# loicmagne/tinynerf

Measured on AMD Instinct MI355X. Metric: ray-samples/sec (K-Planes training step: sampler + render fwd + bwd + Adam), higher is better.
Workload: dtype f32 (f16x2-split products)

## Files before the change

include/tinynerf_hip.h:

```cpp
#ifndef TINYNERF_HIP_H
#define TINYNERF_HIP_H

#include <stdint.h>

#ifdef __cplusplus
extern "C" {
#endif

#define TN_ABI_VERSION 6

enum {
    TN_OK = 0,
    TN_E_NULL = -1,
    TN_E_SIZE = -2,
    TN_E_CONFIG = -3,
    TN_E_ALIGN = -4
};

const char *tn_last_error_string(void);
const char *tn_last_warning_string(void);
int tn_abi_version(void);

int tn_weights_fwd(const float *sigmas, const float *steps, const int32_t *info, float threshold,
                   float *weights, int64_t n_samples, int64_t n_rays, void *stream);
// ... 78 lines not shown
#define TN_MLP_STASHED 2
#define TN_MLP_CHAIN_ONLY 4
#define TN_MLP_WGRAD_ONLY 8
#define TN_MLP_GRAD_Y_ROWS 16

#define TN_MLP_BF16X3 32

#define TN_MLP_F16X2 64

#define TN_MLP_ROWS_ONLY 128
#define TN_MLP_X_FROM_ROWS 256

#define TN_MLP_SKIP_LAST 1024
#define TN_MLP_LAYERWISE 2048
#define TN_MLP_LEAN 512

typedef struct tn_mlp_desc {
    int32_t n_layers;
    int32_t in_dim;
    int32_t dims[TN_MLP_MAX_LAYERS + 1];
    int32_t encoding;
    int32_t n_freqs;
    int32_t out_activation;
    int32_t flags;
    const float *freqs;
    const float *weights[TN_MLP_MAX_LAYERS];
    const float *biases[TN_MLP_MAX_LAYERS];
    const int32_t *aux_index;
    int32_t aux_stride;
    int32_t reserved;
    const float *row_gate;
    const float *x_rows;
    float *grad_x_rows;
    int64_t x_rows_tile_stride;
    int64_t grad_x_rows_tile_stride;
    const void *grad_x_mask_rows;
    int64_t grad_x_mask_tile_stride;
} tn_mlp_desc;

#define TN_MERGE_MAX_HEADS 4
typedef struct tn_merge_head {
    const float *weight, *bias;
    int32_t rows, ld, col0, reserved;
    float *out_weight, *out_bias;
    const float *grad_merged_weight, *grad_merged_bias;
} tn_merge_head;
int tn_linear_merge_fwd(int32_t n_heads, const tn_merge_head *heads, const float *w_last, const float *b_last, int32_t F, void *stream);
int tn_linear_merge_bwd(int32_t n_heads, const tn_merge_head *heads, const float *w_last, const float *b_last, int32_t F,
                        float *grad_w_last, float *grad_b_last, void *stream);

int tn_linear_fwd(const float *x, const float *weight, const float *bias, int64_t n, int32_t in_features,
                  int32_t out_features, float *y, void *stream);
int tn_linear_bwd(const float *x, const float *weight, const float *grad_y, int64_t n, int32_t in_features,
                  int32_t out_features, float *grad_x, float *grad_weight, float *grad_bias, void *stream);

int tn_mlp_rows_view(const tn_mlp_desc *desc, int64_t n, int64_t *y_rows, int64_t *grad_y_rows, int64_t *tile_stride);
int tn_mlp_rows_view_hidden(const tn_mlp_desc *desc, int64_t n, int64_t *h_rows, int64_t *grad_h_rows, int64_t *mask_rows,
                            int64_t *tile_stride);

int tn_mlp_fwd(const tn_mlp_desc *desc, const float *x, const float *aux, int64_t n, float *y,
               float *pre_act, void *stream);
int64_t tn_mlp_fwd_workspace_bytes(const tn_mlp_desc *desc, int64_t n);
int tn_mlp_fwd_ws(const tn_mlp_desc *desc, const float *x, const float *aux, int64_t n, float *y, void *workspace,
                  int64_t workspace_bytes, void *stream);
int tn_mlp_fwd_stash(const tn_mlp_desc *desc, const float *x, const float *aux, int64_t n, float *y,
                     void *workspace, int64_t workspace_bytes, void *stream);
int tn_mlp_fwd_stash_pair(const tn_mlp_desc *desc, const tn_mlp_desc *partner, const float *x, const float *aux, int64_t n,
                          float *y, float *partner_y, void *workspace, int64_t workspace_bytes, void *partner_workspace,
                          int64_t partner_workspace_bytes, void *stream);
int tn_dir_encode(const float *dirs, int64_t n, const float *freqs, int n_freqs, float *out, int stride, void *stream);
int64_t tn_mlp_bwd_workspace_bytes(const tn_mlp_desc *desc, int64_t n);
int tn_mlp_bwd(const tn_mlp_desc *desc, const float *x, const float *aux, const float *grad_y,
               int64_t n, float *const *grad_weights, float *const *grad_biases, float *grad_x,
               void *workspace, int64_t workspace_bytes, void *stream);
int tn_mlp_bwd_pair(const tn_mlp_desc *desc, const tn_mlp_desc *partner, const float *x, const float *aux,
                    const float *grad_y, const float *partner_grad_y, int64_t n, float *const *grad_weights,
                    float *const *grad_biases, float *const *partner_grad_weights, float *const *partner_grad_biases,
                    float *grad_x, void *workspace, int64_t workspace_bytes, void *partner_workspace,
                    int64_t partner_workspace_bytes, void *stream);

int tn_mlp_lean_supported(const tn_mlp_desc *desc, const tn_mlp_desc *partner);

#define TN_KPLANES_MAX_SCALES 4
typedef struct tn_kplanes_desc {
    int32_t n_scales;
    int32_t channels;
    int32_t height[TN_KPLANES_MAX_SCALES];
    int32_t width[TN_KPLANES_MAX_SCALES];
    const float *planes[TN_KPLANES_MAX_SCALES][3];
} tn_kplanes_desc;

int tn_kplanes_fwd(const tn_kplanes_desc *desc, const float *x, int64_t x_stride, int64_t n,
                   float *feat, void *stream);
int tn_kplanes_bwd(const tn_kplanes_desc *desc, const float *x, int64_t x_stride, int64_t n,
                   const float *grad_feat, float *const (*grad_planes)[3], void *stream);

int tn_plane_reg_fwd(const float *plane, int H, int W, int C, double *sums, void *stream);
int tn_plane_reg_bwd(const float *plane, int H, int W, int C, float cy, float cx, float cl1,
                     const float *upstream, float *grad, void *stream);

#define TN_MULTI_MAX 32
typedef struct tn_plane_reg_item {
    const float *plane;
    float *grad;
    int32_t H, W, C;
    float cy, cx, cl1;
} tn_plane_reg_item;
int tn_plane_reg_multi(const tn_plane_reg_item *items, int32_t n_items, float upstream, double *sums, void *stream);

#define TN_COBAFA_MAX_LEVELS 8
typedef struct tn_cobafa_desc {
    int32_t n_levels;
    int32_t coef_res[3];
    int32_t res[TN_COBAFA_MAX_LEVELS][3];
    int32_t channels[TN_COBAFA_MAX_LEVELS];
    float freqs[TN_COBAFA_MAX_LEVELS];
    const float *coef;
    const float *basis[TN_COBAFA_MAX_LEVELS];
} tn_cobafa_desc;
int tn_cobafa_fwd(const tn_cobafa_desc *desc, const float *x, int64_t n, float *feat, void *stream);
int tn_cobafa_bwd(const tn_cobafa_desc *desc, const float *x, int64_t n, const float *grad_feat, float *grad_coef,
                  float *const *grad_basis, void *stream);

#define TN_HASHGRID_MAX_LEVELS 16
typedef struct tn_hashgrid_desc {
    int32_t n_levels, features;
    int32_t res[TN_HASHGRID_MAX_LEVELS];
    int32_t hashed[TN_HASHGRID_MAX_LEVELS];
    int64_t entries[TN_HASHGRID_MAX_LEVELS];
    int64_t offset[TN_HASHGRID_MAX_LEVELS];
    const float *table;
} tn_hashgrid_desc;
int tn_hashgrid_fwd(const tn_hashgrid_desc *desc, const float *x, int64_t x_stride, int64_t n, float *feat, void *stream);
int tn_hashgrid_bwd(const tn_hashgrid_desc *desc, const float *x, int64_t x_stride, int64_t n, const float *grad_feat,
                    float *grad_table, void *stream);

int tn_kplanes_mlp_fwd_pair(const tn_kplanes_desc *kdesc, const float *coords, int64_t coord_stride, const tn_mlp_desc *desc,
                            const tn_mlp_desc *partner, const float *aux, int64_t n, float *feat, float *y, float *partner_y,
                            void *workspace, int64_t workspace_bytes, void *partner_workspace, int64_t partner_workspace_bytes,
                            void *stream);

int tn_kplanes_mlp_fwd(const tn_kplanes_desc *kdesc, const float *coords, int64_t coord_stride, const tn_mlp_desc *desc, int64_t n,
                       float *feat, float *y, void *stream);

int tn_kplanes_mlp_bwd_pair(const tn_kplanes_desc *kdesc, const float *coords, int64_t coord_stride,
                            float *const (*grad_planes)[3], const tn_mlp_desc *desc, const tn_mlp_desc *partner,
                            const float *feat, const float *aux, const float *grad_y, const float *partner_grad_y, int64_t n,
                            float *const *grad_weights, float *const *grad_biases, float *const *partner_grad_weights,
                            float *const *partner_grad_biases, float *grad_feat, void *workspace, int64_t workspace_bytes,
                            void *partner_workspace, int64_t partner_workspace_bytes, void *stream);

int tn_basis_dot_fwd(const float *f, const float *basis, int64_t n, int32_t channels, int32_t n_out, int32_t activation,
                     float *out, void *stream);
int tn_basis_dot_bwd(const float *f, const float *basis, const float *grad_out, int64_t n, int32_t channels, int32_t n_out,
                     int32_t activation, float *grad_f, float *grad_basis, int32_t accumulate_f, void *stream);

int tn_ray_aux(const float *packed, const int32_t *info, int64_t n_rays, int32_t *ray_ids, float *steps, float *dirs,
               void *stream);

int tn_mse_grad(const float *rendered, const float *target, int64_t n, float scale, const float *scale_dev, float *grad,
                double *sumsq, void *stream);
int tn_render_rays_fwd(const float *sigmas, const float *steps, const float *rgbs, const int32_t *info, const float *bg,
                       float threshold, float *weights, float *rendered, float *gate, int64_t n_samples, int64_t n_rays,
                       void *stream);
int tn_render_rays_bwd(const float *sigmas, const float *steps, const float *rgbs, const int32_t *info, const float *bg,
                       const float *weights, const float *grad_rendered, float *grad_rgbs, float *grad_sigmas,
                       int64_t n_samples, int64_t n_rays, void *stream);
int tn_mse_grad_gated(const float *rendered, const float *target, int64_t n, float scale, const float *scale_dev,
                      const float *gate, float *grad, double *sumsq, void *stream);

enum { TN_DIST_LINEAR = 0, TN_DIST_UNBOUNDED = 1 };
int tn_distortion_fwd(const float *weights, const float *t_values, const float *steps, const int32_t *info, int64_t n_rays,
                      int32_t warp, float near, float range, float *loss, double *sum, void *stream);
int tn_distortion_bwd(const float *weights, const float *t_values, const float *steps, const int32_t *info, int64_t n_rays,
                      int32_t warp, float near, float range, const float *grad_loss, float scale, const float *scale_dev,
                      float *grad_weights, void *stream);
int tn_render_rays_bwd_dw(const float *sigmas, const float *steps, const float *rgbs, const int32_t *info, const float *bg,
                          const float *weights, const float *grad_rendered, const float *grad_weights_extra, float *grad_rgbs,
                          float *grad_sigmas, int64_t n_samples, int64_t n_rays, void *stream);
int tn_ssim_workspace_bytes(int64_t H, int64_t W, int32_t C, int64_t *bytes);
int tn_ssim(const float *a, const float *b, int64_t H, int64_t W, int32_t C, float data_range, float *map, void *workspace,
            int64_t workspace_bytes, float *mean, void *stream);
int tn_gather_rays(const float *rays_o, const float *rays_d, const float *rgbs, const int32_t *idx, int64_t n,
                   float *out_o, float *out_d, float *out_rgb, void *stream);
typedef struct tn_camera_table {
    const float *c2w;
    const float *lens;
    const int32_t *model;
    const int32_t *size;
    const int64_t *pixel_offset;
    const uint8_t *rgb;
    int64_t n_pixels;
    int32_t n_img, reserved;
} tn_camera_table;
enum { TN_LENS_PINHOLE = 0, TN_LENS_OPENCV = 1, TN_LENS_FISHEYE = 2 };
int tn_camera_rays(const tn_camera_table *cams, const int32_t *idx, int64_t first, int64_t stride, int64_t n,
                   float *out_o, float *out_d, float *out_rgb, void *stream);
int tn_points_workspace_bytes(int64_t n, int64_t *bytes);
int tn_points_compact(const float *rays_o, const float *rays_d,
                      const float *rgb,
                      const float *opacity, const float *depth,
                      const float *bg,
                      const float *box,
                      float min_opacity, int64_t n, int64_t capacity,
                      float *points,
                      uint8_t *colors,
                      int32_t *src,
                      int64_t *count,
                      void *workspace, void *stream);

int tn_adam_step(float *param, float *grad, float *exp_avg, float *exp_avg_sq, int64_t n, float lr, float beta1,
                 float beta2, float eps, float weight_decay, int32_t step, int32_t zero_grad, void *stream);

typedef struct tn_adam_item {
    float *param, *grad, *exp_avg, *exp_avg_sq;
    int64_t n;
} tn_adam_item;
int tn_adam_multi(const tn_adam_item *items, int32_t n_items, float lr, float beta1, float beta2, float eps,
                  float weight_decay, int32_t step, int32_t zero_grad, void *stream);

int tn_adam_multi_gated(const tn_adam_item *items, int32_t n_items, float lr, float beta1, float beta2, float eps,
                        float weight_decay, int32_t *step_dev, const float *gate, int32_t zero_grad, void *stream);

typedef struct tn_adam_reg_item {
    const float *param;
    float *param_out, *grad, *exp_avg, *exp_avg_sq;
    int64_t n;
    int32_t H, W, C, sum_slot;
    float cy, cx, cl1;
    int32_t row0, row1, reserved;
} tn_adam_reg_item;
int tn_adam_reg_multi(const tn_adam_reg_item *items, int32_t n_items, float lr, float beta1, float beta2, float eps,
                      float weight_decay, int32_t step, int32_t zero_grad, float upstream, double *sums, void *stream);

#ifdef __cplusplus
}
#endif
#endif
```

tinynerf_amd/_lib.py:

```python
from __future__ import annotations

import ctypes as C
import os
from typing import Optional

import torch

_HERE = os.path.dirname(os.path.abspath(__file__))
LIB_PATH = os.environ.get("TN_LIB_PATH") or os.path.join(_HERE, "libtinynerf_hip.so")

TN_MLP_MAX_LAYERS = 12
TN_KPLANES_MAX_SCALES = 4

MARCH_AABB, MARCH_UNBOUNDED = 0, 1
CONTRACT_AABB, CONTRACT_MIP360_INF, CONTRACT_MIP360_L2 = 0, 1, 2
ACT_NONE, ACT_EXP_M1, ACT_SIGMOID, ACT_EXP = 0, 1, 2, 3
ENC_NONE, ENC_POSENC, ENC_DIR_CAT, ENC_AUX_CAT = 0, 1, 2, 3
DIST_LINEAR, DIST_UNBOUNDED = 0, 1


class SamplerDesc(C.Structure):
    _fields_ = [
        ("marcher", C.c_int32), ("contraction", C.c_int32), ("n_samples", C.c_int32),
        ("grid_d", C.c_int32), ("grid_h", C.c_int32), ("grid_w", C.c_int32),
        ("aabb", C.c_float * 6), ("near", C.c_float), ("far", C.c_float),
        ("step_size", C.c_float), ("threshold", C.c_float),
        ("t_table", C.c_void_p), ("delta_table", C.c_void_p), ("grid", C.c_void_p), ("jitter", C.c_void_p),
        ("seed", C.c_uint64), ("use_rng", C.c_int32), ("reserved", C.c_int32),
        ("coarse", C.c_void_p),
    ]


class MlpDesc(C.Structure):
    _fields_ = [
        ("n_layers", C.c_int32), ("in_dim", C.c_int32), ("dims", C.c_int32 * (TN_MLP_MAX_LAYERS + 1)),
        ("encoding", C.c_int32), ("n_freqs", C.c_int32), ("out_activation", C.c_int32), ("flags", C.c_int32),
        ("freqs", C.c_void_p),
        ("weights", C.c_void_p * TN_MLP_MAX_LAYERS), ("biases", C.c_void_p * TN_MLP_MAX_LAYERS),
        ("aux_index", C.c_void_p), ("aux_stride", C.c_int32), ("reserved", C.c_int32),
        ("row_gate", C.c_void_p),
        ("x_rows", C.c_void_p), ("grad_x_rows", C.c_void_p), ("x_rows_tile_stride", C.c_int64), ("grad_x_rows_tile_stride", C.c_int64),
        ("grad_x_mask_rows", C.c_void_p), ("grad_x_mask_tile_stride", C.c_int64),
    ]


class MergeHead(C.Structure):
    _fields_ = [
        ("weight", C.c_void_p), ("bias", C.c_void_p),
        ("rows", C.c_int32), ("ld", C.c_int32), ("col0", C.c_int32), ("reserved", C.c_int32),
        ("out_weight", C.c_void_p), ("out_bias", C.c_void_p),
        ("grad_merged_weight", C.c_void_p), ("grad_merged_bias", C.c_void_p),
    ]


class KPlanesDesc(C.Structure):
    _fields_ = [
        ("n_scales", C.c_int32), ("channels", C.c_int32),
        ("height", C.c_int32 * TN_KPLANES_MAX_SCALES), ("width", C.c_int32 * TN_KPLANES_MAX_SCALES),
        ("planes", (C.c_void_p * 3) * TN_KPLANES_MAX_SCALES),
    ]


TN_COBAFA_MAX_LEVELS = 8
TN_MULTI_MAX = 32
MLP_ACCUM_GRAD_X = 1
MLP_STASHED = 2
MLP_CHAIN_ONLY = 4
MLP_WGRAD_ONLY = 8
MLP_GRAD_Y_ROWS = 16
MLP_BF16X3 = 32
MLP_F16X2 = 64
MLP_ROWS_ONLY = 128
MLP_X_FROM_ROWS = 256
MLP_LEAN = 512
MLP_SKIP_LAST = 1024
MLP_LAYERWISE = 2048
ABI_VERSION = 6


class PlaneRegItem(C.Structure):
    _fields_ = [("plane", C.c_void_p), ("grad", C.c_void_p), ("H", C.c_int32), ("W", C.c_int32), ("C", C.c_int32),
                ("cy", C.c_float), ("cx", C.c_float), ("cl1", C.c_float)]


class AdamItem(C.Structure):
    _fields_ = [("param", C.c_void_p), ("grad", C.c_void_p), ("exp_avg", C.c_void_p), ("exp_avg_sq", C.c_void_p), ("n", C.c_int64)]



class AdamRegItem(C.Structure):
    _fields_ = [("param", C.c_void_p), ("param_out", C.c_void_p), ("grad", C.c_void_p), ("exp_avg", C.c_void_p), ("exp_avg_sq", C.c_void_p),
                ("n", C.c_int64), ("H", C.c_int32), ("W", C.c_int32), ("C", C.c_int32), ("sum_slot", C.c_int32),
                ("cy", C.c_float), ("cx", C.c_float), ("cl1", C.c_float), ("row0", C.c_int32), ("row1", C.c_int32), ("reserved", C.c_int32)]


class CobafaDesc(C.Structure):
    _fields_ = [
        ("n_levels", C.c_int32), ("coef_res", C.c_int32 * 3), ("res", (C.c_int32 * 3) * TN_COBAFA_MAX_LEVELS),
        ("channels", C.c_int32 * TN_COBAFA_MAX_LEVELS), ("freqs", C.c_float * TN_COBAFA_MAX_LEVELS),
        ("coef", C.c_void_p), ("basis", C.c_void_p * TN_COBAFA_MAX_LEVELS),
    ]


TN_HASHGRID_MAX_LEVELS = 16


class HashGridDesc(C.Structure):
    _fields_ = [
        ("n_levels", C.c_int32), ("features", C.c_int32),
        ("res", C.c_int32 * TN_HASHGRID_MAX_LEVELS), ("hashed", C.c_int32 * TN_HASHGRID_MAX_LEVELS),
        ("entries", C.c_int64 * TN_HASHGRID_MAX_LEVELS), ("offset", C.c_int64 * TN_HASHGRID_MAX_LEVELS),
        ("table", C.c_void_p),
    ]


LENS_PINHOLE, LENS_OPENCV, LENS_FISHEYE = 0, 1, 2


class CameraTable(C.Structure):
    _fields_ = [("c2w", C.c_void_p), ("lens", C.c_void_p), ("model", C.c_void_p), ("size", C.c_void_p), ("pixel_offset", C.c_void_p),
                ("rgb", C.c_void_p), ("n_pixels", C.c_int64), ("n_img", C.c_int32), ("reserved", C.c_int32)]


_lib: Optional[C.CDLL] = None
_TRACE = bool(os.environ.get("TN_TRACE"))


def lib() -> C.CDLL:
    global _lib
    if _lib is None:
        if not os.path.exists(LIB_PATH):
            raise RuntimeError(
                f"{LIB_PATH} is missing: the HIP kernels were not built. Run `python -m tinynerf_amd.build` "
                "(needs hipcc). tinynerf_amd has no CPU fallback.")
        _lib = C.CDLL(LIB_PATH)
        _lib.tn_last_error_string.restype = C.c_char_p
        got = int(_lib.tn_abi_version())
        if got != ABI_VERSION:
            _lib = None
            raise RuntimeError(f"{LIB_PATH} has ABI version {got}, tinynerf_amd expects {ABI_VERSION}: rebuild it (`python -m tinynerf_amd.build`)")
    return _lib


def check(rc: int, fn: str) -> None:
    if rc != 0:
        msg = lib().tn_last_error_string().decode(errors="replace")
        raise RuntimeError(f"{fn} failed (code {rc}): {msg}")


def ptr(t: Optional[torch.Tensor]) -> C.c_void_p:
    return C.c_void_p(None) if t is None else C.c_void_p(t.data_ptr())


def stream(device: torch.device) -> C.c_void_p:
    return C.c_void_p(torch.cuda.current_stream(device).cuda_stream)


def require_cuda(*tensors: Optional[torch.Tensor]) -> torch.device:
    dev = None
    for t in tensors:
        if t is None:
            continue
        if not t.is_cuda:
            raise RuntimeError("tinynerf_amd: tensor must be a CUDA (HIP) tensor -- there is no CPU path")
        if not t.is_contiguous():
            raise RuntimeError("tinynerf_amd: tensor must be contiguous")
        if dev is None:
            dev = t.device
        elif t.device != dev:
            raise RuntimeError("tinynerf_amd: tensors are on different devices")
    assert dev is not None
    return dev


def call_plain(name: str, *args) -> None:
    check(getattr(lib(), name)(*args), name)
# ... 12 lines not shown
```

tinynerf_amd/config.py:

```python
from __future__ import annotations

import itertools
import os
from dataclasses import dataclass, fields, replace
from typing import Iterator, Mapping

MATMULS = ("f16x2", "bf16x3", "fp32")
_FLAGS = {"rows_handoff": "TN_ROWS_HANDOFF", "merge_last": "TN_MERGE_LAST", "heads_pair": "TN_HEADS_PAIR", "kp_lean": "TN_KP_LEAN",
          "infer_pair": "TN_INFER_PAIR", "adam_overlap": "TN_ADAM_OVERLAP", "side_plan": "TN_SIDE_PLAN"}


@dataclass(frozen=True)
class Config:
    matmul: str = "f16x2"
    rows_handoff: bool = True
    merge_last: bool = True
    heads_pair: bool = True
    kp_lean: bool = True
    infer_pair: bool = True
    adam_overlap: bool = True
    side_plan: bool = True

    def validate(self) -> "Config":
        if self.matmul not in MATMULS:
            raise RuntimeError(f"TN_MATMUL={self.matmul}: fp32, bf16x3 or f16x2")
        off = [n for n in _FLAGS if not getattr(self, n)]
        if self.matmul != "f16x2" and off:
            raise RuntimeError(f"tinynerf_amd.config: {', '.join(_FLAGS[n] + '=0' for n in off)} with TN_MATMUL={self.matmul}: the A / B switches "
                               "belong to the f16x2 path; with bf16x3 / fp32 they stay at their defaults (see tinynerf_amd/config.py)")
        if self.merge_last and not self.rows_handoff:
            return replace(self, merge_last=False)
        return self

    @staticmethod
    def from_env(env: Mapping[str, str] = os.environ) -> "Config":
        kw = {"matmul": env.get("TN_MATMUL", "f16x2").lower()}
        for name, var in _FLAGS.items():
            kw[name] = env.get(var, "1") != "0"
        return Config(**kw).validate()

    def as_env(self) -> dict:
        return {"TN_MATMUL": self.matmul, **{var: "1" if getattr(self, name) else "0" for name, var in _FLAGS.items()}}


def supported_combinations() -> Iterator[Config]:
    seen = set()
    for mm in MATMULS:
        names = list(_FLAGS) if mm == "f16x2" else []
        for bits in itertools.product((True, False), repeat=len(names)):
            try:
                c = Config(matmul=mm, **dict(zip(names, bits))).validate()
            except RuntimeError:
                continue
            if c not in seen:
                seen.add(c)
                yield c


def apply(cfg: Config) -> None:
    from . import fused, models, run
    cfg = cfg.validate()
    models.MATMUL = cfg.matmul
    fused.ROWS_HANDOFF, fused.MERGE_LAST, fused.HEADS_PAIR_BACKWARD = cfg.rows_handoff, cfg.merge_last, cfg.heads_pair
    fused.KP_LEAN, fused.INFER_PAIR = cfg.kp_lean, cfg.infer_pair
    run.ADAM_OVERLAP, run.SIDE_PLAN = cfg.adam_overlap, cfg.side_plan


CONFIG = Config.from_env()
```

tinynerf_amd/csrc/kplanes.hip:

```cpp
#include "kplanes_scatter.h"
#include <algorithm>

namespace {

using tn::f32x4k;

struct KpArgs {
    int n_scales, C;
    int H[TN_KPLANES_MAX_SCALES], W[TN_KPLANES_MAX_SCALES];
    const float *planes[TN_KPLANES_MAX_SCALES][3];
    float *grads[TN_KPLANES_MAX_SCALES][3];
};

template <int NV>
__global__ __launch_bounds__(256) void kplanes_fwd_kernel(KpArgs a, const float *__restrict__ x, int64_t x_stride,
                                                          int64_t n, float *__restrict__ feat)
{
    const int lane = tn::lane_id(), j = lane & 31, h = lane >> 5;
    const int64_t n_tiles = (n + 31) >> 5;
    const int C = a.C, FD = a.n_scales * C;
    for (int64_t tile = (int64_t)blockIdx.x * 4 + (threadIdx.x >> 6); tile < n_tiles; tile += (int64_t)gridDim.x * 4) {
        const int64_t row = tile * 32 + j;
        if (row >= n) continue;
        const float xs[3] = {x[row * x_stride], x[row * x_stride + 1], x[row * x_stride + 2]};
        for (int s = 0; s < a.n_scales; ++s) {
            f32x4k prod[NV];
#pragma unroll
            for (int q = 0; q < NV; ++q) prod[q] = f32x4k{1.f, 1.f, 1.f, 1.f};
#pragma unroll
            for (int p = 0; p < 3; ++p) {
                if (a.planes[s][p] == nullptr) continue;
                float u, v;
                tn::pair_uv(xs, p, u, v);
                const tn::PlaneTaps t = tn::plane_taps(u, v, a.H[s], a.W[s], C);
                f32x4k val[NV];
                tn::plane_gather<NV>(a.planes[s][p], t, h * (C / 2), val);
#pragma unroll
                for (int q = 0; q < NV; ++q) prod[q] = prod[q] * val[q];
            }
            f32x4k *o = reinterpret_cast<f32x4k *>(feat + row * FD + s * C + h * (C / 2));
#pragma unroll
            for (int q = 0; q < NV; ++q) o[q] = prod[q];
        }
    }
}

template <int NV>
__global__ __launch_bounds__(256, 3) void kplanes_bwd_kernel(KpArgs a, const float *__restrict__ x, int64_t x_stride,
                                                          int64_t n, const float *__restrict__ grad_feat)
{
    __shared__ __attribute__((aligned(16))) float lds[4 * tn::KP_WAVE_LDS];
    const int lane = tn::lane_id(), j = lane & 31, h = lane >> 5;
    float *wave_lds = lds + (threadIdx.x >> 6) * tn::KP_WAVE_LDS;
    const int64_t n_tiles = (n + 31) >> 5;
    const int C = a.C, FD = a.n_scales * C;
    for (int64_t tile = (int64_t)blockIdx.x * 4 + (threadIdx.x >> 6); tile < n_tiles; tile += (int64_t)gridDim.x * 4) {
        const int64_t row = tile * 32 + j;
        const bool valid = row < n;
        const int64_t rr = valid ? row : 0;
        const float xs[3] = {x[rr * x_stride], x[rr * x_stride + 1], x[rr * x_stride + 2]};
        for (int s = 0; s < a.n_scales; ++s) {
            f32x4k g[NV];
#pragma unroll
            for (int q = 0; q < NV; ++q)
                g[q] = valid ? reinterpret_cast<const f32x4k *>(grad_feat + row * FD + s * C + h * (C / 2))[q]
                             : f32x4k{0.f, 0.f, 0.f, 0.f};
            const float *const pl[3] = {a.planes[s][0], a.planes[s][1], a.planes[s][2]};
            float *const gr[3] = {a.grads[s][0], a.grads[s][1], a.grads[s][2]};
            tn::kp_scatter_scale<NV, 4>(pl, gr, a.H[s], a.W[s], C, xs, valid, g, h * (C / 2), wave_lds, j, h);
        }
    }
}

int make_args(const tn_kplanes_desc *d, KpArgs &a, float *const (*grads)[3])
{
    TN_REQUIRE(d, TN_E_NULL, "kplanes: null descriptor");
    TN_REQUIRE(d->n_scales >= 1 && d->n_scales <= TN_KPLANES_MAX_SCALES, TN_E_CONFIG, "kplanes: n_scales out of range");
    TN_REQUIRE(d->channels == 8 || d->channels == 16 || d->channels == 32, TN_E_CONFIG, "kplanes: channels must be 8, 16 or 32");
    a.n_scales = d->n_scales; a.C = d->channels;
    for (int s = 0; s < d->n_scales; ++s) {
        TN_REQUIRE(d->height[s] > 0 && d->width[s] > 0, TN_E_SIZE, "kplanes: bad plane resolution");
        TN_REQUIRE((int64_t)d->height[s] * d->width[s] * d->channels < (1ll << 30), TN_E_SIZE, "kplanes: plane too large (2^30 elements)");
        a.H[s] = d->height[s]; a.W[s] = d->width[s];
        TN_REQUIRE(d->planes[s][0], TN_E_NULL, "kplanes: null plane pointer");
        for (int p = 0; p < 3; ++p) {
            TN_REQUIRE(((uintptr_t)d->planes[s][p] & 15) == 0, TN_E_ALIGN, "kplanes: planes must be 16-byte aligned");
            a.planes[s][p] = d->planes[s][p];
            a.grads[s][p] = nullptr;
            if (grads && d->planes[s][p]) {
                TN_REQUIRE(grads[s][p], TN_E_NULL, "kplanes: null grad plane pointer");
                a.grads[s][p] = grads[s][p];
            }
        }
    }
    return TN_OK;
}

template <int ACT>
__device__ __forceinline__ float bd_act(float v)
{
    if (ACT == TN_ACT_EXP_M1) return expf(v - 1.0f);
    if (ACT == TN_ACT_EXP) return expf(v);
    if (ACT == TN_ACT_SIGMOID) return 1.0f / (1.0f + expf(-v));
    return v;
}

template <int ACT>
__global__ __launch_bounds__(256) void basis_dot_fwd_kernel(const float *__restrict__ f, const float *__restrict__ basis, int64_t n, int C,
                                                            int K, float *__restrict__ out)
{
    const int lane = tn::lane_id();
    const int64_t wave = ((int64_t)blockIdx.x * blockDim.x + threadIdx.x) >> 6, n_waves = ((int64_t)gridDim.x * blockDim.x) >> 6;
    for (int64_t i = wave; i < n; i += n_waves) {
        const float *fi = f + i * C, *bi = basis + i * (int64_t)K * C;
        for (int k = 0; k < K; ++k) {
            float acc = 0.0f;
            for (int c = lane; c < C; c += 64) acc += fi[c] * bi[k * C + c];
            acc = tn::wave_sum(acc);
            if (lane == 0) out[i * K + k] = bd_act<ACT>(acc);
        }
    }
}

template <int ACT>
__global__ __launch_bounds__(256) void basis_dot_bwd_kernel(const float *__restrict__ f, const float *__restrict__ basis,
                                                            const float *__restrict__ g_out, int64_t n, int C, int K,
                                                            float *__restrict__ g_f, float *__restrict__ g_basis, int accumulate_f)
{
    const int lane = tn::lane_id();
    const int64_t wave = ((int64_t)blockIdx.x * blockDim.x + threadIdx.x) >> 6, n_waves = ((int64_t)gridDim.x * blockDim.x) >> 6;
    for (int64_t i = wave; i < n; i += n_waves) {
        const float *fi = f + i * C, *bi = basis + i * (int64_t)K * C;
        float gv[4];
        for (int k = 0; k < K; ++k) {
            float acc = 0.0f;
            for (int c = lane; c < C; c += 64) acc += fi[c] * bi[k * C + c];
            acc = tn::wave_sum(acc);
            const float g = g_out[i * K + k];
            if (ACT == TN_ACT_EXP_M1) gv[k] = g * expf(fminf(fmaxf(acc - 1.0f, -15.0f), 15.0f));
            else if (ACT == TN_ACT_EXP) gv[k] = g * expf(fminf(fmaxf(acc, -15.0f), 15.0f));
            else if (ACT == TN_ACT_SIGMOID) { const float y = 1.0f / (1.0f + expf(-acc)); gv[k] = g * y * (1.0f - y); }
            else gv[k] = g;
        }
        for (int c = lane; c < C; c += 64) {
            const float fc = fi[c];
            float a = accumulate_f ? g_f[i * C + c] : 0.0f;
            for (int k = 0; k < K; ++k) {
                a += gv[k] * bi[k * C + c];
                if (g_basis) g_basis[(i * K + k) * C + c] = gv[k] * fc;
            }
            g_f[i * C + c] = a;
        }
    }
}

inline unsigned tile_blocks(int64_t n) { return (unsigned)std::min<int64_t>(((n + 31) / 32 + 3) / 4, 256 * 8); }

}

extern "C" int tn_kplanes_fwd(const tn_kplanes_desc *desc, const float *x, int64_t x_stride, int64_t n, float *feat,
                              void *stream)
{
    KpArgs a;
    if (int rc = make_args(desc, a, nullptr)) return rc;
    TN_REQUIRE(n >= 0 && x_stride >= 3, TN_E_SIZE, "tn_kplanes_fwd: bad size");
    if (n == 0) return TN_OK;
    TN_REQUIRE(x && feat, TN_E_NULL, "tn_kplanes_fwd: null pointer");
    TN_REQUIRE(((uintptr_t)feat & 15) == 0, TN_E_ALIGN, "tn_kplanes_fwd: feat must be 16-byte aligned");
    hipStream_t s = (hipStream_t)stream;
    const dim3 grid(tile_blocks(n)), block(256);
    switch (a.C) {
    case 8: kplanes_fwd_kernel<1><<<grid, block, 0, s>>>(a, x, x_stride, n, feat); break;
    case 16: kplanes_fwd_kernel<2><<<grid, block, 0, s>>>(a, x, x_stride, n, feat); break;
    default: kplanes_fwd_kernel<4><<<grid, block, 0, s>>>(a, x, x_stride, n, feat); break;
    }
    return tn::check_launch("kplanes_fwd_kernel");
}
// ... 57 lines not shown
```

tinynerf_amd/csrc/kplanes_device.h:

```cpp
#pragma once
#include "tn_common.h"

namespace tn {

typedef float f32x4k __attribute__((ext_vector_type(4)));

struct PlaneTaps {
    int off[4];
    float w[4];
    int cell;
};

__device__ __forceinline__ PlaneTaps plane_taps(float u, float v, int H, int W, int C) {
    PlaneTaps t;
    float u1 = u + 1.0f, v1 = v + 1.0f;
    asm volatile("" : "+v"(u1), "+v"(v1));
    float ix = (u1 * 0.5f) * (float)(W - 1);
    float iy = (v1 * 0.5f) * (float)(H - 1);
    asm volatile("" : "+v"(ix), "+v"(iy));
    const float x0f = floorf(ix), y0f = floorf(iy);
    const float fx = ix - x0f, fy = iy - y0f;
    const float gx = (x0f + 1.0f) - ix, gy = (y0f + 1.0f) - iy;
    t.w[0] = gx * gy; t.w[1] = fx * gy; t.w[2] = gx * fy; t.w[3] = fx * fy;
    const bool bx0 = x0f >= 0.0f && x0f < (float)W, bx1 = x0f + 1.0f >= 0.0f && x0f + 1.0f < (float)W;
    const bool by0 = y0f >= 0.0f && y0f < (float)H, by1 = y0f + 1.0f >= 0.0f && y0f + 1.0f < (float)H;
    const int x0 = bx0 ? (int)x0f : 0, x1 = bx1 ? (int)x0f + 1 : 0;
    const int y0 = by0 ? (int)y0f : 0, y1 = by1 ? (int)y0f + 1 : 0;
    t.off[0] = (bx0 && by0) ? (y0 * W + x0) * C : -1;
    t.off[1] = (bx1 && by0) ? (y0 * W + x1) * C : -1;
    t.off[2] = (bx0 && by1) ? (y1 * W + x0) * C : -1;
    t.off[3] = (bx1 && by1) ? (y1 * W + x1) * C : -1;
    const float cx = fminf(fmaxf(x0f, -2.0f), (float)W + 1.0f), cy = fminf(fmaxf(y0f, -2.0f), (float)H + 1.0f);
    t.cell = ((int)cy + 2) * (W + 4) + (int)cx + 2;
    return t;
}

template <int NV, int CS = 4>
__device__ __forceinline__ void plane_gather(const float *__restrict__ plane, const PlaneTaps &t, int c0, f32x4k (&out)[NV]) {
    f32x4k tex[4][NV];
    float w[4];
    const char *base = reinterpret_cast<const char *>(plane);
#pragma unroll
    for (int k = 0; k < 4; ++k) {
        const bool in = t.off[k] >= 0;
        unsigned boff = (unsigned)((in ? t.off[k] : 0) + c0) * 4u;
        asm volatile("" : "+v"(boff));
        w[k] = in ? t.w[k] : 0.0f;
#pragma unroll
        for (int v = 0; v < NV; ++v) tex[k][v] = *reinterpret_cast<const f32x4k *>(base + boff + (unsigned)(v * CS * 4));
    }
#pragma unroll
    for (int v = 0; v < NV; ++v) {
        f32x4k acc = tex[0][v] * w[0];
#pragma unroll
        for (int k = 1; k < 4; ++k)
#pragma unroll
            for (int e = 0; e < 4; ++e) acc[e] = __builtin_fmaf(tex[k][v][e], w[k], acc[e]);
        out[v] = acc;
    }
}

__device__ __forceinline__ void pair_uv(const float x[3], int p, float &u, float &v) {
    u = (p == 2) ? x[1] : x[0];
    v = (p == 0) ? x[1] : x[2];
}

}
```

tinynerf_amd/csrc/kplanes_scatter.h:

```cpp
#pragma once
#include "kplanes_device.h"

#ifdef TN_PHASE_TIMERS
extern __device__ unsigned long long tn_phase_cycles_b[16];
#endif
namespace tn {

constexpr int KP_GS = 36;
constexpr int KP_WAVE_LDS = 32 * KP_GS + 2 * 4 * 32;

template <int NV, int CS>
__device__ __forceinline__ void kp_scatter_scale(const float *const (&planes)[3], float *const (&grads)[3], int H, int W, int C,
                                                 const float (&xs)[3], bool valid, const f32x4k (&g)[NV], int c0,
                                                 float *__restrict__ wave_lds, int j, int h)
{
#ifdef TN_PHASE_TIMERS
    unsigned long long pts_ = __builtin_amdgcn_s_memtime();
#define TN_PTS(k) { __builtin_amdgcn_sched_barrier(0); const unsigned long long n_ = __builtin_amdgcn_s_memtime(); if (tn::lane_id() == 0) atomicAdd(&tn_phase_cycles_b[k], n_ - pts_); pts_ = __builtin_amdgcn_s_memtime(); __builtin_amdgcn_sched_barrier(0); }
#endif
    float *tileG = wave_lds;
    int *tileO = reinterpret_cast<int *>(tileG + 32 * KP_GS);
    float *tileW = tileG + 32 * KP_GS + 4 * 32;
    PlaneTaps t[3];
    f32x4k val[3][NV];
#pragma unroll
    for (int p = 0; p < 3; ++p) {
        float u, v;
        pair_uv(xs, p, u, v);
        t[p] = plane_taps(u, v, H, W, C);
        if (planes[p]) {
            plane_gather<NV, CS>(planes[p], t[p], c0, val[p]);
            __builtin_amdgcn_sched_barrier(0);
        } else {
#pragma unroll
            for (int q = 0; q < NV; ++q) val[p][q] = f32x4k{1.f, 1.f, 1.f, 1.f};
        }
    }
#ifdef TN_PHASE_TIMERS
    TN_PTS(8)
#endif
#pragma unroll
    for (int p = 0; p < 3; ++p) {
        if (grads[p] == nullptr) continue;
#pragma unroll
        for (int q = 0; q < NV; ++q) {
            const f32x4k gp = p == 0 ? g[q] * val[1][q] * val[2][q]
                                     : (p == 1 ? g[q] * val[0][q] * val[2][q] : g[q] * (val[0][q] * val[1][q]));
            *reinterpret_cast<f32x4k *>(tileG + j * KP_GS + c0 + CS * q) = gp;
        }
#pragma unroll
        for (int k = 0; k < 2; ++k) {
            const int o = h ? t[p].off[2 + k] : t[p].off[0 + k];
            const float w = h ? t[p].w[2 + k] : t[p].w[0 + k];
            const bool live = valid && o >= 0;
            tileO[(2 * h + k) * 32 + j] = live ? 4 * o : 0;
            tileW[(2 * h + k) * 32 + j] = live ? w : 0.0f;
        }
        const int cell = valid ? t[p].cell : -1 - j;
        const int next_cell = __shfl_down(cell, 1, 64);
        const int dcell = (j < 31) ? next_cell - cell : 0x40000000;
        const int rowlen = W + 4;
        const unsigned run_end = (unsigned)__ballot(dcell != 0);
        const unsigned mv_xp = (unsigned)__ballot(dcell == 1), mv_xm = (unsigned)__ballot(dcell == -1);
        const unsigned mv_yp = (unsigned)__ballot(dcell == rowlen), mv_ym = (unsigned)__ballot(dcell == -rowlen);
        const unsigned mv_pp = (unsigned)__ballot(dcell == rowlen + 1), mv_mp = (unsigned)__ballot(dcell == rowlen - 1);
        const unsigned mv_pm = (unsigned)__ballot(dcell == -rowlen + 1), mv_mm = (unsigned)__ballot(dcell == -rowlen - 1);
        const unsigned mv_diag = mv_pp | mv_mp | mv_pm | mv_mm;
        asm volatile("" ::: "memory");
#ifdef TN_PHASE_TIMERS
        TN_PTS(9)
#endif
        const int c = j;
        char *const gplane = reinterpret_cast<char *>(grads[p]);
        const unsigned c4 = 4u * (unsigned)c;
        auto add_at = [&](unsigned byte_off, float v) { atomicAdd(reinterpret_cast<float *>(gplane + byte_off), v); };
        if (c < C) {
            const int4 *O0 = reinterpret_cast<const int4 *>(tileO + (2 * h) * 32), *O1 = O0 + 8;
            const f32x4k *W0 = reinterpret_cast<const f32x4k *>(tileW + (2 * h) * 32);
            const f32x4k *W1 = W0 + 8;
            float a0 = 0.0f, a1 = 0.0f;
#pragma clang loop unroll(disable)
            for (int s4 = 0; s4 < 8; ++s4) {
                const f32x4k w0 = W0[s4], w1 = W1[s4];
                const int4 o0v = O0[s4], o1v = O1[s4];
                const int o0a[4] = {o0v.x, o0v.y, o0v.z, o0v.w}, o1a[4] = {o1v.x, o1v.y, o1v.z, o1v.w};
                float gv[4];
#pragma unroll
                for (int u = 0; u < 4; ++u) gv[u] = tileG[(4 * s4 + u) * KP_GS + c];
#pragma unroll
                for (int u = 0; u < 4; ++u) {
                    const int sI = 4 * s4 + u;
                    a0 = fmaf(gv[u], w0[u], a0);
                    a1 = fmaf(gv[u], w1[u], a1);
                    if ((run_end >> sI) & 1u) {
                        const unsigned o0 = (unsigned)o0a[u] + c4, o1 = (unsigned)o1a[u] + c4;
                        if ((mv_xp >> sI) & 1u) {
                            add_at(o0, a0);
                            a0 = a1; a1 = 0.0f;
                        } else if ((mv_xm >> sI) & 1u) {
                            add_at(o1, a1);
                            a1 = a0; a0 = 0.0f;
                        } else if ((mv_yp >> sI) & 1u) {
                            const float t0 = __shfl_xor(a0, 32, 64), t1 = __shfl_xor(a1, 32, 64);
                            if (h == 0) {
                                add_at(o0, a0);
                                add_at(o1, a1);
                            }
                            a0 = h == 0 ? t0 : 0.0f; a1 = h == 0 ? t1 : 0.0f;
                        } else if ((mv_ym >> sI) & 1u) {
                            const float t0 = __shfl_xor(a0, 32, 64), t1 = __shfl_xor(a1, 32, 64);
                            if (h == 1) {
                                add_at(o0, a0);
                                add_at(o1, a1);
                            }
                            a0 = h == 1 ? t0 : 0.0f; a1 = h == 1 ? t1 : 0.0f;
                        } else if ((mv_diag >> sI) & 1u) {
                            const float t0 = __shfl_xor(a0, 32, 64), t1 = __shfl_xor(a1, 32, 64);
                            if ((mv_pp >> sI) & 1u) {
                                add_at(o0, a0);
                                if (h == 0) add_at(o1, a1);
                                a0 = h == 0 ? t1 : 0.0f; a1 = 0.0f;
                            } else if ((mv_mp >> sI) & 1u) {
                                add_at(o1, a1);
                                if (h == 0) add_at(o0, a0);
                                a1 = h == 0 ? t0 : 0.0f; a0 = 0.0f;
                            } else if ((mv_pm >> sI) & 1u) {
                                add_at(o0, a0);
                                if (h == 1) add_at(o1, a1);
                                a0 = h == 1 ? t1 : 0.0f; a1 = 0.0f;
                            } else {
                                add_at(o1, a1);
                                if (h == 1) add_at(o0, a0);
                                a1 = h == 1 ? t0 : 0.0f; a0 = 0.0f;
                            }
                        } else {
                            add_at(o0, a0);
                            add_at(o1, a1);
                            a0 = 0.0f; a1 = 0.0f;
                        }
                    }
                }
            }
        }
        asm volatile("" ::: "memory");
// ... 8 lines not shown
```

tinynerf_amd/csrc/mlp_bwd2.hip:

```cpp
#include "mlp_stage.h"
#include "kplanes_scatter.h"
#include "phase_timers.h"
#include <algorithm>
#include <type_traits>

extern "C" int64_t tn_mlp_bwd_layers_workspace_bytes(const tn_mlp_desc *desc, int64_t n);
extern "C" int tn_mlp_bwd_layers(const tn_mlp_desc *desc, const float *x, const float *aux, const float *grad_y, int64_t n,
                                 float *const *grad_weights, float *const *grad_biases, float *grad_x, float *workspace, void *stream);
extern "C" int tn_mlp_wgrad_rows2(const float *g_rows, int64_t g_stride, const float *g_rows2, int64_t g_stride2, const float *a_rows,
                                  int64_t a_stride, int na, float *gW, int ldw, int col0, float *gB, float *gW2, int ldw2, int col02,
                                  float *gB2, int64_t n, void *stream);
extern "C" int tn_heads_dx_rows(const float *w_a, int ld_a, int col0_a, const float *w_b, int ld_b, int col0_b, const float *g_a, int64_t gs_a,
                                const float *g_b, int64_t gs_b, int F, float *out, int64_t out_stride, const void *mask, int64_t mask_stride,
                                int64_t n, void *stream);
extern "C" int tn_mlp_wgrad_lean_pair(const tn_mlp_desc *desc, const tn_mlp_desc *partner, const float *x, const float *aux, int64_t n,
                                      float *const *gw, float *const *gb, float *const *gws, float *const *gbs, const float *ws_a,
                                      const float *ws_b, void *stream);
extern "C" int tn_mlp_wgrad_lean_check(const tn_mlp_desc *desc, const tn_mlp_desc *partner, const float *x, const float *aux, int64_t n,
                                       float *const *gw, float *const *gb, float *const *gws, float *const *gbs, const float *ws_a,
                                       const float *ws_b);
extern "C" int tn_mlp_wgrad_rows(const float *g_rows, int64_t g_stride, int ng, const float *a_rows, int64_t a_stride, int na, float *gW,
                                 int ldw, int col0, int kmax, float *gB, int64_t n, void *stream);

TN_PHASE_COUNTERS(tn_phase_cycles_b, tn_debug_phase_cycles_b)
#define TN_PTB_BEGIN TN_PHASE_BEGIN(ptb_)
#define TN_PTB(k) TN_PHASE(tn_phase_cycles_b, ptb_, k)
namespace {

using tn::f32x16;
using tn::f32x4;
using tn::act_grad;
using namespace tn::mlp;

template <int N, class F>
__device__ __forceinline__ void static_for(F &&f) {
    if constexpr (N > 0) {
        static_for<N - 1>(f);
        f(std::integral_constant<int, N - 1>{});
    }
}

struct PairArgs { MlpArgs b; const float *gy; float *stash; int64_t g0_stride = 0; };

struct KpBwd {
    int H[3], W[3];
    const float *planes[3][3];
    float *grads[3][3];
    const float *coords;
    int64_t coord_stride;
};

template <int H>
__device__ __forceinline__ void first_dgrad(const float *__restrict__ Wf, int sf, int out, const float (&gp)[4],
                                            const unsigned (&mask)[H / 32], int h, f32x16 (&G)[H / 32])
{
#pragma unroll
    for (int kb = 0; kb < H / 32; ++kb) {
#pragma unroll
        for (int q = 0; q < 4; ++q) {
            f32x4 acc4 = {0.f, 0.f, 0.f, 0.f};
#pragma unroll
            for (int o = 0; o < 4; ++o) {
                if (o < out) {
                    const f32x4 w = *reinterpret_cast<const f32x4 *>(Wf + o * sf + 32 * kb + 8 * q + 4 * h);
                    acc4 += w * gp[o];
                }
            }
#pragma unroll
            for (int u = 0; u < 4; ++u) G[kb][4 * q + u] = mask_keep(acc4[u], mask[kb], 4 * q + u);
        }
    }
}

template <int H, int NH, int WPB, bool STASHED, bool ACCUM = false, bool PAIR = false, bool KP = false, bool G0B = false>
__global__ __launch_bounds__(WPB * 64) void mlp_chain_kernel(MlpArgs a, const float *__restrict__ x, const float *__restrict__ aux,
                                                             const float *__restrict__ gy, int64_t n, float *__restrict__ gx,
                                                             float *__restrict__ stash, PairArgs pr, KpBwd kp)
{
    static_assert(!KP || (STASHED && PAIR && !ACCUM && H == 64), "the fused scatter belongs to the paired, stashed chain of the width-64 heads");
    static_assert(!G0B || (STASHED && !PAIR && !KP && !ACCUM), "G0B: another head's G_0 rows join a stashed, unpaired chain's grad_x");
    extern __shared__ __attribute__((aligned(16))) float lds[];
    constexpr int T = H / 32;
    constexpr int L = NH + 1;
    stage_weights(a, lds);
    const float *ldsb = lds + a.lds_floats;
    if constexpr (PAIR || G0B) stage_weights(pr.b, lds + a.lds_floats);
    __syncthreads();
    if constexpr (STASHED && NH > 1) {
        constexpr int sl = H + 4;
        for (int l = 1; l < NH; ++l) {
            float *W = lds + a.w_off[l];
            for (int e = threadIdx.x; e < H * H; e += blockDim.x) {
                const int r = e / H, c = e - r * H;
                if (r < c) { const float t = W[r * sl + c]; W[r * sl + c] = W[c * sl + r]; W[c * sl + r] = t; }
            }
        }
        __syncthreads();
    }
    const int lane = tn::lane_id(), j_ = lane & 31, h_ = lane >> 5;
    const int wave = __builtin_amdgcn_readfirstlane(threadIdx.x >> 6);
    const int64_t n_tiles = (n + 31) >> 5;
    const int out = a.out_dim;

    unsigned nmask[NH][T];
    float npre[4], ngy[4];
    unsigned bmask[T];
    float bpre[4], bgy[4];
    const StashTile sb(H, 1, 0);
    const StashTile sa(H, NH, a.enc, a.in_dim, a.K0_pad);
    auto fetch_tile = [&](int64_t t) {
        if constexpr (PAIR) {
            const float *tb = pr.stash + t * (int64_t)sb.floats(), *qb = tb + sb.pre();
            const unsigned *mb = reinterpret_cast<const unsigned *>(tb + sb.masks());
#pragma unroll
            for (int ob = 0; ob < T; ++ob) bmask[ob] = mb[sb.mask(0, ob) + lane];
            int64_t rb = t * 32 + j_;
            rb = rb < n ? rb : n - 1;
            const int outb = pr.b.out_dim;
#pragma unroll
            for (int o = 0; o < 4; ++o) {
                const int oc = o < outb ? o : outb - 1;
                bpre[o] = qb[oc * 32 + j_];
                bgy[o] = pr.gy[rb * outb + oc];
            }
        }
        const float *ta = stash + t * (int64_t)sa.floats(), *q = ta + sa.pre();
        const unsigned *mm = reinterpret_cast<const unsigned *>(ta + sa.masks());
#pragma unroll
        for (int l = 0; l < NH; ++l)
#pragma unroll
            for (int ob = 0; ob < T; ++ob) nmask[l][ob] = mm[sa.mask(l, ob) + lane];
        int64_t r = t * 32 + j_;
        r = r < n ? r : n - 1;
#pragma unroll
        for (int o = 0; o < 4; ++o) {
            const int oc = o < out ? o : out - 1;
            npre[o] = q[oc * 32 + j_];
            ngy[o] = gy[r * out + oc];
        }
    };
    if constexpr (STASHED) {
        const int64_t t0 = (int64_t)blockIdx.x * WPB + wave;
        fetch_tile(t0 < n_tiles ? t0 : n_tiles - 1);
    }

    for (int64_t tile = (int64_t)blockIdx.x * WPB + wave; tile < n_tiles; tile += (int64_t)gridDim.x * WPB) {
        int j = j_, h = h_;
        asm volatile("" : "+v"(j), "+v"(h));
        TN_PTB_BEGIN
        const int64_t row = tile * 32 + j;
        const bool valid = row < n;
        float *st = stash + tile * (int64_t)sa.floats();
        float *stH = st, *stG = st + sa.g(0), *stP = st + sa.g_pre(), *stE = st + sa.e();
        const float *Wf = lds + a.w_off[L - 1];
        const float *Bf = lds + a.b_off[L - 1];
        const int sf = a.stride[L - 1];
        unsigned mask[NH][T];
        float gp[4];
        unsigned pmask[T];
        float gpb[4];
        if constexpr (STASHED) {
#pragma unroll
            for (int l = 0; l < NH; ++l)
#pragma unroll
                for (int ob = 0; ob < T; ++ob) mask[l][ob] = nmask[l][ob];
#pragma unroll
            for (int o = 0; o < 4; ++o) gp[o] = (valid && o < out) ? ngy[o] * act_grad(npre[o], a.out_act) : 0.0f;
            if constexpr (PAIR) {
#pragma unroll
// ... 139 lines not shown
                {
                    constexpr int NG = 4 * T;
                    float cur[4], nxt[4];
#pragma unroll
                    for (int u = 0; u < 4; ++u) cur[u] = W0[(4 * h + u) * s0 + 32 * kt + j];
#pragma unroll
                    for (int g = 0; g < NG; ++g) {
                        const int tn_ = g >> 2, q = g & 3;
                        if (g + 1 < NG) {
#pragma unroll
                            for (int u = 0; u < 4; ++u) nxt[u] = W0[(8 * (g + 1) + 4 * h + u) * s0 + 32 * kt + j];
                        }
#pragma unroll
                        for (int u = 0; u < 4; ++u) acc = tn::mfma32(cur[u], G[tn_][4 * q + u], acc);
                        __builtin_amdgcn_sched_barrier(0);
#pragma unroll
                        for (int u = 0; u < 4; ++u) cur[u] = nxt[u];
                    }
                }
                if constexpr (PAIR || G0B) {
                    const float *W0b = ldsb + pr.b.w_off[0];
                    const int s0b = pr.b.stride[0];
#pragma unroll
                    for (int tn_ = 0; tn_ < T; ++tn_)
#pragma unroll
                        for (int q = 0; q < 4; ++q)
#pragma unroll
                            for (int u = 0; u < 4; ++u)
                                acc = tn::mfma32(W0b[(32 * tn_ + 8 * q + 4 * h + u) * s0b + 32 * kt + j], Gb[tn_][4 * q + u], acc);
                }
                tn::pin16(acc);
                if constexpr (KP) {
                    if (kt == 0) gacc[0] = acc; else if (kt == 1) gacc[1] = acc; else gacc[2] = acc;
                    if (gx == nullptr) continue;
                }
                if (gxr != nullptr) {
                    if (!KP && a.gx_mask_rows != nullptr) {
                        const unsigned mb = a.gx_mask_rows[tile * a.gx_mask_stride + kt * 64 + lane];
#pragma unroll
                        for (int r = 0; r < 16; ++r) acc[r] = mask_keep(acc[r], mb, r);
                    }
                    store_rows(gxr + kt * 32 * 32, acc, 0, j, h);
                    continue;
                }
                if constexpr (ACCUM) {
                    if (valid) {
#pragma unroll
                        for (int q = 0; q < 4; ++q) {
                            f32x4 v = old[q];
#pragma unroll
                            for (int u = 0; u < 4; ++u) v[u] += acc[4 * q + u];
                            *reinterpret_cast<f32x4 *>(gx + row * a.in_dim + 32 * kt + 8 * q + 4 * h) = v;
                        }
                    }
#pragma unroll
                    for (int q = 0; q < 4; ++q) old[q] = oldn[q];
                } else if (valid) {
#pragma unroll
                    for (int q = 0; q < 4; ++q) {
                        const int f0 = 32 * kt + 8 * q + 4 * h;
                        if (f0 + 3 < a.in_dim && (a.in_dim & 3) == 0) {
                            f32x4 v;
#pragma unroll
                            for (int u = 0; u < 4; ++u) v[u] = acc[4 * q + u];
                            f32x4 *dst = reinterpret_cast<f32x4 *>(gx + row * a.in_dim + f0);
                            if (a.accum_gx) v += *dst;
                            *dst = v;
                        } else {
#pragma unroll
                            for (int u = 0; u < 4; ++u)
                                if (f0 + u < a.in_dim) {
                                    float *dst = gx + row * a.in_dim + f0 + u;
                                    *dst = a.accum_gx ? *dst + acc[4 * q + u] : acc[4 * q + u];
                                }
                        }
                    }
                }
            }
            TN_PTB(2)
            if constexpr (KP) {
                const float *cr = kp.coords + (valid ? row : 0) * kp.coord_stride;
                const float xs[3] = {cr[0], cr[1], cr[2]};
                float *wave_lds = lds + a.lds_floats + pr.b.lds_floats + wave * tn::KP_WAVE_LDS;
#pragma unroll
                for (int sc = 0; sc < 3; ++sc) {
                    tn::f32x4k g4[4];
#pragma unroll
                    for (int q = 0; q < 4; ++q) g4[q] = tn::f32x4k{gacc[sc][4 * q], gacc[sc][4 * q + 1], gacc[sc][4 * q + 2], gacc[sc][4 * q + 3]};
                    const float *const pl[3] = {kp.planes[sc][0], kp.planes[sc][1], kp.planes[sc][2]};
                    float *const gr[3] = {kp.grads[sc][0], kp.grads[sc][1], kp.grads[sc][2]};
                    tn::kp_scatter_scale<4, 8>(pl, gr, kp.H[sc], kp.W[sc], 32, xs, valid, g4, 4 * h, wave_lds, j, h);
                    TN_PTB(3 + sc)
                }
            }
        }
    }
}

struct WgradArgs {
    int n_layers, in_dim, K0, K0_pad, enc, n_freqs, out_dim, Tk0, total_tiles;
    int tk_skip;
    const int *aux_index;
    int aux_stride;
    float *gW[TN_MLP_MAX_LAYERS];
    float *gB[TN_MLP_MAX_LAYERS];
    int K[TN_MLP_MAX_LAYERS], N[TN_MLP_MAX_LAYERS];
};

constexpr int RS = 36;

template <bool AUX>
__device__ __forceinline__ void first_layer_column(const WgradArgs &a, int q, int xs, int aw, const float *ldsX, const float *ldsA, int h,
                                                   const float *&cp, int &cstride)
{
    if (q < xs) { cp = ldsX + 16 * h * a.in_dim + q; cstride = a.in_dim; }
    else if (AUX && q < a.K0_pad) { cp = ldsA + 16 * h * aw + (q - xs); cstride = aw; }
}

__device__ __forceinline__ void flush_tile(const WgradArgs &a, int l, int tn_, int tk, f32x16 &acc, float dbsum, int i, int h)
{
    tn::pin16(acc);
    const int Nl = a.N[l], Kl = a.K[l];
    const int k = 32 * tk + i;
    const bool kok = k < Kl;
    float *col = a.gW[l] + (kok ? (l == 0 ? layer0_col(a.enc, a.K0, a.in_dim, k) : k) : 0);
#pragma unroll
    for (int r = 0; r < 16; ++r) {
        const int nn = 32 * tn_ + tn::frow(r, h);
        if (kok && nn < Nl) atomicAdd(col + (int64_t)nn * Kl, acc[r]);
    }
    if (tk == 0) {
        dbsum += __shfl_xor(dbsum, 32, 64);
        const int nn = 32 * tn_ + i;
        if (h == 0 && nn < Nl) atomicAdd(&a.gB[l][nn], dbsum);
    }
}

template <int H, int NH>
__device__ __forceinline__ void decode_tile(const WgradArgs &a, int id, int &l, int &tn_, int &tk) {
    constexpr int T = H / 32;
    const int tk0n = a.Tk0 - a.tk_skip;
    const int n0 = T * tk0n;
    if (id < n0) { l = 0; tn_ = id / tk0n; tk = a.tk_skip + id - tn_ * tk0n; return; }
    id -= n0;
    if (id < (NH - 1) * T * T) { l = 1 + id / (T * T); id -= (l - 1) * T * T; tn_ = id / T; tk = id - tn_ * T; return; }
    id -= (NH - 1) * T * T;
    l = NH; tn_ = 0; tk = id;
}

template <int H, int NH, int MAXS, int NW, int NCH, bool AUX>
__global__ __launch_bounds__(NW * 64) void mlp_wgrad_kernel(WgradArgs a, const float *__restrict__ x, const float *__restrict__ aux,
                                                            int64_t n, const float *__restrict__ stash)
{
    extern __shared__ __attribute__((aligned(16))) float lds[];
    const int lane = tn::lane_id(), i_ = lane & 31, h_ = lane >> 5;
    const int wave = __builtin_amdgcn_readfirstlane(threadIdx.x >> 6);
    const int64_t n_tiles = (n + 31) >> 5;
    const int xs = x_slots(a.enc, a.in_dim);
    const int xs_st = 32 * a.tk_skip >= xs ? 0 : xs;
    const StashTile st(H, NH, a.enc, a.in_dim, a.K0_pad);
    const int extra = st.extra;
    const int R = st.rows_w();
    const int row_chunks = R * 8;
    const int x_chunks = xs_st > 0 ? (32 * a.in_dim) / 4 : 0;
    const int aw = AUX ? a.K0_pad - a.in_dim : 0;
    float *ldsR = lds;
    float *ldsX = lds + R * RS;
    float *ldsA = ldsX + (xs_st > 0 ? 32 * a.in_dim : 0);
    f32x16 acc[MAXS];
    float dbacc[MAXS];
    int tl[MAXS], ttn[MAXS], ttk[MAXS];
    tn::zero_tiles(acc);
#pragma unroll
    for (int m = 0; m < MAXS; ++m) {
// ... 210 lines not shown
            for (int e = 0; e < 4; ++e) {
                f32x4 gv0 = g0[e], gv1 = g1[e];
                if (!gok) { gv0 = f32x4{0.f, 0.f, 0.f, 0.f}; gv1 = gv0; }
                f32x4 av0 = {0.f, 0.f, 0.f, 0.f}, av1;
                if (kind == 0) {
                    if (cp != nullptr) {
#pragma unroll
                        for (int u = 0; u < 4; ++u) av0[u] = cp[(4 * e + u) * cstride];
                    }
                    av1 = av0;
                } else if (kind == 1) { av0 = hc[e]; av1 = av0; }
                else { av0 = r0[e]; av1 = r1[e]; }
#pragma unroll
                for (int u = 0; u < 4; ++u) {
                    acc[0] = tn::mfma32(gv0[u], av0[u], acc[0]);
                    acc[1] = tn::mfma32(gv1[u], av1[u], acc[1]);
                }
                gs0 += (gv0[0] + gv0[1]) + (gv0[2] + gv0[3]);
                gs1 += (gv1[0] + gv1[1]) + (gv1[2] + gv1[3]);
            }
            if (kind == 2 || tk == 0) { dbacc[0] += gs0; dbacc[1] += gs1; }
        }
        __syncthreads();
        cur ^= 1;
    }
    if (kind < 0) return;
#pragma unroll
    for (int m = 0; m < 2; ++m) flush_tile(a, l, kind == 2 ? 0 : m, kind == 2 ? m : tk, acc[m], dbacc[m], i_, h_);
}

struct WgradPlan { int R, Rt, xs, aw, chunks; size_t lds; };
WgradPlan wgrad_plan(int enc, int in_dim, int K0_pad, int H, int NH, bool x_elsewhere = false) {
    WgradPlan p;
    const StashTile st(H, NH, enc, in_dim, K0_pad);
    p.R = st.rows_w(); p.Rt = st.rows();
    p.xs = x_elsewhere ? 0 : x_slots(enc, in_dim);
    p.aw = enc == TN_ENC_AUX_CAT ? K0_pad - in_dim : 0;
    p.chunks = p.R * 8 + (p.xs > 0 ? 8 * in_dim : 0);
    p.lds = ((size_t)p.R * 36 + (p.xs > 0 ? 32 * (size_t)in_dim : 0) + 32 * (size_t)p.aw) * 4;
    return p;
}

MlpArgs compact_first_layer(const MlpArgs &a)
{
    MlpArgs c = a;
    const int H = a.N[0];
    c.K0_pad = (a.in_dim + 7) & ~7;
    lay_out_lds(c, H);
    return c;
}

MlpArgs first_layer_only(const MlpArgs &a)
{
    MlpArgs c = compact_first_layer(a);
    c.n_layers = 1;
    c.lds_floats = c.b_off[0] + ((a.N[0] + 3) & ~3);
    return c;
}

int launch_chain_g0b(const MlpArgs &b, const MlpArgs &a, const float *x, const float *gy_b, int64_t n, float *gx, float *stash_b,
                     const float *g0_rows_a, int64_t g0_stride_a, hipStream_t s)
{
    constexpr int WPS = 8;
    PairArgs pr;
    pr.b = first_layer_only(a); pr.gy = nullptr; pr.stash = const_cast<float *>(g0_rows_a); pr.g0_stride = g0_stride_a;
    const size_t lds_bytes = ((size_t)b.lds_floats + (size_t)pr.b.lds_floats) * 4;
    return launch(mlp_chain_kernel<64, 1, WPS, true, false, false, false, true>, WPS, lds_bytes, grid_per_cu(n, WPS, lds_bytes), s,
                  "mlp_chain_kernel(g0b)", b, x, nullptr, gy_b, n, gx, stash_b, pr, KpBwd());
}

StashTile stash_tile(const MlpArgs &m) { return StashTile(64, m.n_layers - 1, m.enc, m.in_dim, m.K0_pad); }
int64_t tile_floats(const MlpArgs &m) { return stash_tile(m).floats(); }
int64_t g0_floats(const MlpArgs &m) { return stash_tile(m).g(0); }

bool x_cols_from_rows(const MlpArgs &a, bool stashed) {
    return stashed && a.x_rows != nullptr && (a.in_dim == 128 || a.in_dim == 256) && x_slots(a.enc, a.in_dim) == a.in_dim;
}
bool x_cols_from_rows2(const MlpArgs &a, const MlpArgs &b) {
    return x_cols_from_rows(a, true) && b.x_rows == a.x_rows && b.x_rows_stride == a.x_rows_stride && extra_rows(a.enc, a.in_dim, a.K0_pad) == 0;
}

template <int H, int NH>
int launch_chain(const MlpArgs &a, const float *x, const float *aux, const float *gy, int64_t n, float *gx, float *stash, bool stashed,
                 hipStream_t s, const PairArgs *pair = nullptr, const KpBwd *kpb = nullptr)
{
    if (kpb) {
        if constexpr (H == 64 && NH == 4) {
            if (!(pair && stashed && a.enc == TN_ENC_AUX_CAT && a.in_dim == 96)) return tn::fail(TN_E_CONFIG, "mlp_bwd: fused scatter needs the paired K-Planes heads");
            constexpr int WPK = 8;
            const MlpArgs ac = compact_first_layer(a);
            PairArgs pr = *pair;
            pr.b = compact_first_layer(pair->b);
            const size_t lds_bytes = ((size_t)ac.lds_floats + (size_t)pr.b.lds_floats + (size_t)WPK * tn::KP_WAVE_LDS) * 4;
            if (lds_bytes > (size_t)LDS_LIMIT_BYTES) return tn::fail(TN_E_CONFIG, "mlp_bwd: weights + scatter tiles do not fit LDS");
            return launch(mlp_chain_kernel<H, NH, WPK, true, false, true, true>, WPK, lds_bytes, grid_blocks(n, WPK, 256), s,
                          "mlp_chain_kernel(kplanes)", ac, x, aux, gy, n, gx, stash, pr, *kpb);
        } else return tn::fail(TN_E_CONFIG, "mlp_bwd: fused scatter is built for the 5-layer colour head");
    }
    size_t lds_bytes = (size_t)a.lds_floats * 4;
    constexpr int WPB = 8;
    constexpr int WPS = NH == 1 ? 10 : 16;
    constexpr int WPP = 8;
    int wpb = stashed ? WPS : WPB;
    auto kern = stashed ? mlp_chain_kernel<H, NH, WPS, true> : mlp_chain_kernel<H, NH, WPB, false>;
    if (stashed && a.accum_gx && (gx != nullptr || a.gx_rows != nullptr) && a.enc != TN_ENC_POSENC && (a.in_dim & 31) == 0) kern = mlp_chain_kernel<H, NH, WPS, true, true>;
    PairArgs pr;
    pr.gy = nullptr; pr.stash = nullptr;
    if (pair) {
        pr = *pair;
        if constexpr (NH == 4) kern = mlp_chain_kernel<H, NH, WPP, true, false, true>;
        else return tn::fail(TN_E_CONFIG, "mlp_bwd: the paired chain is built for the 5-layer colour head");
        wpb = WPP;
        lds_bytes += (size_t)pr.b.lds_floats * 4;
    } else pr.b = a;
    if (lds_bytes > (size_t)LDS_LIMIT_BYTES) return tn::fail(TN_E_CONFIG, "mlp_bwd: weights do not fit LDS");
    return launch(kern, wpb, lds_bytes, grid_per_cu(n, wpb, lds_bytes), s, "mlp_chain_kernel", a, x, aux, gy, n, gx, stash, pr, KpBwd());
}

int chain(const MlpArgs &a, const float *x, const float *aux, const float *gy, int64_t n, float *gx, float *stash, bool stashed,
          hipStream_t s, const PairArgs *pair = nullptr, const KpBwd *kpb = nullptr)
{
    return a.n_layers == 2 ? launch_chain<64, 1>(a, x, aux, gy, n, gx, stash, stashed, s, pair, kpb)
                           : launch_chain<64, 4>(a, x, aux, gy, n, gx, stash, stashed, s, pair, kpb);
}

using WgradKern = decltype(&mlp_wgrad_kernel<64, 1, 1, 8, 4, false>);

struct WgradStep {
    WgradArgs w;
    bool rows;
    WgradKern kern;
    int waves;
    size_t lds;
    int64_t blocks;
    const char *what;
};

template <int H, int NH>
int plan_wgrad(WgradStep &st, const MlpArgs &a, float *const *gw, float *const *gb, int64_t n, bool stashed)
{
    WgradArgs &w = st.w;
    constexpr int T = H / 32;
    w.n_layers = a.n_layers; w.in_dim = a.in_dim; w.K0 = a.K0; w.K0_pad = a.K0_pad; w.enc = a.enc; w.n_freqs = a.n_freqs;
    w.out_dim = a.out_dim;
    w.Tk0 = (a.K0_pad + 31) / 32;
    for (int l = 0; l < a.n_layers; ++l) { w.gW[l] = gw[l]; w.gB[l] = gb[l]; w.K[l] = a.K[l]; w.N[l] = a.N[l]; }
    w.aux_index = a.aux_index; w.aux_stride = a.aux_stride;
    st.rows = x_cols_from_rows(a, stashed);
    w.tk_skip = st.rows ? a.in_dim / 32 : 0;
    w.total_tiles = T * (w.Tk0 - w.tk_skip) + (NH - 1) * T * T + T;
    const WgradPlan wp = wgrad_plan(a.enc, a.in_dim, a.K0_pad, H, NH, st.rows);
    if (wp.lds > (size_t)LDS_LIMIT_BYTES) return tn::fail(TN_E_CONFIG, "mlp_bwd: workspace tile does not fit LDS");
    if (wp.xs > 0 && (a.in_dim & 3)) return tn::fail(TN_E_CONFIG, "mlp_bwd: in_dim must be a multiple of 4");
    const bool aux = a.enc == TN_ENC_AUX_CAT;
    st.what = "mlp_wgrad_kernel";
    if (extra_rows(a.enc, a.in_dim, a.K0_pad) == 0 && (wp.xs > 0 || (st.rows && aux)) && NH >= 2) {
        if constexpr (H == 64 && NH >= 2) {
            constexpr int RG4 = H + NH * H + 4;
            const int xw4 = st.rows ? 0 : a.in_dim;
            st.lds = 2 * ((size_t)RG4 * RS + 32 * (size_t)xw4 + 32 * (size_t)wp.aw) * 4 + 32 * 16;
            if (st.lds <= (size_t)LDS_LIMIT_BYTES && w.Tk0 - w.tk_skip + (NH - 1) * 2 + 1 <= 12 && RG4 * 8 + 8 * xw4 <= 5 * 768) {
                st.kern = aux ? mlp_wgrad4_kernel<NH, 12, 5, true> : mlp_wgrad4_kernel<NH, 12, 5, false>;
                st.waves = 12; st.blocks = grid_blocks(n, 1, 256); st.what = "mlp_wgrad4_kernel";
                return TN_OK;
            }
        }
    }
    struct Tiling { int max_tiles, max_chunks; WgradKern kern; int waves; };
    const Tiling tilings[] = {
        {8, 4 * 512, mlp_wgrad_kernel<H, NH, 1, 8, 4, false>, 8},    {16, 4 * 1024, mlp_wgrad_kernel<H, NH, 1, 16, 4, false>, 16},
        {24, 7 * 768, mlp_wgrad_kernel<H, NH, 2, 12, 7, false>, 12}, {32, 6 * 1024, mlp_wgrad_kernel<H, NH, 2, 16, 6, false>, 16},
        {48, 10 * 1024, mlp_wgrad_kernel<H, NH, 3, 16, 10, false>, 16}};
    st.lds = wp.lds; st.blocks = grid_blocks(n, 1, 256 * (wp.lds * 2 <= (size_t)LDS_LIMIT_BYTES ? 2 : 1));
    if (aux) {
        if constexpr (NH == 4) {
            if (st.rows && w.total_tiles <= 24 && wp.chunks <= 7 * 768 && wp.aw <= 64) {
                st.kern = mlp_wgrad_kernel<H, NH, 2, 12, 7, true>; st.waves = 12; st.what = "mlp_wgrad_kernel(aux)";
                return TN_OK;
            }
        }
        return tn::fail(TN_E_CONFIG, "mlp_bwd: TN_ENC_AUX_CAT outside the paired weight-gradient tiling");
    }
    for (const Tiling &t : tilings)
        if (w.total_tiles <= t.max_tiles && wp.chunks <= t.max_chunks) { st.kern = t.kern; st.waves = t.waves; return TN_OK; }
    return tn::fail(TN_E_CONFIG, "mlp_bwd: configuration outside the wgrad tiling");
}

int plan_wgrad(WgradStep &st, const MlpArgs &a, float *const *gw, float *const *gb, int64_t n, bool stashed)
{
    return a.n_layers == 2 ? plan_wgrad<64, 1>(st, a, gw, gb, n, stashed) : plan_wgrad<64, 4>(st, a, gw, gb, n, stashed);
}

int run_wgrad(const WgradStep &st, const MlpArgs &a, const float *x, const float *aux, int64_t n, float *stash, hipStream_t s)
{
    if (st.rows && !a.x_wgrad_done) {
        const int col0 = (a.enc == TN_ENC_DIR_CAT || a.enc == TN_ENC_AUX_CAT) ? a.K0 - a.in_dim : 0;
        if (int rc = tn_mlp_wgrad_rows(stash + g0_floats(a), tile_floats(a), 64, a.x_rows, a.x_rows_stride, a.in_dim, st.w.gW[0], a.K0, col0,
                                       a.in_dim, st.w.gB[0], n, s)) return rc;
    }
    return launch(st.kern, st.waves, st.lds, st.blocks, s, st.what, st.w, x, aux, n, stash);
}

}

extern "C" int64_t tn_mlp_bwd_workspace_bytes(const tn_mlp_desc *desc, int64_t n)
{
    if (n <= 0 || !desc) return 0;
    if (!two_pass_supported(desc)) {
        if (desc->encoding == TN_ENC_AUX_CAT) return 0;
        return tn_mlp_bwd_layers_workspace_bytes(desc, n);
    }
    const int H = desc->dims[1], NH = desc->n_layers - 1;
    return ((n + 31) / 32) * (int64_t)StashTile(H, NH, desc->encoding, desc->in_dim, (desc->dims[0] + 7) & ~7).floats() * (int64_t)sizeof(float);
}

extern "C" int tn_mlp_bwd(const tn_mlp_desc *desc, const float *x, const float *aux, const float *grad_y, int64_t n,
                          float *const *grad_weights, float *const *grad_biases, float *grad_x, void *workspace,
                          int64_t workspace_bytes, void *stream)
{
    TN_REQUIRE(desc, TN_E_NULL, "tn_mlp_bwd: null descriptor");
    const int64_t need = tn_mlp_bwd_workspace_bytes(desc, n);
    const bool stashed = (desc->flags & TN_MLP_STASHED) != 0;
    const bool two_pass = two_pass_supported(desc);
    if (stashed || desc->encoding == TN_ENC_AUX_CAT) {
        TN_REQUIRE(two_pass || (stashed && desc->encoding != TN_ENC_AUX_CAT && need > 0), TN_E_CONFIG,
                   "tn_mlp_bwd: TN_ENC_AUX_CAT needs a configuration of the two-pass form, TN_MLP_STASHED one with a workspace");
        if (n == 0) return TN_OK;
        TN_REQUIRE(workspace && workspace_bytes >= need, TN_E_NULL, "tn_mlp_bwd: TN_MLP_STASHED / TN_ENC_AUX_CAT need the workspace");
    }
    if (!two_pass) {
        if (n == 0) return TN_OK;
        TN_REQUIRE(need > 0, TN_E_CONFIG, "tn_mlp_bwd: unsupported layer configuration");
        TN_REQUIRE(workspace && workspace_bytes >= need, TN_E_NULL, "tn_mlp_bwd: this configuration needs the workspace");
        TN_REQUIRE(((uintptr_t)workspace & 15) == 0, TN_E_ALIGN, "tn_mlp_bwd: workspace must be 16-byte aligned");
        return tn_mlp_bwd_layers(desc, x, aux, grad_y, n, grad_weights, grad_biases, grad_x, (float *)workspace, stream);
    }
    if (n == 0) return TN_OK;
    TN_REQUIRE(workspace != nullptr && workspace_bytes >= need, TN_E_NULL, "tn_mlp_bwd: workspace missing or too small (tn_mlp_bwd_workspace_bytes)");
    MlpArgs a;
    int H = 0;
    if (int rc = plan(desc, a, H)) return rc;
    TN_REQUIRE(x && grad_y && grad_weights && grad_biases, TN_E_NULL, "tn_mlp_bwd: null pointer");
    TN_REQUIRE((a.enc != TN_ENC_DIR_CAT && a.enc != TN_ENC_AUX_CAT) || aux, TN_E_NULL, "tn_mlp_bwd: dir_cat / aux_cat need aux");
    TN_REQUIRE(((uintptr_t)workspace & 15) == 0, TN_E_ALIGN, "tn_mlp_bwd: workspace must be 16-byte aligned");
    TN_REQUIRE(a.enc != TN_ENC_AUX_CAT || ((uintptr_t)aux & 15) == 0, TN_E_ALIGN, "tn_mlp_bwd: aux table must be 16-byte aligned");
    for (int l = 0; l < a.n_layers; ++l)
        TN_REQUIRE(grad_weights[l] && grad_biases[l], TN_E_NULL, "tn_mlp_bwd: null gradient pointer");
    hipStream_t s = (hipStream_t)stream;
    float *ws = (float *)workspace;
    WgradStep w;
    if (int rc = plan_wgrad(w, a, grad_weights, grad_biases, n, stashed)) return rc;
    if (int rc = chain(a, x, aux, grad_y, n, grad_x, ws, stashed, s)) return rc;
    return run_wgrad(w, a, x, aux, n, ws, s);
}

static int bwd_pair_common(const tn_mlp_desc *desc, const tn_mlp_desc *partner, const float *x, const float *aux,
                           const float *grad_y, const float *partner_grad_y, int64_t n, float *const *grad_weights,
                           float *const *grad_biases, float *const *partner_grad_weights, float *const *partner_grad_biases,
                           float *grad_x, void *workspace, int64_t workspace_bytes, void *partner_workspace,
                           int64_t partner_workspace_bytes, void *stream, const KpBwd *kpb)
{
    TN_REQUIRE(desc && partner, TN_E_NULL, "tn_mlp_bwd_pair: null descriptor");
    TN_REQUIRE((desc->flags & TN_MLP_STASHED) && (partner->flags & TN_MLP_STASHED), TN_E_CONFIG,
               "tn_mlp_bwd_pair: both heads need TN_MLP_STASHED workspaces (tn_mlp_fwd_stash)");
    TN_REQUIRE(two_pass_supported(desc) && two_pass_supported(partner), TN_E_CONFIG, "tn_mlp_bwd_pair: outside the two-pass form's configurations");
    TN_REQUIRE(desc->n_layers == 5 && partner->n_layers == 2 && partner->encoding == TN_ENC_NONE && partner->in_dim == desc->in_dim &&
                   partner->dims[1] == desc->dims[1] && desc->dims[1] == 64 && (desc->in_dim & 31) == 0 && desc->encoding != TN_ENC_POSENC,
               TN_E_CONFIG, "tn_mlp_bwd_pair: a 5-layer head and a 2-layer partner on the same x (width 64, in_dim % 32 == 0)");
    if (n == 0) return TN_OK;
    const int64_t need_a = tn_mlp_bwd_workspace_bytes(desc, n), need_b = tn_mlp_bwd_workspace_bytes(partner, n);
    TN_REQUIRE(workspace && workspace_bytes >= need_a && partner_workspace && partner_workspace_bytes >= need_b, TN_E_NULL,
               "tn_mlp_bwd_pair: workspace missing or too small");
    TN_REQUIRE(x && grad_y && partner_grad_y && (grad_x || kpb || desc->grad_x_rows) && grad_weights && grad_biases && partner_grad_weights && partner_grad_biases,
               TN_E_NULL, "tn_mlp_bwd_pair: null pointer");
    MlpArgs a, b;
    int H = 0, Hb = 0;
    if (int rc = plan(desc, a, H)) return rc;
    if (int rc = plan(partner, b, Hb)) return rc;
    TN_REQUIRE((a.enc != TN_ENC_DIR_CAT && a.enc != TN_ENC_AUX_CAT) || aux, TN_E_NULL, "tn_mlp_bwd_pair: dir_cat / aux_cat need aux");
    for (int l = 0; l < a.n_layers; ++l) TN_REQUIRE(grad_weights[l] && grad_biases[l], TN_E_NULL, "tn_mlp_bwd_pair: null gradient pointer");
    for (int l = 0; l < b.n_layers; ++l)
        TN_REQUIRE(partner_grad_weights[l] && partner_grad_biases[l], TN_E_NULL, "tn_mlp_bwd_pair: null gradient pointer");
    hipStream_t s = (hipStream_t)stream;
    float *ws_a = (float *)workspace, *ws_b = (float *)partner_workspace;
    PairArgs pr;
    pr.b = b; pr.gy = partner_grad_y; pr.stash = ws_b;
    a.accum_gx = 0;
    const bool chain_half = !(desc->flags & TN_MLP_WGRAD_ONLY), wgrad = !(desc->flags & TN_MLP_CHAIN_ONLY);
    TN_REQUIRE(chain_half || wgrad, TN_E_CONFIG, "tn_mlp_bwd_pair: TN_MLP_CHAIN_ONLY and TN_MLP_WGRAD_ONLY exclude each other");
    const bool lean = (desc->flags & TN_MLP_LEAN) != 0;
    TN_REQUIRE(lean == ((partner->flags & TN_MLP_LEAN) != 0), TN_E_CONFIG, "tn_mlp_bwd_pair: TN_MLP_LEAN must be set on both heads or on neither");
    if (lean) {
        if (wgrad)
            if (int rc = tn_mlp_wgrad_lean_check(desc, partner, x, aux, n, grad_weights, grad_biases, partner_grad_weights,
                                                 partner_grad_biases, ws_a, ws_b)) return rc;
        if (chain_half)
            if (int rc = chain(a, x, aux, grad_y, n, grad_x, ws_a, true, s, &pr, kpb)) return rc;
        if (!wgrad) return TN_OK;
        return tn_mlp_wgrad_lean_pair(desc, partner, x, aux, n, grad_weights, grad_biases, partner_grad_weights, partner_grad_biases,
                                      ws_a, ws_b, stream);
    }
    MlpArgs aw = a, bw = b;
    const bool rows2 = x_cols_from_rows2(a, b);
    if (rows2) { aw.x_wgrad_done = 1; bw.x_wgrad_done = 1; }
    WgradStep wa, wb;
    if (wgrad) {
        if (int rc = plan_wgrad(wa, aw, grad_weights, grad_biases, n, true)) return rc;
        if (int rc = plan_wgrad(wb, bw, partner_grad_weights, partner_grad_biases, n, true)) return rc;
    }
    const bool rows_split = kpb == nullptr && a.gx_rows != nullptr && b.gx_rows == a.gx_rows && a.x_rows != nullptr && grad_x == nullptr &&
                            a.enc == TN_ENC_AUX_CAT && (a.in_dim & 31) == 0 &&
                            ((size_t)b.lds_floats + (size_t)first_layer_only(a).lds_floats) * 4 <= (size_t)LDS_LIMIT_BYTES;
    const bool fits = kpb != nullptr || ((size_t)a.lds_floats + (size_t)b.lds_floats) * 4 <= (size_t)LDS_LIMIT_BYTES;
    if (chain_half) {
        if (rows_split) {
            MlpArgs a0 = a;
            a0.gx_rows = nullptr;
            if (int rc = chain(a0, x, aux, grad_y, n, nullptr, ws_a, true, s)) return rc;
            if (a.f2 && b.f2 && (a.in_dim == 128 || a.in_dim == 256)) {
                MlpArgs b0 = b;
                b0.gx_rows = nullptr;
                if (int rc = chain(b0, x, nullptr, partner_grad_y, n, nullptr, ws_b, true, s)) return rc;
                const int col0 = a.K0 - a.in_dim;
                if (int rc = tn_heads_dx_rows(desc->weights[0], a.K0, col0, partner->weights[0], b.K0, 0, ws_a + g0_floats(a), tile_floats(a),
                                              ws_b + g0_floats(b), tile_floats(b), a.in_dim, a.gx_rows, a.gx_rows_stride, a.gx_mask_rows,
                                              a.gx_mask_stride, n, s)) return rc;
            } else if (int rc = launch_chain_g0b(b, a, x, partner_grad_y, n, nullptr, ws_b, ws_a + g0_floats(a), tile_floats(a), s)) return rc;
        } else if (fits) {
            if (int rc = chain(a, x, aux, grad_y, n, grad_x, ws_a, true, s, &pr, kpb)) return rc;
        } else {
            if (int rc = chain(a, x, aux, grad_y, n, grad_x, ws_a, true, s)) return rc;
            MlpArgs b1 = b;
            b1.accum_gx = 1;
            if (int rc = chain(b1, x, nullptr, partner_grad_y, n, grad_x, ws_b, true, s)) return rc;
        }
    }
    if (!wgrad) return TN_OK;
    if (rows2) {
        const int col0 = (a.enc == TN_ENC_DIR_CAT || a.enc == TN_ENC_AUX_CAT) ? a.K0 - a.in_dim : 0;
        if (int rc = tn_mlp_wgrad_rows2(ws_a + g0_floats(a), tile_floats(a), ws_b + g0_floats(b), tile_floats(b), a.x_rows, a.x_rows_stride,
                                        a.in_dim, grad_weights[0], a.K0, col0, grad_biases[0], partner_grad_weights[0], b.K0, 0,
                                        partner_grad_biases[0], n, s)) return rc;
    }
    if (int rc = run_wgrad(wa, aw, x, aux, n, ws_a, s)) return rc;
    return run_wgrad(wb, bw, x, nullptr, n, ws_b, s);
}

extern "C" int tn_mlp_bwd_pair(const tn_mlp_desc *desc, const tn_mlp_desc *partner, const float *x, const float *aux,
                               const float *grad_y, const float *partner_grad_y, int64_t n, float *const *grad_weights,
                               float *const *grad_biases, float *const *partner_grad_weights, float *const *partner_grad_biases,
                               float *grad_x, void *workspace, int64_t workspace_bytes, void *partner_workspace,
                               int64_t partner_workspace_bytes, void *stream)
{
    return bwd_pair_common(desc, partner, x, aux, grad_y, partner_grad_y, n, grad_weights, grad_biases, partner_grad_weights,
                           partner_grad_biases, grad_x, workspace, workspace_bytes, partner_workspace, partner_workspace_bytes, stream,
                           nullptr);
}

extern "C" int tn_kplanes_mlp_bwd_pair(const tn_kplanes_desc *kd, const float *coords, int64_t coord_stride,
                                       float *const (*grad_planes)[3], const tn_mlp_desc *desc, const tn_mlp_desc *partner,
                                       const float *feat, const float *aux, const float *grad_y, const float *partner_grad_y, int64_t n,
                                       float *const *grad_weights, float *const *grad_biases, float *const *partner_grad_weights,
                                       float *const *partner_grad_biases, float *grad_feat, void *workspace, int64_t workspace_bytes,
                                       void *partner_workspace, int64_t partner_workspace_bytes, void *stream)
{
    TN_REQUIRE(kd && desc && partner && grad_planes, TN_E_NULL, "tn_kplanes_mlp_bwd_pair: null descriptor");
    TN_REQUIRE(kd->n_scales == 3 && kd->channels == 32 && desc->in_dim == 96 && partner->in_dim == 96 && desc->encoding == TN_ENC_AUX_CAT,
               TN_E_CONFIG, "tn_kplanes_mlp_bwd_pair: 3 scales x 32 channels feeding the aux-table colour head and the sigma head (run.py:136-139)");
    TN_REQUIRE(coord_stride >= 3, TN_E_SIZE, "tn_kplanes_mlp_bwd_pair: bad coordinate stride");
    if (n == 0) return TN_OK;
    TN_REQUIRE(coords, TN_E_NULL, "tn_kplanes_mlp_bwd_pair: null coordinates");
    KpBwd kp;
    if (int rc = kp_planes(kd, coords, coord_stride, kp)) return rc;
    for (int s = 0; s < 3; ++s)
        for (int p = 0; p < 3; ++p) kp.grads[s][p] = grad_planes[s][p];
    return bwd_pair_common(desc, partner, feat, aux, grad_y, partner_grad_y, n, grad_weights, grad_biases, partner_grad_weights,
                           partner_grad_biases, grad_feat, workspace, workspace_bytes, partner_workspace, partner_workspace_bytes, stream,
                           &kp);
}
```

tinynerf_amd/csrc/planes_reg.hip:

```cpp
#include "tn_common.h"
#include <algorithm>
#include <math.h>

namespace {

typedef float f4 __attribute__((ext_vector_type(4)));

struct AdamHyper { float lr, b1, b2, eps, wd, bc1, bc2_sqrt; };

__host__ __device__ inline void bias_corrections(float b1, float b2, double step, float &bc1, float &bc2_sqrt)
{
    bc1 = (float)(1.0 - pow((double)b1, step));
    bc2_sqrt = (float)sqrt(1.0 - pow((double)b2, step));
}

__device__ __forceinline__ void adam_update(const AdamHyper &h, float &p, float g, float &m, float &v)
{
    const float gg = g + h.wd * p;
    m = m + (gg - m) * (1.0f - h.b1);
    v = h.b2 * v + (1.0f - h.b2) * gg * gg;
    const float denom = sqrtf(v) / h.bc2_sqrt + h.eps;
    p = p - (h.lr / h.bc1) * (m / denom);
}

// ... 86 lines not shown
                adam_update(h, p[e], g[e], m[e], v[e]);
                if (zero_grad) g[e] = 0.0f;
            }
        }
    }
}

struct RegItems { tn_plane_reg_item it[TN_MULTI_MAX]; };
struct AdamItems { tn_adam_item it[TN_MULTI_MAX]; };

__global__ __launch_bounds__(256) void plane_reg_multi_kernel(RegItems items, float up, double *__restrict__ sums)
{
    const tn_plane_reg_item &t = items.it[blockIdx.y];
    const int W = t.W, H = t.H, C4 = t.C >> 2;
    const int64_t total = (int64_t)H * W * C4;
    const f4 *q = reinterpret_cast<const f4 *>(t.plane);
    f4 *g = reinterpret_cast<f4 *>(t.grad);
    const float cy2 = 2.0f * t.cy, cx2 = 2.0f * t.cx;
    Sums3<float> s;
    for (int64_t i = (int64_t)blockIdx.x * blockDim.x + threadIdx.x; i < total; i += (int64_t)gridDim.x * blockDim.x) {
        const f4 r = reg_texel<true>(q, i, q[i], H, W, C4, cy2, cx2, t.cl1, &s);
        if (g != nullptr) g[i] += r * up;
    }
    if (sums == nullptr) return;
    block_add3(s.y, s.x, s.l, sums + 3 * blockIdx.y);
}

__global__ void adam_gate_kernel(int32_t *__restrict__ step, const float *__restrict__ gate)
{
    if (gate[0] > 0.0f) step[0] += 1;
}

template <bool GATED>
__global__ __launch_bounds__(256) void adam_multi_kernel(AdamItems items, float lr, float b1, float b2, float eps, float wd, float bc1,
                                                         float bc2_sqrt, int zero_grad, const int32_t *__restrict__ step_dev,
                                                         const float *__restrict__ gate, int32_t *__restrict__ nonfinite)
{
    const tn_adam_item &t = items.it[blockIdx.y];
    bool bad = false;
    float *__restrict__ p = t.param; float *__restrict__ g = t.grad; float *__restrict__ m = t.exp_avg; float *__restrict__ v = t.exp_avg_sq;
    const int64_t n = t.n, n4 = (n + 3) / 4;
    if constexpr (GATED) {
        if (!(gate[0] > 0.0f)) {
            if (zero_grad)
                for (int64_t e = (int64_t)blockIdx.x * blockDim.x + threadIdx.x; e < n; e += (int64_t)gridDim.x * blockDim.x) g[e] = 0.0f;
            return;
        }
        bias_corrections(b1, b2, (double)step_dev[0], bc1, bc2_sqrt);
    }
    const AdamHyper h{lr, b1, b2, eps, wd, bc1, bc2_sqrt};
    for (int64_t i = (int64_t)blockIdx.x * blockDim.x + threadIdx.x; i < n4; i += (int64_t)gridDim.x * blockDim.x) {
        if (4 * i + 3 < n) {
            f4 pv = reinterpret_cast<f4 *>(p)[i], gv = reinterpret_cast<f4 *>(g)[i];
            f4 mv = reinterpret_cast<f4 *>(m)[i], vv = reinterpret_cast<f4 *>(v)[i];
            adam_update4(h, pv, gv, mv, vv);
#pragma unroll
            for (int c = 0; c < 4; ++c) bad |= !(fabsf(pv[c]) <= 3.402823466e38f);
            reinterpret_cast<f4 *>(p)[i] = pv; reinterpret_cast<f4 *>(m)[i] = mv; reinterpret_cast<f4 *>(v)[i] = vv;
            if (zero_grad) reinterpret_cast<f4 *>(g)[i] = f4{0.f, 0.f, 0.f, 0.f};
        } else {
            for (int64_t e = 4 * i; e < n; ++e) {
                adam_update(h, p[e], g[e], m[e], v[e]);
                bad |= !(fabsf(p[e]) <= 3.402823466e38f);
                if (zero_grad) g[e] = 0.0f;
            }
        }
    }
    if (nonfinite != nullptr && bad) nonfinite[0] = 1;
}

struct AdamRegItems { tn_adam_reg_item it[TN_MULTI_MAX / 2]; };

__global__ __launch_bounds__(256) void adam_reg_multi_kernel(AdamRegItems items, float lr, float b1, float b2, float eps, float wd, float bc1,
                                                             float bc2_sqrt, int zero_grad, float up, double *__restrict__ sums)
{
    const tn_adam_reg_item &t = items.it[blockIdx.y];
    const AdamHyper h{lr, b1, b2, eps, wd, bc1, bc2_sqrt};
    const float *__restrict__ p = t.param; float *__restrict__ po = t.param_out;
    float *__restrict__ g = t.grad; float *__restrict__ m = t.exp_avg; float *__restrict__ v = t.exp_avg_sq;
    const int64_t n = t.n, n4 = (n + 3) / 4;
    const bool reg = t.H > 0;
    const int W = t.W, H = t.H, C4 = t.C >> 2;
    const float cy2 = 2.0f * t.cy, cx2 = 2.0f * t.cx;
    Sums3<float> s;
    const int64_t own0 = (reg && t.row1 > 0) ? (int64_t)t.row0 * W * C4 : 0, own1 = (reg && t.row1 > 0) ? (int64_t)t.row1 * W * C4 : n4;
    for (int64_t i = (int64_t)blockIdx.x * blockDim.x + threadIdx.x; i < n4; i += (int64_t)gridDim.x * blockDim.x) {
        if (i < own0 || i >= own1) {
            if (zero_grad) reinterpret_cast<f4 *>(g)[i] = f4{0.f, 0.f, 0.f, 0.f};
            continue;
        }
        if (4 * i + 3 < n) {
            const f4 *q = reinterpret_cast<const f4 *>(p);
            f4 pv = q[i], gv = reinterpret_cast<f4 *>(g)[i];
            f4 mv = reinterpret_cast<f4 *>(m)[i], vv = reinterpret_cast<f4 *>(v)[i];
            if (reg) gv += reg_texel<true>(q, i, pv, H, W, C4, cy2, cx2, t.cl1, &s) * up;
            adam_update4(h, pv, gv, mv, vv);
            reinterpret_cast<f4 *>(po)[i] = pv; reinterpret_cast<f4 *>(m)[i] = mv; reinterpret_cast<f4 *>(v)[i] = vv;
            if (zero_grad) reinterpret_cast<f4 *>(g)[i] = f4{0.f, 0.f, 0.f, 0.f};
        } else {
            for (int64_t e = 4 * i; e < n; ++e) {
                float pe = p[e];
                adam_update(h, pe, g[e], m[e], v[e]);
                po[e] = pe;
                if (zero_grad) g[e] = 0.0f;
            }
        }
    }
    if (!reg || sums == nullptr) return;
    block_add3(s.y, s.x, s.l, sums + 3 * t.sum_slot);
}

inline unsigned blocks_for(int64_t n) { return (unsigned)std::min<int64_t>((n + 255) / 256, 256 * 8); }

inline bool plane_shape_ok(int H, int W, int C) { return H > 0 && W > 0 && C > 0 && (C & 3) == 0; }
template <typename... P> inline bool none_null(const P *...p) { return (... && (p != nullptr)); }
template <typename... P> inline bool aligned16(const P *...p) { return ((... | (uintptr_t)p) & 15) == 0; }

#define REQUIRE_ADAM_ITEM(fn, t, ...)                                                                     \
    do {                                                                                                  \
        TN_REQUIRE((t).n >= 0, TN_E_SIZE, fn ": negative size");                                          \
        TN_REQUIRE((t).n == 0 || none_null(__VA_ARGS__), TN_E_NULL, fn ": null pointer");                 \
        TN_REQUIRE(aligned16(__VA_ARGS__), TN_E_ALIGN, fn ": buffers must be 16-byte aligned");           \
    } while (0)

inline int64_t float4s(const tn_plane_reg_item &t) { return (int64_t)t.H * t.W * (t.C / 4); }
template <typename Item> inline int64_t float4s(const Item &t) { return (t.n + 3) / 4; }

template <typename Pack, typename Item, typename Check, typename Launch>
int for_chunks(const Item *items, int n_items, Check check, Launch launch)
{
    constexpr int MAXI = (int)(sizeof(Pack) / sizeof(Item));
    for (int base = 0; base < n_items; base += MAXI) {
        Pack pack;
        const int cnt = std::min(MAXI, n_items - base);
        int64_t largest = 0;
        for (int i = 0; i < cnt; ++i) {
            if (int rc = check(items[base + i])) return rc;
            pack.it[i] = items[base + i];
            largest = std::max(largest, float4s(items[base + i]));
        }
        if (largest == 0) continue;
        if (int rc = launch(pack, dim3(std::min<unsigned>(blocks_for(largest), 1024), (unsigned)cnt), base)) return rc;
    }
    return TN_OK;
}

}

extern "C" int tn_plane_reg_fwd(const float *plane, int H, int W, int C, double *sums, void *stream)
{
    TN_REQUIRE(plane_shape_ok(H, W, C), TN_E_SIZE, "tn_plane_reg_fwd: bad shape (C must be a multiple of 4)");
    TN_REQUIRE(plane && sums, TN_E_NULL, "tn_plane_reg_fwd: null pointer");
    TN_REQUIRE(aligned16(plane), TN_E_ALIGN, "tn_plane_reg_fwd: plane must be 16-byte aligned");
    const int64_t n = (int64_t)H * W * (C / 4);
    plane_reg_fwd_kernel<<<dim3(blocks_for(n)), dim3(256), 0, (hipStream_t)stream>>>(plane, H, W, C / 4, sums);
    return tn::check_launch("plane_reg_fwd_kernel");
}

extern "C" int tn_plane_reg_bwd(const float *plane, int H, int W, int C, float cy, float cx, float cl1, const float *upstream,
                                float *grad, void *stream)
{
    TN_REQUIRE(plane_shape_ok(H, W, C), TN_E_SIZE, "tn_plane_reg_bwd: bad shape (C must be a multiple of 4)");
    TN_REQUIRE(plane && upstream && grad, TN_E_NULL, "tn_plane_reg_bwd: null pointer");
    TN_REQUIRE(aligned16(plane, grad), TN_E_ALIGN, "tn_plane_reg_bwd: buffers must be 16-byte aligned");
    const int64_t n = (int64_t)H * W * (C / 4);
    plane_reg_bwd_kernel<<<dim3(blocks_for(n)), dim3(256), 0, (hipStream_t)stream>>>(plane, H, W, C / 4, cy, cx, cl1, upstream, grad);
    return tn::check_launch("plane_reg_bwd_kernel");
}

extern "C" int tn_adam_step(float *param, float *grad, float *exp_avg, float *exp_avg_sq, int64_t n, float lr, float beta1,
                            float beta2, float eps, float weight_decay, int32_t step, int32_t zero_grad, void *stream)
{
    TN_REQUIRE(n >= 0 && step >= 1, TN_E_SIZE, "tn_adam_step: bad size / step");
    if (n == 0) return TN_OK;
    TN_REQUIRE(param && grad && exp_avg && exp_avg_sq, TN_E_NULL, "tn_adam_step: null pointer");
    TN_REQUIRE(aligned16(param, grad, exp_avg, exp_avg_sq), TN_E_ALIGN, "tn_adam_step: buffers must be 16-byte aligned");
    float bc1, bc2_sqrt;
    bias_corrections(beta1, beta2, (double)step, bc1, bc2_sqrt);
    const int64_t n4 = (n + 3) / 4;
    adam_kernel<<<dim3(blocks_for(n4)), dim3(256), 0, (hipStream_t)stream>>>(param, grad, exp_avg, exp_avg_sq, n4, n, lr, beta1, beta2, eps,
                                                                             weight_decay, bc1, bc2_sqrt, zero_grad);
    return tn::check_launch("adam_kernel");
}

extern "C" int tn_plane_reg_multi(const tn_plane_reg_item *items, int32_t n_items, float upstream, double *sums, void *stream)
{
    TN_REQUIRE(n_items >= 0, TN_E_SIZE, "tn_plane_reg_multi: negative item count");
    TN_REQUIRE(n_items == 0 || items, TN_E_NULL, "tn_plane_reg_multi: null items");
    return for_chunks<RegItems>(
        items, n_items,
        [](const tn_plane_reg_item &t) -> int {
            TN_REQUIRE(plane_shape_ok(t.H, t.W, t.C), TN_E_SIZE, "tn_plane_reg_multi: bad shape (C must be a multiple of 4)");
            TN_REQUIRE(t.plane, TN_E_NULL, "tn_plane_reg_multi: null plane");
            TN_REQUIRE(aligned16(t.plane, t.grad), TN_E_ALIGN, "tn_plane_reg_multi: buffers must be 16-byte aligned");
            return TN_OK;
        },
        [&](const RegItems &pack, dim3 grid, int base) {
            plane_reg_multi_kernel<<<grid, dim3(256), 0, (hipStream_t)stream>>>(pack, upstream, sums ? sums + 3 * base : nullptr);
            return tn::check_launch("plane_reg_multi_kernel");
        });
}

extern "C" int tn_adam_multi(const tn_adam_item *items, int32_t n_items, float lr, float beta1, float beta2, float eps,
                             float weight_decay, int32_t step, int32_t zero_grad, void *stream)
{
    TN_REQUIRE(n_items >= 0 && step >= 1, TN_E_SIZE, "tn_adam_multi: bad item count / step");
    TN_REQUIRE(n_items == 0 || items, TN_E_NULL, "tn_adam_multi: null items");
    float bc1, bc2_sqrt;
    bias_corrections(beta1, beta2, (double)step, bc1, bc2_sqrt);
    return for_chunks<AdamItems>(
        items, n_items,
        [](const tn_adam_item &t) -> int {
            REQUIRE_ADAM_ITEM("tn_adam_multi", t, t.param, t.grad, t.exp_avg, t.exp_avg_sq);
            return TN_OK;
        },
        [&](const AdamItems &pack, dim3 grid, int) {
            adam_multi_kernel<false><<<grid, dim3(256), 0, (hipStream_t)stream>>>(pack, lr, beta1, beta2, eps, weight_decay, bc1, bc2_sqrt,
                                                                                  zero_grad, nullptr, nullptr, nullptr);
            return tn::check_launch("adam_multi_kernel");
        });
}

extern "C" int tn_adam_multi_gated(const tn_adam_item *items, int32_t n_items, float lr, float beta1, float beta2, float eps,
                                   float weight_decay, int32_t *step_dev, const float *gate, int32_t zero_grad, void *stream)
{
    TN_REQUIRE(n_items >= 0, TN_E_SIZE, "tn_adam_multi_gated: bad item count");
    TN_REQUIRE((n_items == 0 || items) && step_dev && gate, TN_E_NULL, "tn_adam_multi_gated: null items / step counter / gate");
    adam_gate_kernel<<<dim3(1), dim3(1), 0, (hipStream_t)stream>>>(step_dev, gate);
    if (int rc = tn::check_launch("adam_gate_kernel")) return rc;
    return for_chunks<AdamItems>(
        items, n_items,
        [](const tn_adam_item &t) -> int {
            REQUIRE_ADAM_ITEM("tn_adam_multi_gated", t, t.param, t.grad, t.exp_avg, t.exp_avg_sq);
            return TN_OK;
        },
        [&](const AdamItems &pack, dim3 grid, int) {
            adam_multi_kernel<true><<<grid, dim3(256), 0, (hipStream_t)stream>>>(pack, lr, beta1, beta2, eps, weight_decay, 1.0f, 1.0f, zero_grad & 1,
                                                                                 step_dev, gate, (zero_grad & 2) ? step_dev + 1 : nullptr);
            return tn::check_launch("adam_multi_kernel<gated>");
        });
}

extern "C" int tn_adam_reg_multi(const tn_adam_reg_item *items, int32_t n_items, float lr, float beta1, float beta2, float eps,
                                 float weight_decay, int32_t step, int32_t zero_grad, float upstream, double *sums, void *stream)
{
    TN_REQUIRE(n_items >= 0 && step >= 1, TN_E_SIZE, "tn_adam_reg_multi: bad item count / step");
    TN_REQUIRE(n_items == 0 || items, TN_E_NULL, "tn_adam_reg_multi: null items");
    float bc1, bc2_sqrt;
    bias_corrections(beta1, beta2, (double)step, bc1, bc2_sqrt);
    return for_chunks<AdamRegItems>(
        items, n_items,
        [&](const tn_adam_reg_item &t) -> int {
            REQUIRE_ADAM_ITEM("tn_adam_reg_multi", t, t.param, t.param_out, t.grad, t.exp_avg, t.exp_avg_sq);
            if (t.H > 0) {
                TN_REQUIRE(t.W > 0 && t.C > 0 && (t.C & 3) == 0 && (int64_t)t.H * t.W * t.C == t.n, TN_E_SIZE,
                           "tn_adam_reg_multi: plane shape must match n (C a multiple of 4)");
                TN_REQUIRE(t.param_out != t.param, TN_E_CONFIG, "tn_adam_reg_multi: a regularised plane needs a separate output buffer");
                TN_REQUIRE(sums == nullptr || t.sum_slot >= 0, TN_E_SIZE, "tn_adam_reg_multi: bad sum slot");
            }
            TN_REQUIRE(t.row1 == 0 ? t.row0 == 0 : (t.H > 0 && t.row0 >= 0 && t.row0 < t.row1 && t.row1 <= t.H), TN_E_SIZE,
                       "tn_adam_reg_multi: rows [row0, row1) must satisfy 0 <= row0 < row1 <= H (row1 == 0, row0 == 0: every row)");
            return TN_OK;
        },
        [&](const AdamRegItems &pack, dim3 grid, int) {
            adam_reg_multi_kernel<<<grid, dim3(256), 0, (hipStream_t)stream>>>(pack, lr, beta1, beta2, eps, weight_decay, bc1, bc2_sqrt, zero_grad,
                                                                               upstream, sums);
            return tn::check_launch("adam_reg_multi_kernel");
        });
}
```

tinynerf_amd/fused.py:

```python
from __future__ import annotations

import ctypes as C
import enum
from dataclasses import dataclass
from typing import Any, Callable, List, Optional, Sequence, Tuple

import torch
from torch.autograd import Function

from . import _lib as L
from .arena import Arena
from .config import CONFIG
from .models import _empty_rows, _hwc, _kplanes_desc, _mlp_desc


ROWS_HANDOFF = CONFIG.rows_handoff


def MATMUL_F16X2() -> bool:
    from . import models
    return ROWS_HANDOFF and models.MATMUL == "f16x2"


FUSE_GATHER = True
# ... 274 lines not shown
    if grad_out is None:
        grad_out = torch.zeros((info.size(0), 3), device=sigma.device)
    g_out = grad_out.contiguous()
    if ctx.gate is not None and not (ctx.gate_in_slot and ctx.stats is not None and ctx.stats.get("upstream_gated")):
        g_out = g_out * (ctx.gate > 0).to(g_out.dtype)
    dev, n, R = sigma.device, sigma.size(0), info.size(0)
    g_rgbs = _alloc(ctx.call.arena, "g_rgbs", (n, 3), dev)
    g_sigma = _alloc(ctx.call.arena, "g_sigma", (n,), dev)
    if not ctx.plan.covered:
        g_rgbs.zero_(); g_sigma.zero_()
    dist = ctx.call.dist
    scale = dist.get("scale") if dist is not None else None
    if dist is None or (scale is None and grad_dist is None):
        L.call("tn_render_rays_bwd", dev, L.ptr(sigma), L.ptr(steps), L.ptr(rgbs), L.ptr(info), L.ptr(bg), L.ptr(weights),
               L.ptr(g_out), L.ptr(g_rgbs), L.ptr(g_sigma), C.c_int64(n), C.c_int64(R))
        return g_rgbs, g_sigma
    g_extra = _alloc(ctx.call.arena, "g_weights_dist", (n,), dev)
    if not ctx.plan.covered:
        g_extra.zero_()
    warp, near, rng = dist["warp"]
    g_dist = None if scale is not None else grad_dist.contiguous()
    L.call("tn_distortion_bwd", dev, L.ptr(weights), L.ptr(dist["t"]), L.ptr(steps), L.ptr(info), C.c_int64(R), C.c_int32(warp),
           C.c_float(near), C.c_float(rng), L.ptr(g_dist), C.c_float(1.0 if scale is None else scale), C.c_void_p(None), L.ptr(g_extra))
    L.call("tn_render_rays_bwd_dw", dev, L.ptr(sigma), L.ptr(steps), L.ptr(rgbs), L.ptr(info), L.ptr(bg), L.ptr(weights),
           L.ptr(g_out), L.ptr(g_extra), L.ptr(g_rgbs), L.ptr(g_sigma), C.c_int64(n), C.c_int64(R))
    return g_rgbs, g_sigma


class _RenderKPlanes(Function):
    @staticmethod
    def forward(ctx: Any, a: _Call, packed: torch.Tensor, info: torch.Tensor, bg: Optional[torch.Tensor], freqs: torch.Tensor,
                *params: torch.Tensor) -> torch.Tensor:
        planes, sig_p, rgb_p = a.split(params)
        dev = L.require_cuda(packed, info, *sig_p, *rgb_p)
        n, R = packed.size(0), info.size(0)
        kdesc, keep = _kplanes_desc(planes)
        F = kdesc.n_scales * kdesc.channels
        feat = _alloc(a.arena, "feat", (n, F), dev)
        table, ray_ids, steps = _ray_aux(packed, info, freqs, a.n_freqs, a.arena, a.hint)
        rdesc, sdesc = _head_descs(sig_p, rgb_p, F, a.n_freqs, freqs, ray_ids, table)
        ws_s, sb = _workspace(sdesc, n, dev, a.arena, "ws_sigma") if a.train else (None, 0)
        ws_r, rb = _workspace(rdesc, n, dev, a.arena, "ws_rgb") if a.train else (None, 0)
        ready = a.hint.get("planes_ready") if (a.hint is not None and a.accumulate) else None
        p = _plan_kplanes(kdesc, keep, rdesc, sdesc, sig_p, rgb_p, a.train, sb, rb, _covered(a.hint, packed, R), ready is not None,
                          a.stats)
        rdesc.flags, sdesc.flags = rdesc.flags | p.flags, sdesc.flags | p.flags
        sigma = _alloc(a.arena, "sigma", (n,), dev)
        rgbs = _alloc(a.arena, "rgbs", (n, 3), dev)
        kp = (C.byref(kdesc), L.ptr(packed), C.c_int64(7))
        if p.fwd in (_KpFwd.INFER_PAIR, _KpFwd.TRAIN_GATHER_PAIR):
            L.call("tn_kplanes_mlp_fwd_pair", dev, *kp, C.byref(rdesc), C.byref(sdesc), L.ptr(table), C.c_int64(n), L.ptr(feat), L.ptr(rgbs),
                   L.ptr(sigma), L.ptr(ws_r), C.c_int64(rb), L.ptr(ws_s), C.c_int64(sb))
        elif p.fwd is _KpFwd.INFER_GATHER_SIGMA:
            L.call("tn_kplanes_mlp_fwd", dev, *kp, C.byref(sdesc), C.c_int64(n), L.ptr(feat), L.ptr(sigma))
        else:
            L.call("tn_kplanes_fwd", dev, *kp, C.c_int64(n), L.ptr(feat))
            if p.fwd is _KpFwd.TRAIN_PAIR:
                L.call("tn_mlp_fwd_stash_pair", dev, C.byref(rdesc), C.byref(sdesc), L.ptr(feat), L.ptr(table), C.c_int64(n), L.ptr(rgbs),
                       L.ptr(sigma), L.ptr(ws_r), C.c_int64(rb), L.ptr(ws_s), C.c_int64(sb))
            else:
                _head_fwd(dev, sdesc, feat, None, n, sigma, ws_s, sb)
        colour = None if p.rays_fwd else lambda w: _head_fwd(dev, rdesc, feat, table, n, rgbs, ws_r, rb, w)
        out, weights = _composite(ctx, a, p.covered, dev, sigma, steps, rgbs, info, bg, colour, rays=p.rays_fwd)
        if p.note_live:
            _note_live_fraction(a.stats, weights)
        ctx.save_for_backward(packed, info, bg, freqs, feat, sigma, steps, table, ray_ids, weights, rgbs, ws_s, ws_r, *params)
        ctx.call, ctx.plan, ctx.planes_ready = a, p, ready
        ctx.param_refs = params if a.accumulate else None
        if a.dist is not None:
            return out, _distortion(ctx, a, dev, weights, steps, info)
        return out

    @staticmethod
    def backward(ctx: Any, grad_out: torch.Tensor, grad_dist: Optional[torch.Tensor] = None):
        packed, info, bg, freqs, feat, sigma, steps, table, ray_ids, weights, rgbs, ws_s, ws_r, *params = ctx.saved_tensors
        a, p = ctx.call, ctx.plan
        planes, sig_p, rgb_p = a.split(params)
        dev, n, F = packed.device, packed.size(0), feat.size(1)
        g_rgbs, g_sigma = _rays_bwd(ctx, grad_out, sigma, steps, rgbs, info, bg, weights, grad_dist)
        grads, returned = _grad_buffers(ctx, params)
        g_planes, k = grads[:a.n_planes], a.n_planes + a.n_sigma
        gw = _grad_ptrs(grads[a.n_planes:k], grads[k:])
        g_feat = _alloc(a.arena, "g_feat", (n, F), dev)
        kdesc, _ = _kplanes_desc(planes)
        gp = ((C.c_void_p * 3) * L.TN_KPLANES_MAX_SCALES)(*[tuple(_hwc(g).data_ptr() for g in g_planes[3 * s:3 * s + 3])
                                                              for s in range(kdesc.n_scales)])
        if p.bwd is _KpBwd.SEPARATE:
            rflags, sflags = L.MLP_STASHED if ws_r is not None else 0, L.MLP_ACCUM_GRAD_X | (L.MLP_STASHED if ws_s is not None else 0)
        else:
            rflags = sflags = L.MLP_STASHED | p.flags
        rdesc, sdesc = _head_descs(sig_p, rgb_p, F, a.n_freqs, freqs, ray_ids, table, rflags, sflags)
        rb, sb = p.rb, p.sb
        if ws_r is None:
            ws_r, rb = _workspace(rdesc, n, dev, a.arena, "ws_rgb")
        if ws_s is None:
            ws_s, sb = _workspace(sdesc, n, dev, a.arena, "ws_sigma")
        base_flags = rdesc.flags
        for phase in (0,) if p.bwd in (_KpBwd.SEPARATE, _KpBwd.PAIR) else (L.MLP_CHAIN_ONLY, L.MLP_WGRAD_ONLY):
            rdesc.flags = base_flags | phase
            if p.bwd is _KpBwd.SCATTER_CHAIN:
                L.call("tn_kplanes_mlp_bwd_pair", dev, C.byref(kdesc), L.ptr(packed), C.c_int64(7), gp, C.byref(rdesc), C.byref(sdesc),
                       L.ptr(feat), L.ptr(table), L.ptr(g_rgbs), L.ptr(g_sigma), C.c_int64(n), *gw, C.c_void_p(None), L.ptr(ws_r),
                       C.c_int64(rb), L.ptr(ws_s), C.c_int64(sb))
            else:
                _heads_bwd(dev, p.bwd is not _KpBwd.SEPARATE, rdesc, sdesc, feat, table, g_rgbs, g_sigma, gw, g_feat, ws_r, rb, ws_s, sb)
                if phase != L.MLP_WGRAD_ONLY:
                    L.call("tn_kplanes_bwd", dev, C.byref(kdesc), L.ptr(packed), C.c_int64(7), C.c_int64(n), L.ptr(g_feat), gp)
            if phase == L.MLP_CHAIN_ONLY and ctx.planes_ready is not None:
                ctx.planes_ready(g_planes)
        return (None, None, None, None, None, *returned)


class _MergeLast(Function):

    @staticmethod
    def forward(ctx: Any, accumulate: bool, pe: int, wc: torch.Tensor, bc: torch.Tensor, ws: torch.Tensor, bs: torch.Tensor,
                w_last: torch.Tensor, b_last: torch.Tensor):
        dev = L.require_cuda(wc, bc, ws, bs, w_last, b_last)
        ps = [t.contiguous() for t in (wc, bc, ws, bs, w_last, b_last)]
        F = w_last.size(0)
        outs = [torch.empty_like(t) for t in ps[:4]]
        heads = (L.MergeHead * 2)()
        for k, col0 in ((0, pe), (1, 0)):
            heads[k].weight, heads[k].bias = ps[2 * k].data_ptr(), ps[2 * k + 1].data_ptr()
            heads[k].rows, heads[k].ld, heads[k].col0 = ps[2 * k].size(0), ps[2 * k].size(1), col0
            heads[k].out_weight, heads[k].out_bias = outs[2 * k].data_ptr(), outs[2 * k + 1].data_ptr()
        L.call("tn_linear_merge_fwd", dev, C.c_int32(2), heads, L.ptr(ps[4]), L.ptr(ps[5]), C.c_int32(F))
        ctx.save_for_backward(*ps)
        ctx.cfg = (accumulate, pe)
        ctx.refs = (wc, bc, ws, bs, w_last, b_last) if accumulate else None
        return tuple(outs)

    @staticmethod
    def backward(ctx: Any, g_wc: torch.Tensor, g_bc: torch.Tensor, g_ws: torch.Tensor, g_bs: torch.Tensor):
        ps = ctx.saved_tensors
        accumulate, pe = ctx.cfg
        dev = ps[0].device
        gm = [g.contiguous() if g is not None else torch.zeros_like(p) for g, p in zip((g_wc, g_bc, g_ws, g_bs), ps[:4])]
        refs = ctx.refs if ctx.refs is not None else [None] * 6
        in_place = [r is not None and r.is_leaf and r.grad is not None and r.grad.is_contiguous() and r.grad.dtype == p.dtype
                    for r, p in zip(refs, ps)]
        grads = [r.grad if ip else torch.zeros_like(p) for r, p, ip in zip(refs, ps, in_place)]
        heads = (L.MergeHead * 2)()
        for k, col0 in ((0, pe), (1, 0)):
            heads[k].weight, heads[k].bias = ps[2 * k].data_ptr(), ps[2 * k + 1].data_ptr()
            heads[k].rows, heads[k].ld, heads[k].col0 = ps[2 * k].size(0), ps[2 * k].size(1), col0
            heads[k].out_weight, heads[k].out_bias = grads[2 * k].data_ptr(), grads[2 * k + 1].data_ptr()
            heads[k].grad_merged_weight, heads[k].grad_merged_bias = gm[2 * k].data_ptr(), gm[2 * k + 1].data_ptr()
        L.call("tn_linear_merge_bwd", dev, C.c_int32(2), heads, L.ptr(ps[4]), L.ptr(ps[5]), C.c_int32(ps[4].size(0)), L.ptr(grads[4]), L.ptr(grads[5]))
        return (None, None, *[None if ip else g for g, ip in zip(grads, in_place)])


class _RenderHeads(Function):

    @staticmethod
    def forward(ctx: Any, a: _Call, feat: torch.Tensor, packed: torch.Tensor, info: torch.Tensor, bg: Optional[torch.Tensor],
                freqs: torch.Tensor, *params: torch.Tensor) -> torch.Tensor:
        _, sig_p, rgb_p = a.split(params)
        feat = feat.contiguous()
        link = a.link if (a.link and a.train and a.link.get("n") == feat.size(0) and a.link.get("y_ptr") == feat.data_ptr()
                          and a.link.get("width") == feat.size(1) and feat.size(1) in (128, 256)) else None
        if link is None and a.link and a.link.get("rows_only"):
            raise RuntimeError("tinynerf_amd: the feature stack left its output as workspace rows only (TN_MLP_ROWS_ONLY) but this render "
                               "node cannot read them")
        dev = L.require_cuda(feat, packed, info, *sig_p, *rgb_p)
        n, R, F = packed.size(0), info.size(0), feat.size(1)
        covered = _covered(a.hint, packed, R)
# ... 140 lines not shown
```

tinynerf_amd/models.py:

```python
from __future__ import annotations

import ctypes as C
import itertools
import os
from typing import Any, Callable, List, Optional, Sequence, Tuple, cast

import torch
from torch.autograd import Function

from . import _lib as L


from .config import CONFIG as _CONFIG
MATMUL = _CONFIG.matmul


def _mlp_desc(params: Sequence[torch.Tensor], in_dim: int, encoding: int, n_freqs: int, out_act: int,
              freqs: Optional[torch.Tensor], flags: int = 0, aux_index: Optional[torch.Tensor] = None, aux_stride: int = 0) -> L.MlpDesc:
    n_layers = len(params) // 2
    if n_layers > L.TN_MLP_MAX_LAYERS:
        raise RuntimeError(f"MLP with {n_layers} layers exceeds the kernel limit {L.TN_MLP_MAX_LAYERS}")
    d = L.MlpDesc()
    d.n_layers = n_layers
    d.in_dim = in_dim
# ... 215 lines not shown
        return out.reshape(*f.shape[:-1], n_out)

    @staticmethod
    def backward(ctx: Any, g: torch.Tensor):
        f2, b2 = ctx.saved_tensors
        n_out, act, f_shape, b_shape = ctx.cfg
        n, Cc = f2.shape
        g = g.reshape(n, n_out).to(torch.float32).contiguous()
        g_f = torch.empty_like(f2)
        g_b = torch.empty_like(b2) if ctx.needs_input_grad[1] else None
        L.call("tn_basis_dot_bwd", f2.device, L.ptr(f2), L.ptr(b2), L.ptr(g), C.c_int64(n), C.c_int32(Cc), C.c_int32(n_out), C.c_int32(act),
               L.ptr(g_f), L.ptr(g_b), C.c_int32(0))
        return g_f.reshape(f_shape) if ctx.needs_input_grad[0] else None, None if g_b is None else g_b.reshape(b_shape), None, None


class TruncatedExponential(Function):

    @staticmethod
    def forward(ctx, x):
        x = x.float().contiguous()
        dev = L.require_cuda(x)
        v = x.reshape(-1, 1)
        one = torch.ones((1, 1), device=dev).expand(v.size(0), 1).contiguous() if v.size(0) else v
        out = torch.empty_like(v)
        L.call("tn_basis_dot_fwd", dev, L.ptr(one), L.ptr(v), C.c_int64(v.size(0)), C.c_int32(1), C.c_int32(1), C.c_int32(L.ACT_EXP), L.ptr(out))
        ctx.save_for_backward(one, v)
        ctx.x_shape = x.shape
        return out.reshape(x.shape)

    @staticmethod
    def backward(ctx, g):
        one, v = ctx.saved_tensors
        g = g.float().contiguous().reshape(-1, 1)
        g_one, g_v = torch.empty_like(one), torch.empty_like(v)
        L.call("tn_basis_dot_bwd", v.device, L.ptr(one), L.ptr(v), L.ptr(g), C.c_int64(v.size(0)), C.c_int32(1), C.c_int32(1),
               C.c_int32(L.ACT_EXP), L.ptr(g_one), L.ptr(g_v), C.c_int32(0))
        return g_v.reshape(ctx.x_shape)


truncated_exp: Callable = TruncatedExponential.apply


class VanillaFeatureMLP(torch.nn.Module):
    def __init__(self, n_freqs: int, hidden_features: int, hidden_layers: int):
        super().__init__()
        in_features = n_freqs * 2 * 3
        self.encoding = PositionalEncoding(n_freqs=n_freqs)
        self.net = MLP(in_features, hidden_features, hidden_layers)
        self.feature_dim = hidden_features
        self.n_freqs = n_freqs

    def forward(self, x):
        return self.net.fused(x, None, L.ENC_POSENC, self.n_freqs, L.ACT_NONE, self.encoding.freqs)


class VanillaOpacityDecoder(torch.nn.Module):
    def __init__(self, feature_dim):
        super().__init__()
        self.net = MLP(feature_dim, 64, 0, 1)
        self.activation = lambda x: truncated_exp(x - 1.)

    def forward(self, features: torch.Tensor) -> torch.Tensor:
        return self.net.fused(features, None, L.ENC_NONE, 0, L.ACT_EXP_M1)


class VanillaColorDecoder(torch.nn.Module):
    def __init__(self, n_freqs: int, in_features: int, hidden_features: int, hidden_layers: int):
        super().__init__()
        self.pe = PositionalEncoding(n_freqs)
        total_features = in_features + n_freqs * 2 * 3 + 3
        self.net = MLP(total_features, hidden_features, hidden_layers, 3)
        self.activation = torch.nn.Sigmoid()
        self.n_freqs = n_freqs

    def forward(self, features: torch.Tensor, rays_d: torch.Tensor) -> torch.Tensor:
        return self.net.fused(features, rays_d, L.ENC_DIR_CAT, self.n_freqs, L.ACT_SIGMOID, self.pe.freqs)


def _hwc(plane: torch.Tensor) -> torch.Tensor:
    p = plane if plane.is_contiguous(memory_format=torch.channels_last) else plane.contiguous(memory_format=torch.channels_last)
    return p.permute(0, 2, 3, 1)[0]


def _kplanes_desc(planes: Sequence[Optional[torch.Tensor]]) -> Tuple[L.KPlanesDesc, List[torch.Tensor]]:
    n_scales = len(planes) // 3
    if n_scales > L.TN_KPLANES_MAX_SCALES:
        raise RuntimeError("too many K-Planes scales for the kernel")
    d = L.KPlanesDesc()
    d.n_scales = n_scales
    d.channels = planes[0].size(1)
    keep = []
    for s in range(n_scales):
        d.height[s] = planes[3 * s].size(2)
        d.width[s] = planes[3 * s].size(3)
        for p in range(3):
            if planes[3 * s + p] is None:
                d.planes[s][p] = None
                continue
            hwc = _hwc(planes[3 * s + p])
            assert hwc.is_contiguous()
            keep.append(hwc)
            d.planes[s][p] = hwc.data_ptr()
    return d, keep


class _KPlanesFeatures(Function):
    @staticmethod
    def forward(ctx: Any, x: torch.Tensor, *planes: torch.Tensor) -> torch.Tensor:
        lead = x.shape[:-1]
        x2 = x.reshape(-1, 3).to(torch.float32)
        if x2.stride(1) != 1 or (x2.size(0) > 1 and x2.stride(0) < 3):
            x2 = x2.contiguous()
        if not x2.is_cuda:
            raise RuntimeError("tinynerf_amd: tensor must be a CUDA (HIP) tensor -- there is no CPU path")
        dev = x2.device
        desc, keep = _kplanes_desc(planes)
        n = x2.size(0)
        stride = x2.stride(0) if n > 1 else 3
        feat = torch.empty((n, desc.n_scales * desc.channels), device=dev)
        L.call("tn_kplanes_fwd", dev, C.byref(desc), L.ptr(x2), C.c_int64(stride), C.c_int64(n), L.ptr(feat))
        ctx.present = [p is not None for p in planes]
        ctx.save_for_backward(x2, *[p if p is not None else x2.new_empty(0) for p in planes])
        return feat.reshape(*lead, feat.size(-1))

    @staticmethod
    def backward(ctx: Any, grad_feat: torch.Tensor):
        x2, *planes = ctx.saved_tensors
        dev = x2.device
        desc, keep = _kplanes_desc([p if ctx.present[i] else None for i, p in enumerate(planes)])
        n = x2.size(0)
        stride = x2.stride(0) if n > 1 else 3
        g = grad_feat.reshape(n, -1).to(torch.float32).contiguous()
        planes = [p if ctx.present[i] else None for i, p in enumerate(planes)]
        grads = [None if p is None else torch.zeros_like(p, memory_format=torch.channels_last) for p in planes]
        gp = ((C.c_void_p * 3) * L.TN_KPLANES_MAX_SCALES)()
        for s in range(desc.n_scales):
            for p in range(3):
                gp[s][p] = None if grads[3 * s + p] is None else _hwc(grads[3 * s + p]).data_ptr()
        L.call("tn_kplanes_bwd", dev, C.byref(desc), L.ptr(x2), C.c_int64(stride), C.c_int64(n), L.ptr(g), gp)
        return (None, *grads)


class _PlaneRegulariser(Function):

    @staticmethod
    def forward(ctx: Any, w_tv: float, w_l1: float, accumulate: bool, *planes: torch.Tensor) -> torch.Tensor:
        dev = planes[0].device
        ctx.refs = planes if accumulate else None
        if not planes[0].is_cuda:
            raise RuntimeError("tinynerf_amd: tensor must be a CUDA (HIP) tensor -- there is no CPU path")
        n = len(planes)
        sums = torch.zeros((n, 3), dtype=torch.float64, device=dev)
        coef = torch.empty((n, 3), dtype=torch.float64)
        for i, p in enumerate(planes):
            _, Cc, H, W = p.shape
            L.call("tn_plane_reg_fwd", dev, L.ptr(_hwc(p)), C.c_int(H), C.c_int(W), C.c_int(Cc),
                   C.c_void_p(sums.data_ptr() + i * 24))
            coef[i, 0] = w_tv / (n * Cc * max(H - 1, 1) * W)
            coef[i, 1] = w_tv / (n * Cc * H * max(W - 1, 1))
            coef[i, 2] = w_l1 / (n * Cc * H * W)
        ctx.coef = coef
        ctx.save_for_backward(*planes)
        return (sums * coef.to(dev)).sum().to(torch.float32)

    @staticmethod
    def backward(ctx: Any, grad_out: torch.Tensor):
        planes = ctx.saved_tensors
        dev = planes[0].device
        up = grad_out.reshape(1).to(torch.float32).contiguous()
        grads = []
        for i, p in enumerate(planes):
            _, Cc, H, W = p.shape
            ref = ctx.refs[i] if ctx.refs is not None else None
            in_place = ref is not None and ref.grad is not None and ref.grad.stride() == p.stride()
            g = ref.grad if in_place else torch.zeros_like(p, memory_format=torch.channels_last)
            cy, cx, cl1 = (float(v) for v in ctx.coef[i])
            L.call("tn_plane_reg_bwd", dev, L.ptr(_hwc(p)), C.c_int(H), C.c_int(W), C.c_int(Cc), C.c_float(cy), C.c_float(cx),
                   C.c_float(cl1), L.ptr(up), L.ptr(_hwc(g)))
            grads.append(None if in_place else g)
        return (None, None, None, *grads)


class KPlanesFeaturePlane(torch.nn.Module):
    def __init__(
        self,
# ... 340 lines not shown
```

tinynerf_amd/optim.py:

```python
from __future__ import annotations

import ctypes as C
from typing import Iterable, Tuple

import torch

from . import _lib as L


class FusedAdam(torch.optim.Optimizer):
    def __init__(self, params: Iterable[torch.Tensor], lr: float = 1e-3, betas: Tuple[float, float] = (0.9, 0.999),
                 eps: float = 1e-8, weight_decay: float = 0.0, zero_grad_in_step: bool = False):
        defaults = dict(lr=lr, betas=betas, eps=eps, weight_decay=weight_decay)
        super().__init__(params, defaults)
        self.zero_grad_in_step = zero_grad_in_step
        self._gated_count = {}
        self._gated_params = {}

    @torch.no_grad()
    def step(self, closure=None, plane_reg=None, gate=None, only=None):
        loss = closure() if closure is not None else None
        reg = {id(p): (slot, *rest) for slot, (p, *rest) in enumerate(plane_reg["spec"])} if plane_reg is not None else {}
        for group in self.param_groups:
            for (t, dev, with_reg), tensors in self._collect(group, reg, gate, only).items():
                common = (C.c_float(group["lr"]), *map(C.c_float, group["betas"]), C.c_float(group["eps"]), C.c_float(group["weight_decay"]),
                          C.c_int32(t), C.c_int32(1 if self.zero_grad_in_step else 0))
                if with_reg:
                    self._launch_reg(dev, tensors, common, reg, plane_reg)
                else:
                    self._launch_plain(dev, tensors, common, gate)
        return loss

    def _state(self, p, shadow: bool = False):
        st = self.state[p]
        if "exp_avg" not in st:
            st.setdefault("step", 0)
            st["exp_avg"] = torch.zeros_like(p, memory_format=torch.preserve_format)
            st["exp_avg_sq"] = torch.zeros_like(p, memory_format=torch.preserve_format)
        if shadow and "shadow" not in st:
            st["shadow"] = torch.empty_like(p, memory_format=torch.preserve_format)
        return st

    def _collect(self, group, reg, gate, only):
        by_step = {}
        for p in group["params"]:
            g = p.grad
            if g is None:
                continue
            if not p.is_cuda:
                raise RuntimeError("tinynerf_amd.FusedAdam: parameters must be CUDA (HIP) tensors -- there is no CPU path")
            if only is not None and (id(p) in reg) != (only == "reg"):
                continue
            st = self._state(p)
            st["step"] += 1
            m, v = st["exp_avg"], st["exp_avg_sq"]
            same = g.stride() == p.stride() == m.stride() == v.stride()
            dense = (p.is_contiguous() or (p.dim() == 4 and p.is_contiguous(memory_format=torch.channels_last))
                     or (p.dim() == 5 and p.is_contiguous(memory_format=torch.channels_last_3d)))
            if not (same and dense and p.dtype == torch.float32):
                raise RuntimeError("tinynerf_amd.FusedAdam: parameter, gradient and state must be dense fp32 with equal strides")
            by_step.setdefault((st["step"] if (gate is None or id(p) in reg) else -1, p.device, id(p) in reg), []).append((p, g, m, v))
        return by_step

    def _launch_plain(self, dev, tensors, common, gate):
        items = (L.AdamItem * len(tensors))()
        for it, (p, g, m, v) in zip(items, tensors):
            it.param, it.grad, it.exp_avg, it.exp_avg_sq, it.n = p.data_ptr(), g.data_ptr(), m.data_ptr(), v.data_ptr(), p.numel()
        if gate is None:
            return L.call("tn_adam_multi", dev, items, C.c_int32(len(tensors)), *common)
        if self._gated_count.get(dev) is None:
            self._gated_count[dev] = torch.tensor([min(self.state[p]["step"] for p, _, _, _ in tensors) - 1, 0], dtype=torch.int32, device=dev)
        self._gated_params[dev] = [p for p, _, _, _ in tensors]
        L.call("tn_adam_multi_gated", dev, items, C.c_int32(len(tensors)), *common[:5], L.ptr(self._gated_count[dev]),
               L.ptr(gate), C.c_int32(common[6].value | 2))

    def _launch_reg(self, dev, tensors, common, reg, plane_reg):
        items = (L.AdamRegItem * len(tensors))()
        for it, (p, g, m, v) in zip(items, tensors):
            slot, H, W, Cc, cy, cx, cl = reg[id(p)]
            if (Cc, H, W) != tuple(p.shape[1:]) or not p.is_contiguous(memory_format=torch.channels_last):
                raise RuntimeError("tinynerf_amd.FusedAdam: plane_reg expects channels_last [1,C,H,W] planes")
            it.param, it.param_out, it.grad = p.data_ptr(), self._state(p, shadow=True)["shadow"].data_ptr(), g.data_ptr()
            it.exp_avg, it.exp_avg_sq, it.n = m.data_ptr(), v.data_ptr(), p.numel()
            it.H, it.W, it.C, it.sum_slot, it.cy, it.cx, it.cl1 = H, W, Cc, slot, cy, cx, cl
            it.row0, it.row1 = (plane_reg.get("rows") or {}).get(id(p), (0, 0))
        L.call("tn_adam_reg_multi", dev, items, C.c_int32(len(tensors)), *common, C.c_float(plane_reg["upstream"]), L.ptr(plane_reg.get("sums")))
        for p, _, _, _ in tensors:
            st = self.state[p]
            p.data, st["shadow"] = st["shadow"], p.data

    def sync_step_counts(self) -> None:
        for dev, cnt in self._gated_count.items():
            if cnt is None:
                continue
            c = int(cnt[0].item())
            for p in self._gated_params.get(dev, []):
                if p in self.state:
                    self.state[p]["step"] = c

    def nonfinite_flag(self, device) -> "torch.Tensor | None":
        for dev, cnt in self._gated_count.items():
            if cnt is not None and dev.type == torch.device(device).type and (torch.device(device).index in (None, dev.index)):
                return cnt[1:2]
        return None

    partial_state_reason = None

    def preallocate(self, params, shadow: bool = False):
        for p in params:
            self._state(p, shadow)

    def state_dict(self):
        if self.partial_state_reason:
            raise RuntimeError("tinynerf_amd.FusedAdam.state_dict(): " + self.partial_state_reason)
        self.sync_step_counts()
        return super().state_dict()

    def load_state_dict(self, state_dict):
        super().load_state_dict(state_dict)
        self._gated_count, self._gated_params = {}, {}
```

tinynerf_amd/run.py:

```python
from __future__ import annotations

import os
import ctypes as C
import math
from dataclasses import dataclass, field
from typing import Callable, Dict, List, Optional, Tuple

import torch

from . import _lib as L
from .core import (ContractionAABB, ContractionMip360, NerfRenderer, OccupancyGrid, RayMarcherAABB,
                   RayMarcherUnbounded, RayProvider, distortion_warp)
from .optim import FusedAdam
from .models import (CobafaFeatureField, HashGridFeatureField, KPlanesFeatureField, VanillaColorDecoder, VanillaFeatureMLP,
                     VanillaOpacityDecoder)


def psnr(x: torch.Tensor, y: torch.Tensor) -> torch.Tensor:
    return -10. * torch.log10(torch.mean((x - y) ** 2))


def ssim(x: torch.Tensor, y: torch.Tensor, data_range: float = 1.0, return_map: bool = False):
    if x.dim() != 3 or x.shape != y.shape:
        raise RuntimeError("ssim: x and y must be [H, W, C] images of the same shape")
    if x.dtype != torch.float32 or y.dtype != torch.float32:
        raise RuntimeError("ssim: x and y must be float32")
    dev = L.require_cuda(x, y)
    H, W, Cn = x.shape
    if H < 11 or W < 11 or not 1 <= Cn <= 4:
        raise RuntimeError("ssim: needs H >= 11, W >= 11 (one whole 11 x 11 window) and 1 <= C <= 4")
    if not float(data_range) > 0.0:
        raise ValueError("ssim: data_range must be > 0")
    nbytes = C.c_int64(0)
    L.call_plain("tn_ssim_workspace_bytes", C.c_int64(H), C.c_int64(W), C.c_int32(Cn), C.byref(nbytes))
    workspace = torch.empty(nbytes.value, dtype=torch.uint8, device=dev)
    mean = torch.empty((), dtype=torch.float32, device=dev)
    smap = torch.empty((H - 10, W - 10, Cn), dtype=torch.float32, device=dev) if return_map else None
    L.call("tn_ssim", dev, L.ptr(x), L.ptr(y), C.c_int64(H), C.c_int64(W), C.c_int32(Cn), C.c_float(data_range), L.ptr(smap),
           L.ptr(workspace), C.c_int64(nbytes.value), L.ptr(mean))
    return (mean, smap) if return_map else mean


_image_ssim = ssim


from .config import CONFIG as _CONFIG
ADAM_OVERLAP = _CONFIG.adam_overlap
SIDE_PLAN = _CONFIG.side_plan


@dataclass
class TrainConfig:
    method: str = "kplanes"
    scene_type: str = "aabb"
    batch_size: int = 1024
    n_samples: int = 1024
    scene_scale: float = 1.0
    grad_scale: float = 2.0 ** 10
    seed: int = 0
    occupancy_res: int = 128
    deterministic: bool = False
    kplanes_resolutions: Tuple[int, ...] = (128, 256, 512)
    shard: int = 1
    host_shuffle: bool = False
    sharded_optimizer: Optional[bool] = None
    distortion_weight: float = 0.0
    hashgrid_log2_table_size: int = 19


def jitter_seed(seed: int, batch_no: int, rank: int = 0) -> int:
    import hashlib
    h = int.from_bytes(hashlib.blake2b(b"tinynerf-jitter:%d:%d" % (seed, batch_no), digest_size=8).digest(), "little")
    return (h & (2 ** 62 - 1)) * 2 + 1 + rank


def refresh_seed(seed: int, train_step: int) -> int:
    return (seed * 7919 + 104729 * (train_step + 1)) % (2 ** 62)


def build_renderer(cfg: TrainConfig, bg_color: Optional[torch.Tensor], device: torch.device):
    if cfg.method == "vanilla":
        feature_module: torch.nn.Module = VanillaFeatureMLP(10, 256, 8)
    elif cfg.method == "kplanes":
        feature_module = KPlanesFeatureField(32, cfg.kplanes_resolutions)
    elif cfg.method == "cobafa":
        feature_module = CobafaFeatureField(
            basis_res=torch.linspace(32., 128, 6).int().tolist(), coef_res=64,
            freqs=torch.linspace(2., 8., 6).tolist(), channels=[8, 8, 8, 4, 4, 4], mlp_hidden_dim=128)
    elif cfg.method == "hashgrid":
        feature_module = HashGridFeatureField(16, 2, cfg.hashgrid_log2_table_size, 16, 2048)
    else:
        raise NotImplementedError(f"Unknown method {cfg.method}.")
    dim = feature_module.feature_dim
    sigma_decoder = VanillaOpacityDecoder(dim)
    rgb_decoder = VanillaColorDecoder(8, dim, 64, 3)
    if cfg.scene_type == "unbounded":
        ray_marcher = RayMarcherUnbounded(cfg.n_samples, 0.1, 1e5, uniform_range=cfg.scene_scale)
        contraction = ContractionMip360(order=float("inf"))
    elif cfg.scene_type == "aabb":
        aabb = torch.tensor([[-1.5, -1.5, -1.5], [1.5, 1.5, 1.5]]).to(device)
        ray_marcher = RayMarcherAABB(aabb, cfg.n_samples, 0.1)
        contraction = ContractionAABB(aabb)
    else:
        raise NotImplementedError(f"Unknown scene type {cfg.scene_type}.")
    occupancy_grid = OccupancyGrid(size=cfg.occupancy_res, step_size=ray_marcher.step_size, threshold=0.01,
                                   decay=0.01 ** (1 / 16)).to(device)
    ray_provider = RayProvider(occupancy_grid=occupancy_grid, contraction=contraction, ray_marcher=ray_marcher)
    renderer = NerfRenderer(feature_module, sigma_decoder, rgb_decoder, bg_color=bg_color).to(device)
    return renderer, occupancy_grid, ray_provider


class Trainer:

    def __init__(self, cfg: TrainConfig, rays_o: Optional[torch.Tensor], rays_d: Optional[torch.Tensor], rgbs: Optional[torch.Tensor],
                 bg_color: Optional[torch.Tensor], device: torch.device, rank: int = 0, world_size: int = 1, *, ray_source=None):
        self.cfg, self.device, self.rank, self.world = cfg, device, rank, world_size
        self.rays_o, self.rays_d, self.rgbs = rays_o, rays_d, rgbs
        self.ray_source = ray_source
        if ray_source is not None:
            if rays_o is not None or rays_d is not None or rgbs is not None:
                raise ValueError("Trainer: either the ray tables or ray_source, not both")
            if ray_source.rgb is None:
                raise ValueError("Trainer: ray_source has no colours to train on")
            if ray_source.device != torch.device(device) and ray_source.device.index is not None and torch.device(device).index is not None:
                raise ValueError("Trainer: ray_source lives on another device")
        self._source_rays = 0 if ray_source is None else len(range(rank, ray_source.n_rays, world_size)) if world_size > 1 else ray_source.n_rays
        with torch.random.fork_rng(devices=[]):
            torch.manual_seed(cfg.seed)
            self.renderer, self.occupancy_grid, self.ray_provider = build_renderer(cfg, bg_color, device)
        bs_ratio = 4096 / cfg.batch_size
        self.steps = int(2048 * bs_ratio)
        self.occupancy_grid_updates = int(16 * bs_ratio)
        self.tv_reg_alpha, self.l1_reg_alpha = 0.0001, 0.
        if cfg.shard < 1 or cfg.batch_size % cfg.shard:
            raise ValueError(f"TrainConfig.shard = {cfg.shard} must divide batch_size = {cfg.batch_size}")
        self.loader_batch = cfg.batch_size // cfg.shard
        self.target_sample_size = self.loader_batch * cfg.n_samples
        if cfg.distortion_weight < 0:
            raise ValueError(f"TrainConfig.distortion_weight = {cfg.distortion_weight} must be >= 0")
        if cfg.distortion_weight > 0 and world_size > 1:
            raise ValueError("TrainConfig.distortion_weight > 0 is single-GPU for now: the mean over ALL ranks' rays is not exchanged yet")
        if cfg.method == "hashgrid" and world_size > 1:
            raise ValueError("TrainConfig.method = 'hashgrid' is single-GPU for now: the table's gradient (49 MB at the default size) "
                             "has no exchange of its own yet")
        self.renderer.distortion_warp = distortion_warp(self.ray_provider.ray_marcher)
        params = list(self.renderer.parameters())
        for p in params:
            p.grad = torch.zeros_like(p)
        self._flat, self._flat_used, self._flat_ids = Trainer._flat_small_grads(params, device) if world_size > 1 else (None, 0, set())
        self.renderer.accumulate_into_grad = True
        self.renderer.reuse_buffers = True
        from .arena import Arena
        from .models import MLP
        self.scratch = Arena()
        for i, m in enumerate(mod for mod in self.renderer.feature_module.modules() if isinstance(mod, MLP)):
            m.__dict__["scratch"] = (self.scratch, f"mlp_ws{i}", {}, True, {})
        if isinstance(self.renderer.feature_module, (CobafaFeatureField, HashGridFeatureField)):
            self.renderer.feature_module.__dict__["accumulate_into_grad"] = True
        self._arena: Dict[str, torch.Tensor] = {}
        self._arena_grown = 0
        self.optimizer = FusedAdam(params, lr=1e-2, eps=1e-15, weight_decay=1e-5, zero_grad_in_step=True)
        if isinstance(self.renderer.feature_module, KPlanesFeatureField):
            self.optimizer.preallocate(self.renderer.feature_module.plane_tensors(), shadow=True)
        self.scheduler = torch.optim.lr_scheduler.MultiStepLR(
            self.optimizer, milestones=[self.steps // 2, self.steps * 3 // 4, self.steps * 5 // 6, self.steps * 9 // 10],
            gamma=0.33)
        self.train_step = 0
        self._cursor = 0
        self._perm: Optional[torch.Tensor] = None
        self._perm_pos = 0
        self._carry = torch.empty(0, dtype=torch.int32, device=device)
        self._k_guess = 8
        self._gen = torch.Generator(device=device)
        self._gen.manual_seed(cfg.seed * 1000003 + rank + 1)
        self._host_gen = torch.Generator().manual_seed(cfg.seed * 1000003 + rank + 1)
        self._batch_no = 0
        self.last: Dict[str, float] = {}
        self.grad_hook: Optional[Callable[["Trainer"], None]] = None
        self._early: Dict[int, object] = {}
        self._pending: Optional[dict] = None
        self._plane_of: Dict[int, int] = {}
        self._reduce_rows: Optional[List[Tuple[int, int]]] = None
        self._reduce_rows_prev: Optional[List[Tuple[int, int]]] = None
        if world_size > 1 and isinstance(self.renderer.feature_module, KPlanesFeatureField):
            self._plane_of = {id(p): i for i, p in enumerate(self.renderer.feature_module.plane_tensors())}
        self._sharded = bool(cfg.sharded_optimizer and world_size > 1 and self._plane_of and
                             all(p.size(2) % world_size == 0 for p in self.renderer.feature_module.plane_tensors()))
        self._gathers: List[object] = []
        if self._sharded:
            self.optimizer.partial_state_reason = Trainer._PARTIAL
        self._plan_host: Optional[torch.Tensor] = None
        self._info_turn = 0
        self._side: Optional[torch.cuda.Stream] = None
        self._side2: Optional[torch.cuda.Stream] = None
        self._gate_ring = torch.zeros(256, device=device)
        self._gate_tick = 0
        self._acc_ring = torch.zeros((64, 1 + 32 * 3 + 1), dtype=torch.float64, device=device)
        self._batch_t: Optional[torch.Tensor] = None
        self._acc_tick = 0
        self.prefetch = True
        self._graveyard: List[torch.Tensor] = []

    @property
    def n_rays(self) -> int:
        return self._source_rays if self.ray_source is not None else self.rays_o.size(0)

    def __del__(self):
        side = getattr(self, "_side", None)
        if side is not None:
            try:
                side.synchronize()
            except Exception:
                pass

    def _on_stream(self, *tensors: Optional[torch.Tensor]) -> None:
        cur = torch.cuda.current_stream(self.device)
        for t in tensors:
            if t is not None and t.is_cuda and t.numel():
                t.record_stream(cur)

    def _buf(self, name: str, shape, dtype) -> torch.Tensor:
        numel = 1
        for d in shape:
            numel *= int(d)
        t = self._arena.get(name)
        if t is None or t.numel() < numel:
            if t is not None:
                self._graveyard.append(t)
            t = torch.empty(int(numel * 1.25) + 64, dtype=dtype, device=self.device)
            self._arena[name] = t
            self._arena_grown += 1
        self._on_stream(t)
        return t[:numel].view(*shape)

    def _epoch_block(self, m: int) -> torch.Tensor:
        n_rays = self.n_rays
        self._on_stream(self._perm, self._carry)
        while self._carry.numel() + (0 if self._perm is None else self._perm.numel() - self._perm_pos) < m:
            if self._perm is not None:
                self._graveyard += [self._perm, self._carry]
                self._carry = torch.cat([self._carry, self._perm[self._perm_pos:]])
            if self.cfg.host_shuffle:
                self._perm = torch.randperm(n_rays, generator=self._host_gen, dtype=torch.int32).to(self.device)
            else:
                self._perm = torch.randperm(n_rays, device=self.device, generator=self._gen, dtype=torch.int32)
            self._perm_pos = 0
        c = self._carry.numel()
        if c == 0:
            return self._perm[self._perm_pos:self._perm_pos + m]
        return torch.cat([self._carry[:m], self._perm[self._perm_pos:self._perm_pos + max(0, m - c)]])

    def _advance(self, r: int) -> None:
        c = self._carry.numel()
        if r >= c:
            self._carry = self._carry[:0]
            self._perm_pos += r - c
        else:
            self._carry = self._carry[r:]

    @torch.no_grad()
    def _launch_plan(self, n_b: Optional[int] = None) -> None:
        cfg, dev = self.cfg, self.device
        B, S = self.loader_batch, cfg.n_samples
        n_chunks = (S + 63) // 64
        n_b = n_b or min(4096, max(2, int(self._k_guess * 1.12) + 3))
        R_all = n_b * B
        if cfg.deterministic:
            idx = ((self._cursor + torch.arange(R_all, device=dev)) % self.n_rays).to(torch.int32)
        else:
            idx = self._epoch_block(R_all)
        self._info_turn ^= 1
        o = self._buf(f"cand_o{self._info_turn}", (R_all, 3), torch.float32)
        d = self._buf(f"cand_d{self._info_turn}", (R_all, 3), torch.float32)
        rgb = self._buf(f"cand_rgb{self._info_turn}", (R_all, 3), torch.float32)
        if self.ray_source is not None:
            self.ray_source.gather(idx, o, d, rgb, first=self.rank if self.world > 1 else 0, stride=self.world if self.world > 1 else 1)
        else:
            L.call("tn_gather_rays", dev, L.ptr(self.rays_o), L.ptr(self.rays_d), L.ptr(self.rgbs), L.ptr(idx), C.c_int64(R_all), L.ptr(o), L.ptr(d),
                   L.ptr(rgb))
        desc = self.ray_provider._desc(dev, not cfg.deterministic, None)
        desc.seed = jitter_seed(cfg.seed, self._batch_no, self.rank)
        maskbits = self._buf("maskbits", (R_all, n_chunks), torch.int64)
        counts = self._buf("counts", (R_all,), torch.int32)
        plan = self._buf("plan", (4,), torch.int32)
        info = self._buf(f"info{self._info_turn}", (R_all, 2), torch.int32)
        L.call("tn_sample_mask", dev, C.byref(desc), L.ptr(o), L.ptr(d), C.c_int64(R_all), L.ptr(maskbits), L.ptr(counts))
        L.call("tn_batch_plan_scan", dev, L.ptr(counts), C.c_int64(R_all), C.c_int32(B), C.c_int64(self.target_sample_size), L.ptr(plan),
               L.ptr(info))
        if self._plan_host is None:
            self._plan_host = torch.empty(4, dtype=torch.int32, pin_memory=True)
            self._plan_event = torch.cuda.Event()
        self._plan_host.copy_(plan, non_blocking=True)
        self._plan_event.record(torch.cuda.current_stream(dev))
        self._pending = dict(n_b=n_b, idx=idx, o=o, d=d, rgb=rgb, desc=desc, maskbits=maskbits, counts=counts, info=info)

    @torch.no_grad()
    def build_batch(self) -> Tuple[torch.Tensor, torch.Tensor, torch.Tensor, int]:
        dev, B = self.device, self.loader_batch
        while True:
            if self._pending is None:
                self._launch_plan()
            pend, self._pending = self._pending, None
            self._plan_event.synchronize()
            del self._graveyard[:]
            self._on_stream(*(pend[k] for k in ("idx", "o", "d", "rgb", "maskbits", "counts", "info")))
            k, n, R, tripped = self._plan_host.tolist()
            if tripped or pend["n_b"] >= 4096:
                break
            self._k_guess = pend["n_b"] * 2
        self._k_guess = k
        self._batch_no += 1
        self.last_plan_seed = int(pend["desc"].seed)
        self._cursor = (self._cursor + R) % self.n_rays
        if not self.cfg.deterministic:
            self._advance(R)
        info = pend["info"][:R]
        packed = self._buf("packed", (n, 7), torch.float32)
        ray_ids = self._buf("ray_ids", (n,), torch.int32)
        steps = self._buf("steps", (n,), torch.float32)
        t = None
        if self.cfg.distortion_weight > 0:
            t = self._buf("t_values", (n,), torch.float32)
            L.call("tn_sample_pack_t", dev, C.byref(pend["desc"]), L.ptr(pend["o"]), L.ptr(pend["d"]), C.c_int64(R), L.ptr(pend["maskbits"]),
                   L.ptr(info), C.c_void_p(None), L.ptr(packed), L.ptr(ray_ids), L.ptr(steps), L.ptr(t), C.c_int64(n))
        else:
            L.call("tn_sample_pack", dev, C.byref(pend["desc"]), L.ptr(pend["o"]), L.ptr(pend["d"]), C.c_int64(R), L.ptr(pend["maskbits"]),
                   L.ptr(info), C.c_void_p(None), L.ptr(packed), L.ptr(ray_ids), L.ptr(steps), C.c_int64(n))
        slot = self._gate_tick % self._gate_ring.numel()
        self._gate_tick += 1
        if slot == 0 and self._gate_tick > 1:
            self._gate_ring.zero_()
        self.renderer._batch_aux = {"key": (packed.data_ptr(), n, R), "ray_ids": ray_ids, "steps": steps, "dirs": pend["d"][:R],
                                    "planes_ready": self._planes_ready if self.world > 1 else (self._planes_adam_early if ADAM_OVERLAP else None),
                                    "gate": self._gate_ring[slot:slot + 1]}
        self._batch_t = t
        return packed, info, pend["rgb"][:R], k

    def sigma_fn(self, t: torch.Tensor) -> torch.Tensor:
        return self.renderer.sigma_decoder(self.renderer.feature_module(t))

    def step(self) -> Dict[str, float]:
        packed, info, target, k = self.build_batch()
        return self.step_on_batch(packed, info, target, k, t=self._batch_t)

    def step_on_batch(self, packed: torch.Tensor, info: torch.Tensor, target: torch.Tensor, k: int = 0,
                      prefetch: Optional[bool] = None, t: Optional[torch.Tensor] = None) -> Dict[str, float]:
        cfg = self.cfg
        if cfg.distortion_weight > 0 and t is None:
            raise ValueError("TrainConfig.distortion_weight > 0: step_on_batch needs t, the ray parameter of every packed sample")
        self.renderer.train()
        if self.train_step % self.occupancy_grid_updates == 0:
            jit = None
            if cfg.deterministic:
                r = cfg.occupancy_res
                jit = torch.full((r, r, r, 3), 0.5, device=self.device)
            self.occupancy_grid.update(self.sigma_fn, jitters=jit, seed=refresh_seed(cfg.seed, self.train_step))
            self._refresh_reduce_rows()
        ray_count = None
        if self.world > 1:
            ray_count = torch.full((1,), float(info.size(0)), device=self.device)
            ray_count_done = torch.distributed.all_reduce(ray_count, async_op=True)
        acc, dist_side = None, None
        if cfg.distortion_weight > 0:
            acc = self._next_acc_row()
            dist_side = {"sum": acc[-1:], "scale": cfg.distortion_weight * cfg.grad_scale / max(info.size(0), 1)}
            stats0 = self.renderer.__dict__.setdefault("_stats", {})
            stats0["dist_train"] = dist_side
            try:
                rendered, _ = self.renderer.render_with_distortion(packed, info, t)
            finally:
                stats0.pop("dist_train", None)
            if not dist_side.get("taken"):
                raise RuntimeError("tinynerf_amd: distortion_weight > 0 needs a renderer the fused render nodes take (fused.supports)")
        else:
            rendered = self.renderer(packed, info)
        gate = getattr(self.renderer, "_stats", {}).get("gate")
        gate_done = None
        if self.world > 1 and gate is not None:
            gate_done = torch.distributed.all_reduce(gate, async_op=True)
        if self.prefetch if prefetch is None else prefetch:
            if not SIDE_PLAN:
                self._launch_plan()
            else:
                if self._side is None:
                    self._side = torch.cuda.Stream(self.device)
                self._side.wait_stream(torch.cuda.current_stream(self.device))
                with torch.cuda.stream(self._side):
                    self._launch_plan()
        R = rendered.size(0)
        if acc is None:
            acc = self._next_acc_row()
        grad = self._buf("grad_rendered", (R, 3), torch.float32)
        if self.world == 1:
            inv, inv_dev = 1.0 / (3.0 * R), None
        else:
            ray_count_done.wait()
            if gate_done is not None:
                gate_done.wait()
            inv, inv_dev = 1.0, (1.0 / (3.0 * ray_count)).float()
        stats = getattr(self.renderer, "_stats", {})
        if gate is not None and stats.get("pre_gated"):
            stats["upstream_gated"] = True
            L.call("tn_mse_grad_gated", self.device, L.ptr(rendered.detach()), L.ptr(target), C.c_int64(3 * R), C.c_float(2.0 * cfg.grad_scale * inv),
                   L.ptr(inv_dev), L.ptr(gate), L.ptr(grad), L.ptr(acc))
        else:
            L.call("tn_mse_grad", self.device, L.ptr(rendered.detach()), L.ptr(target), C.c_int64(3 * R), C.c_float(2.0 * cfg.grad_scale * inv),
                   L.ptr(inv_dev), L.ptr(grad), L.ptr(acc))
        self._early_adam = None
        if ADAM_OVERLAP and self.world == 1 and cfg.method == "kplanes" and self.grad_hook is None:
            spec0, _ = self.renderer.feature_module.regulariser_spec(self.tv_reg_alpha, self.l1_reg_alpha)
            self._early_adam = {"plane_reg": {"spec": spec0, "upstream": cfg.grad_scale, "sums": acc[1:-1]}, "gate": gate, "done": False}
        early_done = False
        try:
            rendered.backward(grad)
            early_done = bool(self._early_adam is not None and self._early_adam.get("done"))
        finally:
            stats["upstream_gated"] = False
            if not early_done:
                self._early_adam = None if self._early_adam is None or not self._early_adam.get("done") else self._early_adam
        reg_coef, plane_reg = None, None
        if cfg.method == "kplanes":
            spec, reg_coef = self.renderer.feature_module.regulariser_spec(self.tv_reg_alpha, self.l1_reg_alpha)
            plane_reg = {"spec": spec, "upstream": cfg.grad_scale, "sums": acc[1:-1]}
            if self._sharded:
                plane_reg["rows"] = {id(p): Trainer._own_rows(p.size(2), self.rank, self.world) for p in self.renderer.feature_module.plane_tensors()}
        self._loss_parts = (acc, inv, inv_dev, reg_coef)
        self._loss_dist = cfg.distortion_weight / max(R, 1) if dist_side is not None else None
        if self.world > 1:
            self.all_reduce_grads(gate)
        if self.grad_hook is not None:
            self.grad_hook(self)
        if self._early_adam is not None and self._early_adam.get("done"):
            self.optimizer.step(plane_reg=plane_reg, gate=gate, only="rest")
            torch.cuda.current_stream(self.device).wait_stream(self._side2)
        else:
            self.optimizer.step(plane_reg=plane_reg, gate=gate)
        if self._sharded:
            works = []
            for p in self.renderer.feature_module.plane_tensors():
                works += Trainer._all_gather_rows(p.data, self.rank, self.world)
            for w in works:
                w.wait()
        self.scheduler.step()
        self.train_step += 1
        self.last = {"n_samples": float(packed.size(0)), "n_rays": float(info.size(0)), "k": float(k)}
        return self.last

    def _next_acc_row(self) -> torch.Tensor:
        row = self._acc_tick % self._acc_ring.size(0)
        self._acc_tick += 1
        if row == 0:
            self._acc_ring.zero_()
        return self._acc_ring[row]

    def global_ray_count(self, local_rays: int, gate: Optional[torch.Tensor] = None):
        if self.world == 1:
            return float(local_rays)
        both = torch.full((2,), float(local_rays), device=self.device)
        if gate is not None:
            both[1:2] = (gate > 0).float()
        torch.distributed.all_reduce(both)
        if gate is not None:
            gate.copy_(both[1:2])
        return both[0]

    def global_mse(self, rendered: torch.Tensor, target: torch.Tensor) -> torch.Tensor:
        return ((rendered - target) ** 2).sum() / (3.0 * Trainer.global_ray_count(self, rendered.size(0)))

    def loss_device(self) -> torch.Tensor:
        acc, inv, inv_dev, reg_coef = self._loss_parts
        v = acc[0] * inv * (inv_dev[0].double() if inv_dev is not None else 1.0)
        if reg_coef is not None:
            v = v + (acc[1:1 + reg_coef.numel()] * reg_coef.reshape(-1)).sum() / (1 if getattr(self, "_sharded", False) else self.world)
        if getattr(self, "_loss_dist", None) is not None:
            v = v + acc[-1] * self._loss_dist
        v = v.float().reshape(1).clone()
        if self.world > 1:
            torch.distributed.all_reduce(v)
        bad = self.optimizer.nonfinite_flag(self.device) if hasattr(self.optimizer, "nonfinite_flag") else None
        if bad is not None:
            v = torch.where(bad != 0, torch.full_like(v, float("nan")), v)
        return v

    def loss_value(self) -> float:
        return float(self.loss_device().item())

    @staticmethod
    def _dense_view(g: torch.Tensor) -> Optional[torch.Tensor]:
        if g.is_contiguous():
            return g
        order = sorted(range(g.dim()), key=lambda d: (-g.stride(d), -g.size(d)))
        v = g.permute(order)
        return v if v.is_contiguous() else None

    @torch.no_grad()
    def _refresh_reduce_rows(self) -> None:
        if not self._plane_of:
            return
        g = self.occupancy_grid
        occ = g.grid > g.threshold
        lo_hi = []
        for keep in (2, 1, 0):
            line = occ.amax(dim=tuple(d for d in range(3) if d != keep)).to(torch.int32)
            idx = torch.arange(line.numel(), device=line.device, dtype=torch.int32)
            big = line.numel() + 1
            lo_hi += [torch.where(line > 0, idx, torch.full_like(idx, big)).amin(), torch.where(line > 0, idx, torch.full_like(idx, -1)).amax()]
        vals = torch.stack(lo_hi).tolist()
        dims = (g.grid.size(2), g.grid.size(1), g.grid.size(0))
        rows: List[Tuple[int, int]] = []
        for i, p in enumerate(self.renderer.feature_module.plane_tensors()):
            axis = (1, 2, 2)[i % 3]
            i0, i1, S, Hp = vals[2 * axis], vals[2 * axis + 1], dims[axis], p.size(2)
            if i1 < 0:
                rows.append((0, 0))
                continue
            v_lo = max(-1.0, -1.0 + 2.0 * (i0 - 1) / max(S - 1, 1)); v_hi = min(1.0, -1.0 + 2.0 * (i1 + 1) / max(S - 1, 1))
            r0 = int(math.floor((v_lo + 1.0) * 0.5 * (Hp - 1))) - 1
            r1 = int(math.floor((v_hi + 1.0) * 0.5 * (Hp - 1))) + 3
            rows.append((max(0, r0), min(Hp, r1)))
        prev = self._reduce_rows if self._reduce_rows is not None else [(0, p.size(2)) for p in self.renderer.feature_module.plane_tensors()]
        self._reduce_rows_prev, self._reduce_rows = prev, rows

    def _reduce_view(self, g: torch.Tensor, plane: Optional[int]) -> Optional[torch.Tensor]:
        flat = Trainer._dense_view(g) if g.numel() >= (1 << 18) else None
        if flat is None or plane is None or self._reduce_rows is None or flat.dim() != 4 or not g.is_contiguous(memory_format=torch.channels_last):
            return flat
        (a0, a1), (b0, b1) = self._reduce_rows[plane], self._reduce_rows_prev[plane]
        r0, r1 = (min(a0, b0), max(a1, b1)) if a1 > a0 and b1 > b0 else ((a0, a1) if a1 > a0 else (b0, b1))
        return flat[:, r0:r1] if r1 > r0 else flat[:, :0]

    @staticmethod
    def _all_reduce_many(views):
        views = [v for v in views if v.numel()]
        if not views:
            return None
        if len(views) == 1:
            return torch.distributed.all_reduce(views[0], async_op=True)
        if torch.distributed.get_backend() != "nccl" and views[0].is_cuda:
            works = [torch.distributed.all_reduce(v, async_op=True) for v in views]

            class _All:
                def wait(self_inner):
                    for w in works:
                        w.wait()
            return _All()
        coalesced = getattr(torch.distributed, "all_reduce_coalesced", None)
        if coalesced is None:
            works = [torch.distributed.all_reduce(v, async_op=True) for v in views]

            class _Each:
                def wait(self_inner):
                    for w in works:
                        w.wait()
            return _Each()
        import warnings
        with warnings.catch_warnings():
            warnings.filterwarnings("ignore", message=".*all_reduce_coalesced.*", category=FutureWarning)
            warnings.filterwarnings("ignore", message=".*all_reduce_coalesced.*", category=UserWarning)
            warnings.filterwarnings("ignore", message=".*all_reduce_coalesced.*", category=DeprecationWarning)
            return coalesced(views, async_op=True)

    @staticmethod
    def _own_rows(H: int, rank: int, world: int) -> Tuple[int, int]:
        return H * rank // world, H * (rank + 1) // world

    @staticmethod
    def _reduce_scatter_rows(g: torch.Tensor, rank: int, world: int):
        flat = Trainer._dense_view(g).view(-1)
        chunk = flat.numel() // world
        own = flat[rank * chunk:(rank + 1) * chunk]
        if torch.distributed.get_backend() == "nccl" or not flat.is_cuda:
            return torch.distributed.reduce_scatter_tensor(own, flat, async_op=True)
        return torch.distributed.all_reduce(flat, async_op=True)

    @staticmethod
    def _all_gather_rows(p: torch.Tensor, rank: int, world: int):
        flat = Trainer._dense_view(p).view(-1)
        chunk = flat.numel() // world
        if torch.distributed.get_backend() == "nccl" or not flat.is_cuda:
            return [torch.distributed.all_gather_into_tensor(flat, flat[rank * chunk:(rank + 1) * chunk], async_op=True)]
        return [torch.distributed.broadcast(flat[r * chunk:(r + 1) * chunk], src=r, async_op=True) for r in range(world)]

    def optimizer_state_dict(self) -> dict:
        if getattr(self, "_sharded", False):
            works = []
            for p in self.renderer.feature_module.plane_tensors():
                st = self.optimizer.state.get(p, {})
                for key in ("exp_avg", "exp_avg_sq"):
                    if key in st:
                        works += Trainer._all_gather_rows(st[key], self.rank, self.world)
            for w in works:
                w.wait()
        self.optimizer.partial_state_reason = None
        try:
            return self.optimizer.state_dict()
        finally:
            if getattr(self, "_sharded", False):
                self.optimizer.partial_state_reason = Trainer._PARTIAL

    _PARTIAL = ("sharded optimizer pass: the planes' Adam moments are valid on the owning rank's rows only -- use "
                "Trainer.optimizer_state_dict(), which gathers them")

    def _planes_adam_early(self, grads) -> None:
        pend = getattr(self, "_early_adam", None)
# ... 198 lines not shown
```

Baseline: 350.3 million.

## Scatter K-Planes gradients into compact occupancy-derived boxes instead of full planes

```diff
diff --git a/include/tinynerf_hip.h b/include/tinynerf_hip.h
--- a/include/tinynerf_hip.h
+++ b/include/tinynerf_hip.h
@@ -184,12 +184,17 @@
 int tn_mlp_lean_supported(const tn_mlp_desc *desc, const tn_mlp_desc *partner);
 
 #define TN_KPLANES_MAX_SCALES 4
+typedef struct tn_kplanes_box {
+    int32_t x0, y0, x1, y1, pitch, reserved;
+} tn_kplanes_box;
 typedef struct tn_kplanes_desc {
     int32_t n_scales;
     int32_t channels;
     int32_t height[TN_KPLANES_MAX_SCALES];
     int32_t width[TN_KPLANES_MAX_SCALES];
     const float *planes[TN_KPLANES_MAX_SCALES][3];
+    tn_kplanes_box grad_box[TN_KPLANES_MAX_SCALES][3];
+    int32_t *grad_box_flag;
 } tn_kplanes_desc;
 
 int tn_kplanes_fwd(const tn_kplanes_desc *desc, const float *x, int64_t x_stride, int64_t n,
@@ -331,6 +336,7 @@
     int32_t H, W, C, sum_slot;
     float cy, cx, cl1;
     int32_t row0, row1, reserved;
+    int32_t box_x0, box_y0, box_x1, box_y1, box_pitch, reserved2;
 } tn_adam_reg_item;
 int tn_adam_reg_multi(const tn_adam_reg_item *items, int32_t n_items, float lr, float beta1, float beta2, float eps,
                       float weight_decay, int32_t step, int32_t zero_grad, float upstream, double *sums, void *stream);
diff --git a/tinynerf_amd/_lib.py b/tinynerf_amd/_lib.py
--- a/tinynerf_amd/_lib.py
+++ b/tinynerf_amd/_lib.py
@@ -53,11 +53,16 @@
     ]
 
 
+class KPlanesBox(C.Structure):
+    _fields_ = [("x0", C.c_int32), ("y0", C.c_int32), ("x1", C.c_int32), ("y1", C.c_int32), ("pitch", C.c_int32), ("reserved", C.c_int32)]
+
+
 class KPlanesDesc(C.Structure):
     _fields_ = [
         ("n_scales", C.c_int32), ("channels", C.c_int32),
         ("height", C.c_int32 * TN_KPLANES_MAX_SCALES), ("width", C.c_int32 * TN_KPLANES_MAX_SCALES),
         ("planes", (C.c_void_p * 3) * TN_KPLANES_MAX_SCALES),
+        ("grad_box", (KPlanesBox * 3) * TN_KPLANES_MAX_SCALES), ("grad_box_flag", C.c_void_p),
     ]
 
 
@@ -91,7 +96,9 @@
 class AdamRegItem(C.Structure):
     _fields_ = [("param", C.c_void_p), ("param_out", C.c_void_p), ("grad", C.c_void_p), ("exp_avg", C.c_void_p), ("exp_avg_sq", C.c_void_p),
                 ("n", C.c_int64), ("H", C.c_int32), ("W", C.c_int32), ("C", C.c_int32), ("sum_slot", C.c_int32),
-                ("cy", C.c_float), ("cx", C.c_float), ("cl1", C.c_float), ("row0", C.c_int32), ("row1", C.c_int32), ("reserved", C.c_int32)]
+                ("cy", C.c_float), ("cx", C.c_float), ("cl1", C.c_float), ("row0", C.c_int32), ("row1", C.c_int32), ("reserved", C.c_int32),
+                ("box_x0", C.c_int32), ("box_y0", C.c_int32), ("box_x1", C.c_int32), ("box_y1", C.c_int32), ("box_pitch", C.c_int32),
+                ("reserved2", C.c_int32)]
 
 
 class CobafaDesc(C.Structure):
diff --git a/tinynerf_amd/config.py b/tinynerf_amd/config.py
--- a/tinynerf_amd/config.py
+++ b/tinynerf_amd/config.py
@@ -67,3 +67,5 @@
 
 
 CONFIG = Config.from_env()
+GRAD_SCRATCH = os.environ.get("TN_GRAD_SCRATCH", "1") != "0"
+GRAD_SCRATCH_LOG = os.environ.get("TN_GRAD_SCRATCH", "1") == "2"
diff --git a/tinynerf_amd/csrc/kplanes.hip b/tinynerf_amd/csrc/kplanes.hip
--- a/tinynerf_amd/csrc/kplanes.hip
+++ b/tinynerf_amd/csrc/kplanes.hip
@@ -10,6 +10,8 @@
     int H[TN_KPLANES_MAX_SCALES], W[TN_KPLANES_MAX_SCALES];
     const float *planes[TN_KPLANES_MAX_SCALES][3];
     float *grads[TN_KPLANES_MAX_SCALES][3];
+    tn::KpGradBox box[TN_KPLANES_MAX_SCALES][3];
+    int *dropped;
 };
 
 template <int NV>
@@ -50,6 +52,15 @@
                                                           int64_t n, const float *__restrict__ grad_feat)
 {
     __shared__ __attribute__((aligned(16))) float lds[4 * tn::KP_WAVE_LDS];
+    __shared__ __attribute__((aligned(16))) int boxes[TN_KPLANES_MAX_SCALES * 3 * tn::KP_BOX_INTS];
+    if (threadIdx.x == 0) {
+#pragma unroll
+        for (int s = 0; s < TN_KPLANES_MAX_SCALES; ++s)
+#pragma unroll
+            for (int p = 0; p < 3; ++p)
+                if (s < a.n_scales) tn::kp_store_box(boxes + (3 * s + p) * tn::KP_BOX_INTS, a.box[s][p]);
+    }
+    __syncthreads();
     const int lane = tn::lane_id(), j = lane & 31, h = lane >> 5;
     float *wave_lds = lds + (threadIdx.x >> 6) * tn::KP_WAVE_LDS;
     const int64_t n_tiles = (n + 31) >> 5;
@@ -67,7 +78,7 @@
                              : f32x4k{0.f, 0.f, 0.f, 0.f};
             const float *const pl[3] = {a.planes[s][0], a.planes[s][1], a.planes[s][2]};
             float *const gr[3] = {a.grads[s][0], a.grads[s][1], a.grads[s][2]};
-            tn::kp_scatter_scale<NV, 4>(pl, gr, a.H[s], a.W[s], C, xs, valid, g, h * (C / 2), wave_lds, j, h);
+            tn::kp_scatter_scale<NV, 4>(pl, gr, boxes + 3 * s * tn::KP_BOX_INTS, a.dropped, a.H[s], a.W[s], C, xs, valid, g, h * (C / 2), wave_lds, j, h);
         }
     }
 }
@@ -93,6 +104,13 @@
             }
         }
     }
+    a.dropped = nullptr;
+    if (grads) {
+        a.dropped = d->grad_box_flag;
+        for (int s = 0; s < d->n_scales; ++s)
+            for (int p = 0; p < 3; ++p)
+                if (int rc = tn::kp_grad_box(d->grad_box[s][p], a.H[s], a.W[s], d->grad_box_flag, a.box[s][p])) return rc;
+    }
     return TN_OK;
 }
 
diff --git a/tinynerf_amd/csrc/kplanes_device.h b/tinynerf_amd/csrc/kplanes_device.h
--- a/tinynerf_amd/csrc/kplanes_device.h
+++ b/tinynerf_amd/csrc/kplanes_device.h
@@ -10,6 +10,8 @@
     float w[4];
     int cell;
 };
+
+__device__ __forceinline__ int cell_row_shift(int W) { return 32 - __builtin_clz(W + 3); }
 
 __device__ __forceinline__ PlaneTaps plane_taps(float u, float v, int H, int W, int C) {
     PlaneTaps t;
@@ -31,7 +33,7 @@
     t.off[2] = (bx0 && by1) ? (y1 * W + x0) * C : -1;
     t.off[3] = (bx1 && by1) ? (y1 * W + x1) * C : -1;
     const float cx = fminf(fmaxf(x0f, -2.0f), (float)W + 1.0f), cy = fminf(fmaxf(y0f, -2.0f), (float)H + 1.0f);
-    t.cell = ((int)cy + 2) * (W + 4) + (int)cx + 2;
+    t.cell = (((int)cy + 2) << cell_row_shift(W)) + (int)cx + 2;
     return t;
 }
 
diff --git a/tinynerf_amd/csrc/kplanes_scatter.h b/tinynerf_amd/csrc/kplanes_scatter.h
--- a/tinynerf_amd/csrc/kplanes_scatter.h
+++ b/tinynerf_amd/csrc/kplanes_scatter.h
@@ -9,8 +9,31 @@
 constexpr int KP_GS = 36;
 constexpr int KP_WAVE_LDS = 32 * KP_GS + 2 * 4 * 32;
 
+struct KpGradBox { int x0, y0, nx, ny, pitch; };
+constexpr int KP_BOX_INTS = 8;
+
+__device__ __forceinline__ void kp_store_box(int *dst, const KpGradBox &b)
+{
+    dst[0] = b.x0; dst[1] = b.y0; dst[2] = b.nx; dst[3] = b.ny; dst[4] = b.pitch;
+}
+
+inline int kp_grad_box(const tn_kplanes_box &b, int H, int W, const int32_t *flag, KpGradBox &out)
+{
+    if (b.pitch == 0) {
+        TN_REQUIRE(b.x0 == 0 && b.y0 == 0 && b.x1 == 0 && b.y1 == 0, TN_E_CONFIG, "kplanes: a gradient box without a pitch");
+        out = KpGradBox{0, 0, W, H, W};
+        return TN_OK;
+    }
+    TN_REQUIRE(b.x0 >= 0 && b.x0 <= b.x1 && b.x1 <= W && b.y0 >= 0 && b.y0 <= b.y1 && b.y1 <= H && b.pitch >= b.x1 - b.x0 && b.pitch <= W,
+               TN_E_SIZE, "kplanes: gradient box must satisfy 0 <= x0 <= x1 <= W, 0 <= y0 <= y1 <= H, x1 - x0 <= pitch <= W");
+    TN_REQUIRE(flag, TN_E_NULL, "kplanes: a gradient box needs grad_box_flag");
+    out = KpGradBox{b.x0, b.y0, b.x1 - b.x0, b.y1 - b.y0, b.pitch};
+    return TN_OK;
+}
+
 template <int NV, int CS>
-__device__ __forceinline__ void kp_scatter_scale(const float *const (&planes)[3], float *const (&grads)[3], int H, int W, int C,
+__device__ __forceinline__ void kp_scatter_scale(const float *const (&planes)[3], float *const (&grads)[3], const int *box,
+                                                 int *__restrict__ dropped, int H, int W, int C,
                                                  const float (&xs)[3], bool valid, const f32x4k (&g)[NV], int c0,
                                                  float *__restrict__ wave_lds, int j, int h)
 {
@@ -48,18 +71,29 @@
                                      : (p == 1 ? g[q] * val[0][q] * val[2][q] : g[q] * (val[0][q] * val[1][q]));
             *reinterpret_cast<f32x4k *>(tileG + j * KP_GS + c0 + CS * q) = gp;
         }
+        const int row_shift = cell_row_shift(W), rowlen = 1 << row_shift;
+        const int cy = t[p].cell >> row_shift, cx = t[p].cell & (rowlen - 1);
+        const int4 b4 = *reinterpret_cast<const int4 *>(box + KP_BOX_INTS * p);
+        const int bx0 = __builtin_amdgcn_readfirstlane(b4.x), by0 = __builtin_amdgcn_readfirstlane(b4.y);
+        const unsigned bnx = (unsigned)__builtin_amdgcn_readfirstlane(b4.z), bny = (unsigned)__builtin_amdgcn_readfirstlane(b4.w);
+        const unsigned pitch = (unsigned)__builtin_amdgcn_readfirstlane(box[KP_BOX_INTS * p + 4]);
+        const int ty = cy - 2 + h;
+        const bool row_in = valid && (unsigned)(ty - by0) < bny, row_in_plane = valid && (unsigned)ty < (unsigned)H;
+        const unsigned row_base = (unsigned)(ty - by0) * pitch - (unsigned)bx0;
+        bool outside = false;
 #pragma unroll
         for (int k = 0; k < 2; ++k) {
-            const int o = h ? t[p].off[2 + k] : t[p].off[0 + k];
             const float w = h ? t[p].w[2 + k] : t[p].w[0 + k];
-            const bool live = valid && o >= 0;
-            tileO[(2 * h + k) * 32 + j] = live ? 4 * o : 0;
+            const int tx = cx - 2 + k;
+            const bool live = row_in && (unsigned)(tx - bx0) < bnx;
+            outside |= row_in_plane && (unsigned)tx < (unsigned)W && !live;
+            tileO[(2 * h + k) * 32 + j] = live ? (int)((row_base + (unsigned)tx) * (unsigned)(4 * C)) : 0;
             tileW[(2 * h + k) * 32 + j] = live ? w : 0.0f;
         }
+        if (outside) *dropped = 1;
         const int cell = valid ? t[p].cell : -1 - j;
         const int next_cell = __shfl_down(cell, 1, 64);
         const int dcell = (j < 31) ? next_cell - cell : 0x40000000;
-        const int rowlen = W + 4;
         const unsigned run_end = (unsigned)__ballot(dcell != 0);
         const unsigned mv_xp = (unsigned)__ballot(dcell == 1), mv_xm = (unsigned)__ballot(dcell == -1);
         const unsigned mv_yp = (unsigned)__ballot(dcell == rowlen), mv_ym = (unsigned)__ballot(dcell == -rowlen);
diff --git a/tinynerf_amd/csrc/mlp_bwd2.hip b/tinynerf_amd/csrc/mlp_bwd2.hip
--- a/tinynerf_amd/csrc/mlp_bwd2.hip
+++ b/tinynerf_amd/csrc/mlp_bwd2.hip
@@ -48,7 +48,10 @@
     float *grads[3][3];
     const float *coords;
     int64_t coord_stride;
+    tn::KpGradBox box[3][3];
+    int *dropped;
 };
+struct KpBwdCall { KpBwd kp; const tn_kplanes_desc *kd; };
 
 template <int H>
 __device__ __forceinline__ void first_dgrad(const float *__restrict__ Wf, int sf, int out, const float (&gp)[4],
@@ -85,6 +88,15 @@
     stage_weights(a, lds);
     const float *ldsb = lds + a.lds_floats;
     if constexpr (PAIR || G0B) stage_weights(pr.b, lds + a.lds_floats);
+    if constexpr (KP) {
+        if (threadIdx.x == 0) {
+            int *boxes = reinterpret_cast<int *>(lds + a.lds_floats + pr.b.lds_floats + WPB * tn::KP_WAVE_LDS);
+#pragma unroll
+            for (int sc = 0; sc < 3; ++sc)
+#pragma unroll
+                for (int p = 0; p < 3; ++p) tn::kp_store_box(boxes + (3 * sc + p) * tn::KP_BOX_INTS, kp.box[sc][p]);
+        }
+    }
     __syncthreads();
     if constexpr (STASHED && NH > 1) {
         constexpr int sl = H + 4;
@@ -390,6 +402,7 @@
                 const float *cr = kp.coords + (valid ? row : 0) * kp.coord_stride;
                 const float xs[3] = {cr[0], cr[1], cr[2]};
                 float *wave_lds = lds + a.lds_floats + pr.b.lds_floats + wave * tn::KP_WAVE_LDS;
+                const int *boxes = reinterpret_cast<const int *>(lds + a.lds_floats + pr.b.lds_floats + WPB * tn::KP_WAVE_LDS);
 #pragma unroll
                 for (int sc = 0; sc < 3; ++sc) {
                     tn::f32x4k g4[4];
@@ -397,7 +410,7 @@
                     for (int q = 0; q < 4; ++q) g4[q] = tn::f32x4k{gacc[sc][4 * q], gacc[sc][4 * q + 1], gacc[sc][4 * q + 2], gacc[sc][4 * q + 3]};
                     const float *const pl[3] = {kp.planes[sc][0], kp.planes[sc][1], kp.planes[sc][2]};
                     float *const gr[3] = {kp.grads[sc][0], kp.grads[sc][1], kp.grads[sc][2]};
-                    tn::kp_scatter_scale<4, 8>(pl, gr, kp.H[sc], kp.W[sc], 32, xs, valid, g4, 4 * h, wave_lds, j, h);
+                    tn::kp_scatter_scale<4, 8>(pl, gr, boxes + 3 * sc * tn::KP_BOX_INTS, kp.dropped, kp.H[sc], kp.W[sc], 32, xs, valid, g4, 4 * h, wave_lds, j, h);
                     TN_PTB(3 + sc)
                 }
             }
@@ -774,7 +787,7 @@
 
 template <int H, int NH>
 int launch_chain(const MlpArgs &a, const float *x, const float *aux, const float *gy, int64_t n, float *gx, float *stash, bool stashed,
-                 hipStream_t s, const PairArgs *pair = nullptr, const KpBwd *kpb = nullptr)
+                 hipStream_t s, const PairArgs *pair = nullptr, const KpBwdCall *kpb = nullptr)
 {
     if (kpb) {
         if constexpr (H == 64 && NH == 4) {
@@ -783,10 +796,15 @@
             const MlpArgs ac = compact_first_layer(a);
             PairArgs pr = *pair;
             pr.b = compact_first_layer(pair->b);
-            const size_t lds_bytes = ((size_t)ac.lds_floats + (size_t)pr.b.lds_floats + (size_t)WPK * tn::KP_WAVE_LDS) * 4;
+            const size_t lds_bytes = ((size_t)ac.lds_floats + (size_t)pr.b.lds_floats + (size_t)WPK * tn::KP_WAVE_LDS + 9 * tn::KP_BOX_INTS) * 4;
             if (lds_bytes > (size_t)LDS_LIMIT_BYTES) return tn::fail(TN_E_CONFIG, "mlp_bwd: weights + scatter tiles do not fit LDS");
+            KpBwd kp = kpb->kp;
+            kp.dropped = kpb->kd->grad_box_flag;
+            for (int sc = 0; sc < 3; ++sc)
+                for (int p = 0; p < 3; ++p)
+                    if (int rc = tn::kp_grad_box(kpb->kd->grad_box[sc][p], kp.H[sc], kp.W[sc], kp.dropped, kp.box[sc][p])) return rc;
             return launch(mlp_chain_kernel<H, NH, WPK, true, false, true, true>, WPK, lds_bytes, grid_blocks(n, WPK, 256), s,
-                          "mlp_chain_kernel(kplanes)", ac, x, aux, gy, n, gx, stash, pr, *kpb);
+                          "mlp_chain_kernel(kplanes)", ac, x, aux, gy, n, gx, stash, pr, kp);
         } else return tn::fail(TN_E_CONFIG, "mlp_bwd: fused scatter is built for the 5-layer colour head");
     }
     size_t lds_bytes = (size_t)a.lds_floats * 4;
@@ -810,7 +828,7 @@
 }
 
 int chain(const MlpArgs &a, const float *x, const float *aux, const float *gy, int64_t n, float *gx, float *stash, bool stashed,
-          hipStream_t s, const PairArgs *pair = nullptr, const KpBwd *kpb = nullptr)
+          hipStream_t s, const PairArgs *pair = nullptr, const KpBwdCall *kpb = nullptr)
 {
     return a.n_layers == 2 ? launch_chain<64, 1>(a, x, aux, gy, n, gx, stash, stashed, s, pair, kpb)
                            : launch_chain<64, 4>(a, x, aux, gy, n, gx, stash, stashed, s, pair, kpb);
@@ -950,7 +968,7 @@
                            const float *grad_y, const float *partner_grad_y, int64_t n, float *const *grad_weights,
                            float *const *grad_biases, float *const *partner_grad_weights, float *const *partner_grad_biases,
                            float *grad_x, void *workspace, int64_t workspace_bytes, void *partner_workspace,
-                           int64_t partner_workspace_bytes, void *stream, const KpBwd *kpb)
+                           int64_t partner_workspace_bytes, void *stream, const KpBwdCall *kpb)
 {
     TN_REQUIRE(desc && partner, TN_E_NULL, "tn_mlp_bwd_pair: null descriptor");
     TN_REQUIRE((desc->flags & TN_MLP_STASHED) && (partner->flags & TN_MLP_STASHED), TN_E_CONFIG,
@@ -1062,11 +1080,13 @@
     TN_REQUIRE(coord_stride >= 3, TN_E_SIZE, "tn_kplanes_mlp_bwd_pair: bad coordinate stride");
     if (n == 0) return TN_OK;
     TN_REQUIRE(coords, TN_E_NULL, "tn_kplanes_mlp_bwd_pair: null coordinates");
-    KpBwd kp;
+    KpBwdCall kc;
+    KpBwd &kp = kc.kp;
+    kc.kd = kd;
     if (int rc = kp_planes(kd, coords, coord_stride, kp)) return rc;
     for (int s = 0; s < 3; ++s)
         for (int p = 0; p < 3; ++p) kp.grads[s][p] = grad_planes[s][p];
     return bwd_pair_common(desc, partner, feat, aux, grad_y, partner_grad_y, n, grad_weights, grad_biases, partner_grad_weights,
                            partner_grad_biases, grad_feat, workspace, workspace_bytes, partner_workspace, partner_workspace_bytes, stream,
-                           &kp);
-}
+                           &kc);
+}
diff --git a/tinynerf_amd/csrc/planes_reg.hip b/tinynerf_amd/csrc/planes_reg.hip
--- a/tinynerf_amd/csrc/planes_reg.hip
+++ b/tinynerf_amd/csrc/planes_reg.hip
@@ -192,6 +192,8 @@
     const bool reg = t.H > 0;
     const int W = t.W, H = t.H, C4 = t.C >> 2;
     const float cy2 = 2.0f * t.cy, cx2 = 2.0f * t.cx;
+    const bool boxed = reg && t.box_pitch > 0;
+    const unsigned box_nx = (unsigned)(t.box_x1 - t.box_x0), box_ny = (unsigned)(t.box_y1 - t.box_y0);
     Sums3<float> s;
     const int64_t own0 = (reg && t.row1 > 0) ? (int64_t)t.row0 * W * C4 : 0, own1 = (reg && t.row1 > 0) ? (int64_t)t.row1 * W * C4 : n4;
     for (int64_t i = (int64_t)blockIdx.x * blockDim.x + threadIdx.x; i < n4; i += (int64_t)gridDim.x * blockDim.x) {
@@ -201,12 +203,18 @@
         }
         if (4 * i + 3 < n) {
             const f4 *q = reinterpret_cast<const f4 *>(p);
-            f4 pv = q[i], gv = reinterpret_cast<f4 *>(g)[i];
+            int64_t gi = i;
+            if (boxed) {
+                const int64_t texel = i / C4;
+                const unsigned bx = (unsigned)((int)(texel % W) - t.box_x0), by = (unsigned)((int)(texel / W) - t.box_y0);
+                gi = (bx < box_nx && by < box_ny) ? ((int64_t)by * t.box_pitch + bx) * C4 + i % C4 : -1;
+            }
+            f4 pv = q[i], gv = gi >= 0 ? reinterpret_cast<f4 *>(g)[gi] : f4{0.f, 0.f, 0.f, 0.f};
             f4 mv = reinterpret_cast<f4 *>(m)[i], vv = reinterpret_cast<f4 *>(v)[i];
             if (reg) gv += reg_texel<true>(q, i, pv, H, W, C4, cy2, cx2, t.cl1, &s) * up;
             adam_update4(h, pv, gv, mv, vv);
             reinterpret_cast<f4 *>(po)[i] = pv; reinterpret_cast<f4 *>(m)[i] = mv; reinterpret_cast<f4 *>(v)[i] = vv;
-            if (zero_grad) reinterpret_cast<f4 *>(g)[i] = f4{0.f, 0.f, 0.f, 0.f};
+            if (zero_grad && gi >= 0) reinterpret_cast<f4 *>(g)[gi] = f4{0.f, 0.f, 0.f, 0.f};
         } else {
             for (int64_t e = 4 * i; e < n; ++e) {
                 float pe = p[e];
@@ -370,6 +378,11 @@
             }
             TN_REQUIRE(t.row1 == 0 ? t.row0 == 0 : (t.H > 0 && t.row0 >= 0 && t.row0 < t.row1 && t.row1 <= t.H), TN_E_SIZE,
                        "tn_adam_reg_multi: rows [row0, row1) must satisfy 0 <= row0 < row1 <= H (row1 == 0, row0 == 0: every row)");
+            TN_REQUIRE(t.box_pitch == 0 ? (t.box_x0 == 0 && t.box_y0 == 0 && t.box_x1 == 0 && t.box_y1 == 0)
+                                        : (t.H > 0 && t.row1 == 0 && t.box_x0 >= 0 && t.box_x0 <= t.box_x1 && t.box_x1 <= t.W && t.box_y0 >= 0 &&
+                                           t.box_y0 <= t.box_y1 && t.box_y1 <= t.H && t.box_pitch >= t.box_x1 - t.box_x0 && t.box_pitch <= t.W),
+                       TN_E_SIZE, "tn_adam_reg_multi: gradient box must satisfy 0 <= x0 <= x1 <= W, 0 <= y0 <= y1 <= H, x1 - x0 <= pitch <= W (planes "
+                                  "only, not with rows)");
             return TN_OK;
         },
         [&](const AdamRegItems &pack, dim3 grid, int) {
diff --git a/tinynerf_amd/fused.py b/tinynerf_amd/fused.py
--- a/tinynerf_amd/fused.py
+++ b/tinynerf_amd/fused.py
@@ -380,7 +380,8 @@
         g_planes, k = grads[:a.n_planes], a.n_planes + a.n_sigma
         gw = _grad_ptrs(grads[a.n_planes:k], grads[k:])
         g_feat = _alloc(a.arena, "g_feat", (n, F), dev)
-        kdesc, _ = _kplanes_desc(planes)
+        take_boxes = a.hint.get("grad_boxes") if (ctx.planes_ready is not None and p.bwd in (_KpBwd.SCATTER_CHAIN, _KpBwd.PAIR_SPLIT)) else None
+        kdesc, _keep = _kplanes_desc(planes, take_boxes() if take_boxes is not None else None)
         gp = ((C.c_void_p * 3) * L.TN_KPLANES_MAX_SCALES)(*[tuple(_hwc(g).data_ptr() for g in g_planes[3 * s:3 * s + 3])
                                                               for s in range(kdesc.n_scales)])
         if p.bwd is _KpBwd.SEPARATE:
diff --git a/tinynerf_amd/models.py b/tinynerf_amd/models.py
--- a/tinynerf_amd/models.py
+++ b/tinynerf_amd/models.py
@@ -321,7 +321,7 @@
     return p.permute(0, 2, 3, 1)[0]
 
 
-def _kplanes_desc(planes: Sequence[Optional[torch.Tensor]]) -> Tuple[L.KPlanesDesc, List[torch.Tensor]]:
+def _kplanes_desc(planes: Sequence[Optional[torch.Tensor]], grad_boxes=None) -> Tuple[L.KPlanesDesc, List[torch.Tensor]]:
     n_scales = len(planes) // 3
     if n_scales > L.TN_KPLANES_MAX_SCALES:
         raise RuntimeError("too many K-Planes scales for the kernel")
@@ -340,6 +340,13 @@
             assert hwc.is_contiguous()
             keep.append(hwc)
             d.planes[s][p] = hwc.data_ptr()
+    if grad_boxes is not None:
+        boxes, flag = grad_boxes
+        for i, (x0, y0, x1, y1, pitch) in enumerate(boxes):
+            b = d.grad_box[i // 3][i % 3]
+            b.x0, b.y0, b.x1, b.y1, b.pitch = x0, y0, x1, y1, pitch
+        d.grad_box_flag = flag.data_ptr()
+        keep.append(flag)
     return d, keep
 
 
diff --git a/tinynerf_amd/optim.py b/tinynerf_amd/optim.py
--- a/tinynerf_amd/optim.py
+++ b/tinynerf_amd/optim.py
@@ -84,6 +84,7 @@
             it.exp_avg, it.exp_avg_sq, it.n = m.data_ptr(), v.data_ptr(), p.numel()
             it.H, it.W, it.C, it.sum_slot, it.cy, it.cx, it.cl1 = H, W, Cc, slot, cy, cx, cl
             it.row0, it.row1 = (plane_reg.get("rows") or {}).get(id(p), (0, 0))
+            it.box_x0, it.box_y0, it.box_x1, it.box_y1, it.box_pitch = (plane_reg.get("boxes") or {}).get(id(p), (0, 0, 0, 0, 0))
         L.call("tn_adam_reg_multi", dev, items, C.c_int32(len(tensors)), *common, C.c_float(plane_reg["upstream"]), L.ptr(plane_reg.get("sums")))
         for p, _, _, _ in tensors:
             st = self.state[p]
diff --git a/tinynerf_amd/run.py b/tinynerf_amd/run.py
--- a/tinynerf_amd/run.py
+++ b/tinynerf_amd/run.py
@@ -1,7 +1,9 @@
 from __future__ import annotations
 
 import os
+import sys
 import ctypes as C
+import functools
 import math
 from dataclasses import dataclass, field
 from typing import Callable, Dict, List, Optional, Tuple
@@ -47,6 +49,7 @@
 from .config import CONFIG as _CONFIG
 ADAM_OVERLAP = _CONFIG.adam_overlap
 SIDE_PLAN = _CONFIG.side_plan
+from .config import GRAD_SCRATCH, GRAD_SCRATCH_LOG
 
 
 @dataclass
@@ -182,6 +185,10 @@
         self._plane_of: Dict[int, int] = {}
         self._reduce_rows: Optional[List[Tuple[int, int]]] = None
         self._reduce_rows_prev: Optional[List[Tuple[int, int]]] = None
+        self._boxes: Optional[List[Tuple[int, int, int, int]]] = None
+        self._boxes_prev: Optional[List[Tuple[int, int, int, int]]] = None
+        self._grid_version = 0
+        self._box_flag: Optional[torch.Tensor] = None
         if world_size > 1 and isinstance(self.renderer.feature_module, KPlanesFeatureField):
             self._plane_of = {id(p): i for i, p in enumerate(self.renderer.feature_module.plane_tensors())}
         self._sharded = bool(cfg.sharded_optimizer and world_size > 1 and self._plane_of and
@@ -292,7 +299,8 @@
             self._plan_event = torch.cuda.Event()
         self._plan_host.copy_(plan, non_blocking=True)
         self._plan_event.record(torch.cuda.current_stream(dev))
-        self._pending = dict(n_b=n_b, idx=idx, o=o, d=d, rgb=rgb, desc=desc, maskbits=maskbits, counts=counts, info=info)
+        self._pending = dict(n_b=n_b, idx=idx, o=o, d=d, rgb=rgb, desc=desc, maskbits=maskbits, counts=counts, info=info,
+                             grid_version=self._grid_version)
 
     @torch.no_grad()
     def build_batch(self) -> Tuple[torch.Tensor, torch.Tensor, torch.Tensor, int]:
@@ -332,7 +340,8 @@
             self._gate_ring.zero_()
         self.renderer._batch_aux = {"key": (packed.data_ptr(), n, R), "ray_ids": ray_ids, "steps": steps, "dirs": pend["d"][:R],
                                     "planes_ready": self._planes_ready if self.world > 1 else (self._planes_adam_early if ADAM_OVERLAP else None),
-                                    "gate": self._gate_ring[slot:slot + 1]}
+                                    "gate": self._gate_ring[slot:slot + 1],
+                                    "grad_boxes": functools.partial(self._take_grad_boxes, pend["grid_version"])}
         self._batch_t = t
         return packed, info, pend["rgb"][:R], k
 
@@ -493,9 +502,13 @@
         v = g.permute(order)
         return v if v.is_contiguous() else None
 
+    def _grad_scratch_on(self) -> bool:
+        return bool(GRAD_SCRATCH and ADAM_OVERLAP and self.world == 1 and self.cfg.method == "kplanes")
+
     @torch.no_grad()
     def _refresh_reduce_rows(self) -> None:
-        if not self._plane_of:
+        scratch = self._grad_scratch_on()
+        if not self._plane_of and not scratch:
             return
         g = self.occupancy_grid
         occ = g.grid > g.threshold
@@ -505,21 +518,54 @@
             idx = torch.arange(line.numel(), device=line.device, dtype=torch.int32)
             big = line.numel() + 1
             lo_hi += [torch.where(line > 0, idx, torch.full_like(idx, big)).amin(), torch.where(line > 0, idx, torch.full_like(idx, -1)).amax()]
-        vals = torch.stack(lo_hi).tolist()
+        if scratch and self._box_flag is None:
+            self._box_flag = torch.zeros(1, dtype=torch.int32, device=self.device)
+        vals = torch.stack(lo_hi + ([self._box_flag[0]] if scratch else [])).tolist()
+        if scratch and vals[6]:
+            raise RuntimeError("tinynerf_amd: a K-Planes sample fell outside the gradient box derived from the occupancy grid -- its plane "
+                               "gradient was dropped (TN_GRAD_SCRATCH=0 keeps the full-size gradient layout)")
         dims = (g.grid.size(2), g.grid.size(1), g.grid.size(0))
+
+        def texels(axis: int, size: int) -> Tuple[int, int]:
+            i0, i1, S = vals[2 * axis], vals[2 * axis + 1], dims[axis]
+            if i1 < 0:
+                return 0, 0
+            v_lo = max(-1.0, -1.0 + 2.0 * (i0 - 1) / max(S - 1, 1)); v_hi = min(1.0, -1.0 + 2.0 * (i1 + 1) / max(S - 1, 1))
+            r0 = int(math.floor((v_lo + 1.0) * 0.5 * (size - 1))) - 1
+            r1 = int(math.floor((v_hi + 1.0) * 0.5 * (size - 1))) + 3
+            return max(0, r0), min(size, r1)
+
         rows: List[Tuple[int, int]] = []
+        boxes: List[Tuple[int, int, int, int]] = []
         for i, p in enumerate(self.renderer.feature_module.plane_tensors()):
-            axis = (1, 2, 2)[i % 3]
-            i0, i1, S, Hp = vals[2 * axis], vals[2 * axis + 1], dims[axis], p.size(2)
-            if i1 < 0:
-                rows.append((0, 0))
-                continue
-            v_lo = max(-1.0, -1.0 + 2.0 * (i0 - 1) / max(S - 1, 1)); v_hi = min(1.0, -1.0 + 2.0 * (i1 + 1) / max(S - 1, 1))
-            r0 = int(math.floor((v_lo + 1.0) * 0.5 * (Hp - 1))) - 1
-            r1 = int(math.floor((v_hi + 1.0) * 0.5 * (Hp - 1))) + 3
-            rows.append((max(0, r0), min(Hp, r1)))
+            rows.append(texels((1, 2, 2)[i % 3], p.size(2)))
+            x0, x1 = texels((0, 0, 1)[i % 3], p.size(3))
+            boxes.append((x0, rows[-1][0], x1, rows[-1][1]) if x1 > x0 and rows[-1][1] > rows[-1][0] else (0, 0, 0, 0))
         prev = self._reduce_rows if self._reduce_rows is not None else [(0, p.size(2)) for p in self.renderer.feature_module.plane_tensors()]
         self._reduce_rows_prev, self._reduce_rows = prev, rows
+        if scratch:
+            self._boxes_prev, self._boxes = self._boxes, boxes
+            self._grid_version += 1
+            if GRAD_SCRATCH_LOG:
+                print("grad boxes (x0, y0, x1, y1) after refresh %d: %s" % (self._grid_version, boxes), file=sys.stderr)
+
+    def _take_grad_boxes(self, batch_version: int):
+        pend = getattr(self, "_early_adam", None)
+        if pend is None or pend.get("done") or self._boxes is None or not self._grad_scratch_on():
+            return None
+        if batch_version == self._grid_version:
+            boxes = self._boxes
+        elif batch_version == self._grid_version - 1 and self._boxes_prev is not None:
+            boxes = [b if not (a[2] > a[0]) else a if not (b[2] > b[0]) else (min(a[0], b[0]), min(a[1], b[1]), max(a[2], b[2]), max(a[3], b[3]))
+                     for a, b in zip(self._boxes, self._boxes_prev)]
+        else:
+            return None
+        with_pitch = [(x0, y0, x1, y1, max(1, x1 - x0)) for x0, y0, x1, y1 in boxes]
+        pend["plane_reg"]["boxes"] = {id(p): b for p, b in zip(self.renderer.feature_module.plane_tensors(), with_pitch)}
+        return with_pitch, self._box_flag
+
+    def grad_box_dropped(self) -> bool:
+        return self._box_flag is not None and bool(self._box_flag.item())
 
     def _reduce_view(self, g: torch.Tensor, plane: Optional[int]) -> Optional[torch.Tensor]:
         flat = Trainer._dense_view(g) if g.numel() >= (1 << 18) else None
```

After: 352.0 million, median of 2. No clear change (+0.5%).
